# YuxiaWu/RAG4DyG

Hardware: AMD Instinct MI355X
Metric: query-seqs/sec encode+top-k over full pool (higher is better)
Workload: dtype f32 (f16x2 operands: two fp16 terms, three products, f32 accumulate)

## Files before the change

include/r4d.h:

```cpp
#ifndef R4D_H
#define R4D_H

#include <stddef.h>
#include <stdint.h>

#ifdef __cplusplus
extern "C" {
#endif

#define R4D_OK 0
#define R4D_ERR_INVALID (-1)
#define R4D_ERR_HIP (-2)
#define R4D_ERR_WORKSPACE (-3)

#define R4D_ABI_VERSION 6

int r4d_abi_version(void);
int r4d_build_flags(void);
const char* r4d_last_error(void);

typedef struct r4d_gpt2_config {
    int32_t n_layer;
    int32_t n_head;
    int32_t n_embd;
    int32_t vocab;
    int32_t n_positions;
    float   ln_eps;
} r4d_gpt2_config;

typedef struct r4d_gpt2_layer {
    const float* ln_1_w;      const float* ln_1_b;
    const float* c_attn_w;    const float* c_attn_b;
    const float* attn_proj_w; const float* attn_proj_b;
    const float* ln_2_w;      const float* ln_2_b;
    const float* c_fc_w;      const float* c_fc_b;
    const float* mlp_proj_w;  const float* mlp_proj_b;
    const float* c_attn_wT;   const float* attn_proj_wT;
    const float* c_fc_wT;     const float* mlp_proj_wT;
    const uint16_t* c_attn_w3;  const uint16_t* attn_proj_w3;
    const uint16_t* c_fc_w3;    const uint16_t* mlp_proj_w3;
    const uint16_t* c_attn_w3t; const uint16_t* attn_proj_w3t;
    const uint16_t* c_fc_w3t;   const uint16_t* mlp_proj_w3t;
    const float* c_attn_wTg;    const float* c_attn_lnc;
    const float* c_fc_wTg;      const float* c_fc_lnc;
    const uint16_t* c_attn_h2;  const uint16_t* attn_proj_h2;
    const uint16_t* c_fc_h2;    const uint16_t* mlp_proj_h2;
} r4d_gpt2_layer;

typedef struct r4d_gpt2_weights {
    const float* wte;
    const float* wpe;
    const float* ln_f_w;
    const float* ln_f_b;
    const r4d_gpt2_layer* layers;
    const float* lm_head;
} r4d_gpt2_weights;

size_t r4d_gpt2_workspace_bytes(const r4d_gpt2_config* cfg, int32_t B, int32_t T);

int r4d_gpt2_encode_f32(const r4d_gpt2_config* cfg, const r4d_gpt2_weights* w,
                        const int64_t* ids_d, const float* inputs_embeds_d, int32_t B, int32_t T,
                        float* out_hidden_d, float* out_meanpool_d, float* out_layers_d, float* out_qkv_d,
                        void* workspace_d, size_t workspace_bytes, void* stream);

size_t r4d_gpt2_groups_workspace_bytes(const r4d_gpt2_config* cfg, int32_t n_groups, const int32_t* Bs,
                                       const int32_t* Ts);
int r4d_gpt2_encode_groups_f32(const r4d_gpt2_config* cfg, const r4d_gpt2_weights* w, int32_t n_groups,
                               const int64_t* const* ids_d, const int32_t* Bs, const int32_t* Ts,
                               float* out_meanpool_d, void* workspace_d, size_t workspace_bytes, void* stream);

int r4d_gpt2_encode_groups_ex_f32(const r4d_gpt2_config* cfg, const r4d_gpt2_weights* w, int32_t n_groups,
                                  const int64_t* const* ids_d, const float* const* embeds_d, const int32_t* Bs,
                                  const int32_t* Ts, float* out_hidden_d, float* out_meanpool_d, float* out_qkv_d,
                                  void* workspace_d, size_t workspace_bytes, void* stream);

size_t r4d_gpt2_decode_workspace_bytes(const r4d_gpt2_config* cfg, int32_t B);
int r4d_gpt2_decode_step_f32(const r4d_gpt2_config* cfg, const r4d_gpt2_weights* w, const int64_t* ids_d,
                             const float* inputs_embeds_d, const int32_t* pos_d, float* kv_cache_d, int32_t B,
                             int32_t t_cap, float* out_hidden_d, void* workspace_d, size_t workspace_bytes,
                             void* stream);

typedef struct r4d_greedy_state {
    float* last_d;
    float* logits_d;
    int64_t* next_d;
    int32_t* lens_d;
    int32_t* pos_d;
    int32_t* active_d;
    int32_t* gen_len_d;
    int32_t* out_tokens_d;
    const int32_t* params_d;
    int32_t out_cap;
} r4d_greedy_state;
typedef struct r4d_decode_graph r4d_decode_graph;

size_t r4d_gpt2_greedy_workspace_bytes(const r4d_gpt2_config* cfg, int32_t B);
int r4d_gpt2_greedy_step_f32(const r4d_gpt2_config* cfg, const r4d_gpt2_weights* w, const r4d_greedy_state* st,
                             float* kv_cache_d, int32_t B, int32_t t_cap, void* workspace_d, size_t workspace_bytes,
                             void* stream);
int r4d_gpt2_greedy_graph_create(const r4d_gpt2_config* cfg, const r4d_gpt2_weights* w, const r4d_greedy_state* st,
                                 float* kv_cache_d, int32_t B, int32_t t_cap, void* workspace_d, size_t workspace_bytes,
                                 r4d_decode_graph** out_graph);
int r4d_decode_graph_launch(r4d_decode_graph* graph, int32_t n_steps, void* stream);
void r4d_decode_graph_destroy(r4d_decode_graph* graph);

int r4d_lm_logits_f32(const float* hidden_d, const float* wte_d, int32_t M, int32_t V, int32_t d,
                      float* logits_d, void* stream);

int r4d_set_attention_fused(int32_t mode);

int r4d_set_attention_h2(int32_t on);
int r4d_set_attention_kblk(int32_t on);
int r4d_pack_kblk_words(const uint32_t* qkv_words_d, int64_t rows, int32_t n_head, int32_t d, uint32_t* kblk_d, void* stream);
int r4d_attention_h2_kblk_f32(const uint32_t* qkv_words_d, const uint32_t* kblk_d, int32_t B, int32_t T, int32_t n_head, int32_t d,
                              float* a_d, void* stream);
int r4d_pack_h2_words_f32(const float* x_d, int64_t n, uint32_t* words_d, void* stream);
int r4d_attention_h2_f32(const uint32_t* qkv_words_d, int32_t B, int32_t T, int32_t n_head, int32_t d, float* a_d, void* stream);

int r4d_set_gemm_h2p(int32_t on);
int r4d_layernorm_lines_f32(const float* x_d, const float* w_d, const float* b_d, int32_t rows, int32_t d, float eps,
                            uint16_t* y_lines_d, void* stream);
int r4d_split2_lines_f16(const float* x_d, int64_t rows, int32_t K, uint16_t* lines_d, void* stream);
int r4d_conv1d_h2p_f32(const uint16_t* x_lines_d, const uint16_t* planes_d, const float* bias_d, const float* residual_d, int32_t M,
                       int32_t K, int32_t N, int32_t epilogue, int32_t out_lines, void* y_d, void* stream);

#define R4D_RANGE_NONFINITE_HIDDEN 1u
#define R4D_RANGE_BAD_NORM 2u
#define R4D_RANGE_BAD_LABEL 4u
int r4d_set_range_flag(uint32_t* flag_d);

int r4d_layernorm_f32(const float* x_d, const float* w_d, const float* b_d, int32_t rows, int32_t d,
                      float eps, float* y_d, void* stream);
int r4d_conv1d_f32(const float* x_d, const float* w_d, const float* w_t_d ,
                   const float* bias_d, const float* residual_d,
                   int32_t M, int32_t K, int32_t N, int32_t epilogue, float* y_d, void* stream);
int r4d_split3_planes_bf16(const float* w_d, int32_t K, int32_t N, int32_t transposed, uint16_t* planes_d, void* stream);
int r4d_conv1d_s3_f32(const float* x_d, const uint16_t* planes_d, const float* bias_d, const float* residual_d,
                      int32_t M, int32_t K, int32_t N, int32_t epilogue, float* y_d, void* stream);
int r4d_split2_planes_f16(const float* w_d, int32_t K, int32_t N, int32_t transposed, uint16_t* planes_d, void* stream);
int r4d_conv1d_h2_f32(const float* x_d, const uint16_t* planes_d, const float* bias_d, const float* residual_d,
                      int32_t M, int32_t K, int32_t N, int32_t epilogue, float* y_d, void* stream);
int r4d_fold_layernorm_f32(const float* wT_d, const float* ln_w_d, const float* ln_b_d, int32_t N, int32_t K, float* wTg_d,
                           float* lnc_d, void* stream);
int r4d_set_gemm_split3(int32_t mode);
int r4d_get_gemm_split3(void);
size_t r4d_attention_workspace_bytes(int32_t B, int32_t n_head, int32_t T);
int r4d_attention_f32(const float* qkv_d, int32_t B, int32_t T, int32_t n_head, int32_t d,
                      float* a_d, void* scores_ws_d, size_t ws_bytes, void* stream);

int r4d_normalize_rows_f32(const float* x_d, int32_t n, int32_t d, float* out_d, void* stream);

size_t r4d_score_topk_workspace_bytes(int32_t Q, int32_t N, int32_t k);
int r4d_score_topk_f32(const float* q_hat_d, const float* pool_hat_d, int32_t Q, int32_t N, int32_t d,
                       int32_t k, int64_t index_offset, float* out_val_d, int64_t* out_idx_d,
                       float* out_scores_d, void* workspace_d, size_t workspace_bytes, void* stream);
size_t r4d_topk_f32_workspace_bytes(int32_t rows, int32_t n, int32_t k);
int r4d_topk_f32(const float* m_d, int32_t rows, int32_t n, int32_t k, float* out_val_d, int64_t* out_idx_d,
                 void* workspace_d, size_t workspace_bytes, void* stream);
size_t r4d_merge_topk_workspace_bytes(int32_t G, int32_t Q, int32_t k);
int r4d_merge_topk_f32(const float* vals_d, const int64_t* idx_d, int32_t G, int32_t Q, int32_t k,
                       float* out_val_d, int64_t* out_idx_d, void* workspace_d, size_t workspace_bytes, void* stream);
size_t r4d_argsort_workspace_bytes(int32_t rows, int32_t n, int32_t elem_bytes);
int r4d_argsort_desc_f32(const float* scores_d, int32_t rows, int32_t n, int32_t* perm_d, void* workspace_d,
                         size_t workspace_bytes, void* stream);
int r4d_argsort_desc_f64(const double* scores_d, int32_t rows, int32_t n, int32_t* perm_d, void* workspace_d,
                         size_t workspace_bytes, void* stream);

int r4d_jaccard_f64(const int32_t* a_ptr_d, const int32_t* a_idx_d, int32_t na, int32_t a_nnz,
                    const int32_t* b_ptr_d, const int32_t* b_idx_d, int32_t nb, int32_t b_nnz,
                    int32_t vocab, int32_t zero_diag, double* out_d, void* stream);
int r4d_jaccard_ordered_f64(const int32_t* a_ptr_d, const int32_t* a_idx_d, int32_t na, int32_t a_nnz,
                            const int32_t* b_ptr_d, const int32_t* b_idx_d, int32_t nb, int32_t b_nnz,
                            int32_t vocab, int32_t zero_diag, const int32_t* a_order_d,
                            const uint32_t* a_dense_d, const uint32_t* b_dense_d, double* out_d, void* stream);
size_t r4d_jaccard_prepared_workspace_bytes(int32_t na, int32_t a_nnz, int32_t nb, int32_t b_nnz, int32_t vocab);
int r4d_jaccard_prepared_f64(const int32_t* a_ptr_d, const int32_t* a_idx_d, int32_t na, int32_t a_nnz,
                             const int32_t* b_ptr_d, const int32_t* b_idx_d, int32_t nb, int32_t b_nnz,
                             int32_t vocab, int32_t zero_diag, int32_t dense_split, int32_t sort_rows,
                             double* out_d, void* workspace_d, size_t workspace_bytes, void* stream);
size_t r4d_topk_f64_workspace_bytes(int32_t rows, int32_t n, int32_t k);
int r4d_topk_f64(const double* m_d, int32_t rows, int32_t n, int32_t k, double* out_val_d,
                 int32_t* out_idx_d, void* workspace_d, size_t workspace_bytes, void* stream);

typedef struct r4d_gpt2_layer_grads {
    float* ln_1_w;      float* ln_1_b;
    float* c_attn_w;    float* c_attn_b;
    float* attn_proj_w; float* attn_proj_b;
    float* ln_2_w;      float* ln_2_b;
    float* c_fc_w;      float* c_fc_b;
    float* mlp_proj_w;  float* mlp_proj_b;
} r4d_gpt2_layer_grads;
typedef struct r4d_gpt2_grads {
    float* wte;
    float* wpe;
    float* ln_f_w;
    float* ln_f_b;
    const r4d_gpt2_layer_grads* layers;
} r4d_gpt2_grads;

typedef struct {
    float embd_p, attn_p, resid_p;
    uint64_t seed, step;
} r4d_train_dropout;
#define R4D_DROPOUT_SITE_EMBD 65535u
int r4d_dropout_f32(const float* x_d, const float* resid_d, int64_t n, float* out_d, float p, uint64_t seed, uint64_t step,
                    uint32_t site, uint64_t index_base, void* stream);

int r4d_set_train_attention(int32_t mode);
int r4d_get_train_attention(void);

size_t r4d_gpt2_train_workspace_bytes(const r4d_gpt2_config* cfg, int32_t n_groups, const int32_t* Bs, const int32_t* Ts);
int r4d_gpt2_train_forward_f32(const r4d_gpt2_config* cfg, const r4d_gpt2_weights* w, int32_t n_groups,
                               const int64_t* const* ids_d, const int32_t* Bs, const int32_t* Ts, float* out_meanpool_d,
                               const r4d_train_dropout* dropout, void* workspace_d, size_t workspace_bytes, void* stream);
int r4d_gpt2_train_backward_f32(const r4d_gpt2_config* cfg, const r4d_gpt2_weights* w, const r4d_gpt2_grads* grads,
                                int32_t n_groups, const int64_t* const* ids_d, const int32_t* Bs, const int32_t* Ts,
                                const float* d_meanpool_d, const r4d_train_dropout* dropout,
                                void* workspace_d, size_t workspace_bytes, void* stream);
size_t r4d_retriever_losses_workspace_bytes(int32_t B);
int r4d_retriever_losses_f32(const float* emb_d, const float* t_anchor_d, const float* t_pos_d, const float* t_neg_d, int32_t B,
                             int32_t d, float temperature, float lambda_decay, float alpha, float grad_scale, float* losses_d,
                             float* d_emb_d, void* workspace_d, size_t workspace_bytes, void* stream);
int r4d_gpt2_train_forward_hidden_f32(const r4d_gpt2_config* cfg, const r4d_gpt2_weights* w, int32_t n_groups,
                                      const int64_t* const* ids_d, const int32_t* Bs, const int32_t* Ts, float* out_hidden_d,
                                      const r4d_train_dropout* dropout, void* workspace_d, size_t workspace_bytes, void* stream);
int r4d_gpt2_train_backward_hidden_f32(const r4d_gpt2_config* cfg, const r4d_gpt2_weights* w, const r4d_gpt2_grads* grads,
                                       int32_t n_groups, const int64_t* const* ids_d, const int32_t* Bs, const int32_t* Ts,
                                       const float* d_hidden_d, const r4d_train_dropout* dropout,
                                       void* workspace_d, size_t workspace_bytes, void* stream);
size_t r4d_lm_ce_workspace_bytes(int32_t N);
int r4d_lm_ce_f32(float* logits_d, int32_t N, int32_t V, int32_t ldV, const int64_t* ids_d, const int64_t* labels_d, int32_t T,
                  float grad_scale, float* loss_d, void* workspace_d, size_t workspace_bytes, void* stream);
typedef struct {
    const float* wte_pad;
    int32_t ldV;
    const uint16_t* w3;
    const uint16_t* w3t;
    const uint16_t* h2;
} r4d_lm_head;
size_t r4d_gpt2_lm_train_workspace_bytes(const r4d_gpt2_config* cfg, int32_t B, int32_t T, int32_t ldV);
int r4d_gpt2_lm_train_step_f32(const r4d_gpt2_config* cfg, const r4d_gpt2_weights* w, const r4d_gpt2_grads* grads,
                               const r4d_lm_head* head, const int64_t* ids_d, int32_t B, int32_t T, float grad_scale, float* loss_d,
                               const r4d_train_dropout* dropout, void* workspace_d, size_t workspace_bytes, void* stream);
#define R4D_HEAD_GRAD_UNTIED 0
#define R4D_HEAD_GRAD_TIED 1
#define R4D_HEAD_GRAD_NONE 2
size_t r4d_rag_train_workspace_bytes(const r4d_gpt2_config* cfg, int32_t B, int32_t Ta, int32_t ldV);
int r4d_rag_train_step_f32(const r4d_gpt2_config* cfg, const r4d_gpt2_weights* w, const r4d_gpt2_grads* grads, const r4d_lm_head* head,
                           int32_t head_mode, float* head_grad_d, const int64_t* aug_ids_d, const float* fused_d, int32_t B, int32_t Ta,
                           int32_t r, float grad_scale, float* loss_d, float* d_fused_d, float* hidden_out_d,
                           const r4d_train_dropout* dropout, void* workspace_d, size_t workspace_bytes, void* stream);
int r4d_weighted_bag_f32(const float* table_d, int32_t vocab, int32_t d, const int64_t* ids_d, const float* weights_d,
                         const int32_t* offsets_d, int32_t n_bags, float* out_d, void* stream);
size_t r4d_embedding_scatter_workspace_bytes(int32_t vocab, int32_t d);
int r4d_embedding_scatter_f32(const float* src_d, const int32_t* row_of_d, const float* weights_d, const int64_t* ids_d, int32_t n,
                              int32_t d, int32_t vocab, float* out_d, void* workspace_d, size_t workspace_bytes, void* stream);
size_t r4d_weight_grad_workspace_bytes(int32_t rows, int32_t in_features, int32_t out_features);
int r4d_weight_grad_f32(const float* x_d, const float* dy_d, int32_t rows, int32_t in_features, int32_t out_features, float* dw_d,
                        float* db_d, void* workspace_d, size_t workspace_bytes, void* stream);
size_t r4d_layernorm_bwd_workspace_bytes(int32_t rows, int32_t d);
int r4d_layernorm_bwd_f32(const float* x_d, const float* w_d, const float* dy_d, const float* add_d, int32_t rows, int32_t d,
                          float eps, float* dx_d, float* dw_d, float* db_d, void* workspace_d, size_t workspace_bytes,
                          void* stream);
int r4d_gelu_new_f32(const float* pre_d, int64_t n, float* y_d, void* stream);
int r4d_gelu_new_bwd_f32(const float* pre_d, const float* dy_d, int64_t n, float* dx_d, void* stream);
int r4d_causal_softmax_bwd_f32(const float* p_d, float* dp_d, int32_t nbh, int32_t T, int32_t ld, float scale_div, void* stream);
int r4d_softmax_dropout_bwd_transpose_f32(const float* p_d, float* dp_d, float* dst_d, int32_t nbh, int32_t T, int32_t ld, float scale_div,
                                          float attn_p, uint64_t seed, uint64_t step, uint32_t site, uint64_t index_base, void* stream);
int r4d_dropout_transpose_f32(const float* p_d, float* out_d, int32_t nbh, int32_t T, int32_t ld, float attn_p, uint64_t seed,
                              uint64_t step, uint32_t site, uint64_t index_base, void* stream);
#define R4D_SUMSQ_FLOATS 1025
int r4d_sumsq_accumulate_f32(const float* x_d, int64_t n, float* accum_d, void* stream);
int r4d_adamw_step_f32(float* p_d, const float* g_d, float* m_d, float* v_d, int64_t n, double lr, double beta1, double beta2,
                       double eps, double weight_decay, int32_t step, const float* grad_sumsq_d, float max_grad_norm,
                       void* stream);

int r4d_profile_enable(int32_t on);
int r4d_profile_num_classes(void);
const char* r4d_profile_class_name(int32_t cls);
int r4d_profile_read(int32_t cls, double* total_ms, int64_t* launches, double* work);

int r4d_dispatch_num_branches(void);
const char* r4d_dispatch_branch_name(int32_t i);
int64_t r4d_dispatch_branch_hits(int32_t i);
int r4d_dispatch_reset(void);

#ifdef __cplusplus
}
#endif
#endif
```

rag4dyg_amd/_lib.py:

```python
import ctypes
import os
from ctypes import POINTER, Structure, c_char_p, c_double, c_float, c_int32, c_int64, c_size_t, c_uint32, c_uint64, c_void_p

PKG = os.path.dirname(os.path.abspath(__file__))
LIB_PATH = os.environ.get("R4D_LIB_PATH") or os.path.join(PKG, "librag4dyg_hip.so")

R4D_ABI_VERSION = 6
HEAD_GRAD_UNTIED, HEAD_GRAD_TIED, HEAD_GRAD_NONE = 0, 1, 2


class R4DError(RuntimeError):
    pass


class GPT2ConfigC(Structure):
    _fields_ = [("n_layer", c_int32), ("n_head", c_int32), ("n_embd", c_int32), ("vocab", c_int32),
                ("n_positions", c_int32), ("ln_eps", c_float)]


class GPT2LayerC(Structure):
    _fields_ = [(n, c_void_p) for n in ("ln_1_w", "ln_1_b", "c_attn_w", "c_attn_b", "attn_proj_w", "attn_proj_b",
                                         "ln_2_w", "ln_2_b", "c_fc_w", "c_fc_b", "mlp_proj_w", "mlp_proj_b",
                                         "c_attn_wT", "attn_proj_wT", "c_fc_wT", "mlp_proj_wT",
                                         "c_attn_w3", "attn_proj_w3", "c_fc_w3", "mlp_proj_w3",
                                         "c_attn_w3t", "attn_proj_w3t", "c_fc_w3t", "mlp_proj_w3t",
                                         "c_attn_wTg", "c_attn_lnc", "c_fc_wTg", "c_fc_lnc",
                                         "c_attn_h2", "attn_proj_h2", "c_fc_h2", "mlp_proj_h2")]


class GreedyStateC(Structure):
    _fields_ = [(n, c_void_p) for n in ("last_d", "logits_d", "next_d", "lens_d", "pos_d", "active_d", "gen_len_d",
                                         "out_tokens_d", "params_d")] + [("out_cap", c_int32)]


class GPT2LayerGradsC(Structure):
    _fields_ = [(n, c_void_p) for n in ("ln_1_w", "ln_1_b", "c_attn_w", "c_attn_b", "attn_proj_w", "attn_proj_b",
                                         "ln_2_w", "ln_2_b", "c_fc_w", "c_fc_b", "mlp_proj_w", "mlp_proj_b")]


class TrainDropoutC(Structure):
    _fields_ = [("embd_p", c_float), ("attn_p", c_float), ("resid_p", c_float), ("seed", c_uint64), ("step", c_uint64)]


class GPT2GradsC(Structure):
    _fields_ = [("wte", c_void_p), ("wpe", c_void_p), ("ln_f_w", c_void_p), ("ln_f_b", c_void_p),
                ("layers", POINTER(GPT2LayerGradsC))]


class LMHeadC(Structure):
    _fields_ = [("wte_pad", c_void_p), ("ldV", c_int32), ("w3", c_void_p), ("w3t", c_void_p), ("h2", c_void_p)]


class GPT2WeightsC(Structure):
    _fields_ = [("wte", c_void_p), ("wpe", c_void_p), ("ln_f_w", c_void_p), ("ln_f_b", c_void_p),
                ("layers", POINTER(GPT2LayerC)), ("lm_head", c_void_p)]


_P = c_void_p
PROTOTYPES = {
    "r4d_abi_version": (c_int32, []),
    "r4d_build_flags": (c_int32, []),
    "r4d_last_error": (c_char_p, []),
    "r4d_gpt2_workspace_bytes": (c_size_t, [POINTER(GPT2ConfigC), c_int32, c_int32]),
    "r4d_gpt2_encode_f32": (c_int32, [POINTER(GPT2ConfigC), POINTER(GPT2WeightsC), _P, _P, c_int32, c_int32,
                                      _P, _P, _P, _P, _P, c_size_t, _P]),
    "r4d_gpt2_groups_workspace_bytes": (c_size_t, [POINTER(GPT2ConfigC), c_int32, POINTER(c_int32), POINTER(c_int32)]),
    "r4d_gpt2_encode_groups_f32": (c_int32, [POINTER(GPT2ConfigC), POINTER(GPT2WeightsC), c_int32, POINTER(_P),
                                             POINTER(c_int32), POINTER(c_int32), _P, _P, c_size_t, _P]),
    "r4d_gpt2_encode_groups_ex_f32": (c_int32, [POINTER(GPT2ConfigC), POINTER(GPT2WeightsC), c_int32, POINTER(_P), POINTER(_P),
                                                POINTER(c_int32), POINTER(c_int32), _P, _P, _P, _P, c_size_t, _P]),
    "r4d_set_attention_fused": (c_int32, [c_int32]),
    "r4d_set_attention_h2": (c_int32, [c_int32]),
    "r4d_set_attention_kblk": (c_int32, [c_int32]),
    "r4d_pack_kblk_words": (c_int32, [_P, c_int64, c_int32, c_int32, _P, _P]),
    "r4d_attention_h2_kblk_f32": (c_int32, [_P, _P, c_int32, c_int32, c_int32, c_int32, _P, _P]),
    "r4d_set_range_flag": (c_int32, [_P]),
    "r4d_set_gemm_h2p": (c_int32, [c_int32]),
    "r4d_layernorm_lines_f32": (c_int32, [_P, _P, _P, c_int32, c_int32, c_float, _P, _P]),
    "r4d_split2_lines_f16": (c_int32, [_P, c_int64, c_int32, _P, _P]),
    "r4d_conv1d_h2p_f32": (c_int32, [_P, _P, _P, _P, c_int32, c_int32, c_int32, c_int32, c_int32, _P, _P]),
    "r4d_pack_h2_words_f32": (c_int32, [_P, c_int64, _P, _P]),
    "r4d_attention_h2_f32": (c_int32, [_P, c_int32, c_int32, c_int32, c_int32, _P, _P]),
    "r4d_gpt2_decode_workspace_bytes": (c_size_t, [POINTER(GPT2ConfigC), c_int32]),
    "r4d_gpt2_decode_step_f32": (c_int32, [POINTER(GPT2ConfigC), POINTER(GPT2WeightsC), _P, _P, _P, _P, c_int32, c_int32,
                                           _P, _P, c_size_t, _P]),
    "r4d_gpt2_greedy_workspace_bytes": (c_size_t, [POINTER(GPT2ConfigC), c_int32]),
    "r4d_gpt2_greedy_step_f32": (c_int32, [POINTER(GPT2ConfigC), POINTER(GPT2WeightsC), POINTER(GreedyStateC), _P, c_int32,
                                           c_int32, _P, c_size_t, _P]),
    "r4d_gpt2_greedy_graph_create": (c_int32, [POINTER(GPT2ConfigC), POINTER(GPT2WeightsC), POINTER(GreedyStateC), _P,
                                               c_int32, c_int32, _P, c_size_t, POINTER(_P)]),
    "r4d_decode_graph_launch": (c_int32, [_P, c_int32, _P]),
    "r4d_decode_graph_destroy": (None, [_P]),
    "r4d_lm_logits_f32": (c_int32, [_P, _P, c_int32, c_int32, c_int32, _P, _P]),
    "r4d_layernorm_f32": (c_int32, [_P, _P, _P, c_int32, c_int32, c_float, _P, _P]),
    "r4d_conv1d_f32": (c_int32, [_P, _P, _P, _P, _P, c_int32, c_int32, c_int32, c_int32, _P, _P]),
    "r4d_split3_planes_bf16": (c_int32, [_P, c_int32, c_int32, c_int32, _P, _P]),
    "r4d_conv1d_s3_f32": (c_int32, [_P, _P, _P, _P, c_int32, c_int32, c_int32, c_int32, _P, _P]),
    "r4d_split2_planes_f16": (c_int32, [_P, c_int32, c_int32, c_int32, _P, _P]),
    "r4d_conv1d_h2_f32": (c_int32, [_P, _P, _P, _P, c_int32, c_int32, c_int32, c_int32, _P, _P]),
    "r4d_fold_layernorm_f32": (c_int32, [_P, _P, _P, c_int32, c_int32, _P, _P, _P]),
    "r4d_set_gemm_split3": (c_int32, [c_int32]),
    "r4d_get_gemm_split3": (c_int32, []),
    "r4d_attention_workspace_bytes": (c_size_t, [c_int32, c_int32, c_int32]),
    "r4d_attention_f32": (c_int32, [_P, c_int32, c_int32, c_int32, c_int32, _P, _P, c_size_t, _P]),
    "r4d_normalize_rows_f32": (c_int32, [_P, c_int32, c_int32, _P, _P]),
    "r4d_score_topk_workspace_bytes": (c_size_t, [c_int32, c_int32, c_int32]),
    "r4d_score_topk_f32": (c_int32, [_P, _P, c_int32, c_int32, c_int32, c_int32, c_int64, _P, _P, _P, _P,
                                     c_size_t, _P]),
    "r4d_topk_f32_workspace_bytes": (c_size_t, [c_int32, c_int32, c_int32]),
    "r4d_topk_f32": (c_int32, [_P, c_int32, c_int32, c_int32, _P, _P, _P, c_size_t, _P]),
    "r4d_merge_topk_workspace_bytes": (c_size_t, [c_int32, c_int32, c_int32]),
    "r4d_merge_topk_f32": (c_int32, [_P, _P, c_int32, c_int32, c_int32, _P, _P, _P, c_size_t, _P]),
    "r4d_argsort_workspace_bytes": (c_size_t, [c_int32, c_int32, c_int32]),
    "r4d_argsort_desc_f32": (c_int32, [_P, c_int32, c_int32, _P, _P, c_size_t, _P]),
    "r4d_argsort_desc_f64": (c_int32, [_P, c_int32, c_int32, _P, _P, c_size_t, _P]),
    "r4d_jaccard_f64": (c_int32, [_P, _P, c_int32, c_int32, _P, _P, c_int32, c_int32, c_int32, c_int32, _P, _P]),
    "r4d_jaccard_ordered_f64": (c_int32, [_P, _P, c_int32, c_int32, _P, _P, c_int32, c_int32, c_int32, c_int32, _P, _P, _P, _P, _P]),
    "r4d_jaccard_prepared_workspace_bytes": (c_size_t, [c_int32, c_int32, c_int32, c_int32, c_int32]),
    "r4d_jaccard_prepared_f64": (c_int32, [_P, _P, c_int32, c_int32, _P, _P, c_int32, c_int32, c_int32, c_int32, c_int32, c_int32, _P, _P,
                                           c_size_t, _P]),
    "r4d_topk_f64_workspace_bytes": (c_size_t, [c_int32, c_int32, c_int32]),
    "r4d_topk_f64": (c_int32, [_P, c_int32, c_int32, c_int32, _P, _P, _P, c_size_t, _P]),
    "r4d_gpt2_train_workspace_bytes": (c_size_t, [POINTER(GPT2ConfigC), c_int32, POINTER(c_int32), POINTER(c_int32)]),
    "r4d_gpt2_train_forward_f32": (c_int32, [POINTER(GPT2ConfigC), POINTER(GPT2WeightsC), c_int32, POINTER(_P), POINTER(c_int32),
                                             POINTER(c_int32), _P, POINTER(TrainDropoutC), _P, c_size_t, _P]),
    "r4d_gpt2_train_backward_f32": (c_int32, [POINTER(GPT2ConfigC), POINTER(GPT2WeightsC), POINTER(GPT2GradsC), c_int32, POINTER(_P),
                                              POINTER(c_int32), POINTER(c_int32), _P, POINTER(TrainDropoutC), _P, c_size_t, _P]),
    "r4d_gpt2_train_forward_hidden_f32": (c_int32, [POINTER(GPT2ConfigC), POINTER(GPT2WeightsC), c_int32, POINTER(_P), POINTER(c_int32),
                                                    POINTER(c_int32), _P, POINTER(TrainDropoutC), _P, c_size_t, _P]),
    "r4d_gpt2_train_backward_hidden_f32": (c_int32, [POINTER(GPT2ConfigC), POINTER(GPT2WeightsC), POINTER(GPT2GradsC), c_int32,
                                                     POINTER(_P), POINTER(c_int32), POINTER(c_int32), _P, POINTER(TrainDropoutC), _P,
                                                     c_size_t, _P]),
    "r4d_lm_ce_workspace_bytes": (c_size_t, [c_int32]),
    "r4d_lm_ce_f32": (c_int32, [_P, c_int32, c_int32, c_int32, _P, _P, c_int32, c_float, _P, _P, c_size_t, _P]),
    "r4d_gpt2_lm_train_workspace_bytes": (c_size_t, [POINTER(GPT2ConfigC), c_int32, c_int32, c_int32]),
    "r4d_gpt2_lm_train_step_f32": (c_int32, [POINTER(GPT2ConfigC), POINTER(GPT2WeightsC), POINTER(GPT2GradsC), POINTER(LMHeadC), _P,
                                             c_int32, c_int32, c_float, _P, POINTER(TrainDropoutC), _P, c_size_t, _P]),
    "r4d_rag_train_workspace_bytes": (c_size_t, [POINTER(GPT2ConfigC), c_int32, c_int32, c_int32]),
    "r4d_rag_train_step_f32": (c_int32, [POINTER(GPT2ConfigC), POINTER(GPT2WeightsC), POINTER(GPT2GradsC), POINTER(LMHeadC), c_int32, _P,
                                         _P, _P, c_int32, c_int32, c_int32, c_float, _P, _P, _P, POINTER(TrainDropoutC), _P, c_size_t, _P]),
    "r4d_weighted_bag_f32": (c_int32, [_P, c_int32, c_int32, _P, _P, _P, c_int32, _P, _P]),
    "r4d_embedding_scatter_workspace_bytes": (c_size_t, [c_int32, c_int32]),
    "r4d_embedding_scatter_f32": (c_int32, [_P, _P, _P, _P, c_int32, c_int32, c_int32, _P, _P, c_size_t, _P]),
    "r4d_retriever_losses_workspace_bytes": (c_size_t, [c_int32]),
    "r4d_retriever_losses_f32": (c_int32, [_P, _P, _P, _P, c_int32, c_int32, c_float, c_float, c_float, c_float, _P, _P, _P, c_size_t, _P]),
    "r4d_dropout_f32": (c_int32, [_P, _P, c_int64, _P, c_float, c_uint64, c_uint64, c_uint32, c_uint64, _P]),
    "r4d_weight_grad_workspace_bytes": (c_size_t, [c_int32, c_int32, c_int32]),
    "r4d_weight_grad_f32": (c_int32, [_P, _P, c_int32, c_int32, c_int32, _P, _P, _P, c_size_t, _P]),
    "r4d_layernorm_bwd_workspace_bytes": (c_size_t, [c_int32, c_int32]),
    "r4d_layernorm_bwd_f32": (c_int32, [_P, _P, _P, _P, c_int32, c_int32, c_float, _P, _P, _P, _P, c_size_t, _P]),
    "r4d_gelu_new_f32": (c_int32, [_P, c_int64, _P, _P]),
    "r4d_gelu_new_bwd_f32": (c_int32, [_P, _P, c_int64, _P, _P]),
    "r4d_causal_softmax_bwd_f32": (c_int32, [_P, _P, c_int32, c_int32, c_int32, c_float, _P]),
    "r4d_softmax_dropout_bwd_transpose_f32": (c_int32, [_P, _P, _P, c_int32, c_int32, c_int32, c_float, c_float, c_uint64, c_uint64,
                                                        c_uint32, c_uint64, _P]),
    "r4d_dropout_transpose_f32": (c_int32, [_P, _P, c_int32, c_int32, c_int32, c_float, c_uint64, c_uint64, c_uint32, c_uint64, _P]),
    "r4d_set_train_attention": (c_int32, [c_int32]),
    "r4d_get_train_attention": (c_int32, []),
    "r4d_sumsq_accumulate_f32": (c_int32, [_P, c_int64, _P, _P]),
    "r4d_adamw_step_f32": (c_int32, [_P, _P, _P, _P, c_int64, c_double, c_double, c_double, c_double, c_double, c_int32, _P, c_float, _P]),
    "r4d_dispatch_num_branches": (c_int32, []),
    "r4d_dispatch_branch_name": (c_char_p, [c_int32]),
    "r4d_dispatch_branch_hits": (c_int64, [c_int32]),
    "r4d_dispatch_reset": (c_int32, []),
    "r4d_profile_enable": (c_int32, [c_int32]),
    "r4d_profile_num_classes": (c_int32, []),
    "r4d_profile_class_name": (c_char_p, [c_int32]),
    "r4d_profile_read": (c_int32, [c_int32, POINTER(c_double), POINTER(c_int64), POINTER(c_double)]),
}

_LIB = None


def load():
    global _LIB
    if _LIB is not None:
        return _LIB
    if not os.path.exists(LIB_PATH):
        raise R4DError(f"{LIB_PATH} not found: build it with `python -m rag4dyg_amd.build` "
                       "(there is no CPU fallback for the product path)")
    import torch
    lib = ctypes.CDLL(LIB_PATH, mode=ctypes.RTLD_GLOBAL)
    for name, (res, args) in PROTOTYPES.items():
        fn = getattr(lib, name)
        fn.restype = res
        fn.argtypes = args
    got = lib.r4d_abi_version()
    if got != R4D_ABI_VERSION:
        raise R4DError(f"ABI mismatch: library {got}, binding {R4D_ABI_VERSION}")
    flags = lib.r4d_build_flags()
    if flags and os.environ.get("R4D_ALLOW_ABLATED_LIB") != "1":
        raise R4DError(f"{LIB_PATH} is a kernel-ablation build (r4d_build_flags() = {flags:#x}): timing aid for tools/ only; "
                       "the product refuses it (set R4D_ALLOW_ABLATED_LIB=1 in a tuning script)")
    _LIB = lib
    return lib


def check(rc, what):
    if rc != 0:
        msg = load().r4d_last_error().decode("utf-8", "replace")
        raise R4DError(f"{what} failed (rc={rc}): {msg}")
```

rag4dyg_amd/build.py:

```python
import os
import subprocess
import sys
from concurrent.futures import ThreadPoolExecutor

PKG = os.path.dirname(os.path.abspath(__file__))
CSRC = os.path.join(PKG, "csrc")
OBJ = os.path.join(PKG, "_build")
LIB = os.path.join(PKG, "librag4dyg_hip.so")
HIPCC = os.environ.get("HIPCC", "/opt/rocm/bin/hipcc")
FLAGS = ["-O3", "--offload-arch=gfx950", "-fPIC", "-std=c++17", "-Wall", "-Wno-unused-function"]


def sources():
    return sorted(os.path.join(CSRC, f) for f in os.listdir(CSRC) if f.endswith(".hip"))


def _deps_mtime():
    hdrs = [os.path.join(CSRC, f) for f in os.listdir(CSRC) if f.endswith(".h")]
    hdrs.append(os.path.join(os.path.dirname(PKG), "include", "r4d.h"))
    return max(os.path.getmtime(h) for h in hdrs)


def _compile(src, force, hdr_m):
    obj = os.path.join(OBJ, os.path.basename(src)[:-4] + ".o")
    if not force and os.path.exists(obj) and os.path.getmtime(obj) >= max(os.path.getmtime(src), hdr_m):
        return obj, False
    cmd = [HIPCC, *FLAGS, "-c", src, "-o", obj]
    r = subprocess.run(cmd, capture_output=True, text=True)
    if r.returncode != 0:
        raise RuntimeError(f"hipcc failed for {src}:\n{r.stdout}\n{r.stderr}")
    if r.stderr.strip():
        sys.stderr.write(r.stderr)
    return obj, True


HANDOFF_KERNELS = {"topk.hip": {"topk_chunk_kernelIfE": (4, 2), "topk_chunk_kernelIdE": (4, 2)},
                   "gemm_skinny.hip": {"gemm_skinny16_kernelILi2ELi0E": (2, 1), "gemm_skinny16_kernelILi3ELi0E": (2, 1)}}


def check_handoff_lowering(src):
    import re
    import tempfile
    names = HANDOFF_KERNELS[os.path.basename(src)]
    with tempfile.TemporaryDirectory() as td:
        asm = os.path.join(td, "k.s")
        r = subprocess.run([HIPCC, "-O3", "--offload-arch=gfx950", "-std=c++17", "--offload-device-only", "-S", src, "-o", asm],
                           capture_output=True, text=True)
        if r.returncode != 0:
            raise RuntimeError(f"hipcc -S failed for {src}:\n{r.stderr}")
        text = open(asm).read()
    for name, (want_st, want_ld) in names.items():
        m = re.search(r"^(_ZN3r4d\d+" + re.escape(name) + r"[^\n:]*):[^\n]*\n(.*?)s_endpgm", text, re.S | re.M)
        if not m:
            raise RuntimeError(f"hand-off check: kernel {name} not found in the assembly of {src}")
        body = m.group(2)
        stores = re.findall(r"global_store_dword(?:x2)? [^\n]*", body)
        loads_sc1 = [ln for ln in re.findall(r"global_load_dword(?:x2)? [^\n]*", body) if " sc1" in ln]
        stores_sc1 = [ln for ln in stores if " sc1" in ln]
        ticket = re.findall(r"global_atomic_add[^\n]*", body)
        if not ticket or len(stores_sc1) < want_st or len(loads_sc1) < want_ld:
            raise RuntimeError(f"hand-off check FAILED for {name}: {len(stores_sc1)} sc1 stores (want {want_st}), {len(loads_sc1)} sc1 loads (want {want_ld}), "
                               f"{len(ticket)} ticket atomics -- the relaxed agent-scope publish / consume of {os.path.basename(src)} "
                               "is no longer lowered to write-through / L1-bypassing instructions; use release / acquire there")


PACKED_F32_FILES = ("gemm_h2.hip", "attention_h2.hip")
PACKED_F32_FORMS = {
    "v_pk_mul_f32 V, V, S op_sel_hi:[1,0]", "v_pk_mul_f32 V, S, V op_sel_hi:[0,1]", "v_pk_mul_f32 V, V, S", "v_pk_mul_f32 V, S, V",
    "v_pk_fma_f32 V, V, S, V op_sel_hi:[1,0,1]", "v_pk_fma_f32 V, S, V, V op_sel_hi:[0,1,1]", "v_pk_fma_f32 V, V, S, V", "v_pk_fma_f32 V, S, V, V",
    "v_pk_fma_f32 V, V, S, V op_sel_hi:[1,0,1] neg_lo:[0,0,1] neg_hi:[0,0,1]",
    "v_pk_fma_f32 V, V, S, V op_sel_hi:[1,0,0] neg_lo:[1,0,0] neg_hi:[1,0,0]",
    "v_pk_fma_f32 V, S, V, V op_sel_hi:[0,1,1] neg_lo:[1,0,0] neg_hi:[1,0,0]",
    "v_pk_add_f32 V, V, S op_sel_hi:[1,0]", "v_pk_add_f32 V, S, V op_sel_hi:[0,1]",
}


def check_packed_f32_forms(src):
    import re
    import tempfile
    with tempfile.TemporaryDirectory() as td:
        asm = os.path.join(td, "k.s")
        r = subprocess.run([HIPCC, "-O3", "--offload-arch=gfx950", "-std=c++17", "--offload-device-only", "-S", src, "-o", asm],
                           capture_output=True, text=True)
        if r.returncode != 0:
            raise RuntimeError(f"hipcc -S failed for {src}:\n{r.stderr}")
        text = open(asm).read()
    seen = {}
    for ln in re.findall(r"^\s*(v_pk_(?:fma|mul|add)_f32 [^\n;]*)", text, re.M):
        if not re.search(r"\bs\[?\d", ln):
            continue
        form = re.sub(r"a\[[0-9:]+\]", "V", re.sub(r"v\[[0-9:]+\]", "V", re.sub(r"\bs\[[0-9:]+\]|\bs\d+\b", "S", ln))).strip()
        seen[form] = seen.get(form, 0) + 1
    new = {f: n for f, n in seen.items() if f not in PACKED_F32_FORMS}
    if new:
        raise RuntimeError(f"packed-fp32 census FAILED for {os.path.basename(src)}: operand forms with an SGPR source that "
                           f"tools/pk_fma_probe.hip has not verified on gfx950: {new} -- add the form to the probe, run it on the GPU, "
                           "then list it in rag4dyg_amd/build.py:PACKED_F32_FORMS (or pin that arithmetic scalar)")
    return seen


def build_library(force=False, verbose=True):
    os.makedirs(OBJ, exist_ok=True)
    hdr_m = _deps_mtime()
    with ThreadPoolExecutor(max_workers=4) as ex:
        res = list(ex.map(lambda s: _compile(s, force, hdr_m), sources()))
    objs = [o for o, _ in res]
    for src, (_o, compiled) in zip(sources(), res):
        if compiled and os.path.basename(src) in HANDOFF_KERNELS:
            check_handoff_lowering(src)
        if compiled and os.path.basename(src) in PACKED_F32_FILES:
            check_packed_f32_forms(src)
    stale = os.path.exists(LIB) and any(os.path.getmtime(o) > os.path.getmtime(LIB) for o in objs)
    if force or stale or any(c for _, c in res) or not os.path.exists(LIB):
        cmd = [HIPCC, "--offload-arch=gfx950", "-shared", "-fPIC", "-o", LIB, *objs]
        r = subprocess.run(cmd, capture_output=True, text=True)
        if r.returncode != 0:
            raise RuntimeError(f"link failed:\n{r.stdout}\n{r.stderr}")
        if verbose:
            print(f"built {LIB}")
    elif verbose:
        print(f"up to date: {LIB}")
    return LIB


if __name__ == "__main__":
    build_library(force="--force" in sys.argv)
```

rag4dyg_amd/csrc/common.h:

```cpp
#pragma once
#include <hip/hip_runtime.h>
#include <stdint.h>
#include <stdio.h>
#include <stdarg.h>
#include "../../include/r4d.h"

namespace r4d {

void set_error(const char* fmt, ...);
int dbgflag_kc(); int dbgflag_att(); int dbgflag_sk(); int dbgflag_jac(); int dbgflag_scan(); int dbgflag_s3(); int dbgflag_h2();

#define R4D_REQUIRE(cond, ...)                     \
    do {                                           \
        if (!(cond)) {                             \
            r4d::set_error(__VA_ARGS__);           \
            return R4D_ERR_INVALID;                \
        }                                          \
    } while (0)

#define R4D_HIP(call)                                                                  \
    do {                                                                               \
        hipError_t e_ = (call);                                                        \
        if (e_ != hipSuccess) {                                                        \
            r4d::set_error("%s: %s", #call, hipGetErrorString(e_));                    \
            return R4D_ERR_HIP;                                                        \
        }                                                                              \
    } while (0)

#define R4D_CHECK_LAUNCH(name)                                                         \
    do {                                                                               \
        hipError_t e_ = hipGetLastError();                                             \
        if (e_ != hipSuccess) {                                                        \
            r4d::set_error("%s: launch failed: %s", name, hipGetErrorString(e_));      \
            return R4D_ERR_HIP;                                                        \
        }                                                                              \
    } while (0)

enum ProfClass {
    PK_GEMM_128x128_NN = 0, PK_GEMM_128x128_NT, PK_GEMM_128x64_NN, PK_GEMM_128x64_NT, PK_GEMM_64x64_NN,
    PK_GEMM_64x64_NT, PK_GEMM_KC_128x128x32, PK_GEMM_KC_128x128x16, PK_GEMM_KC_128x64x16, PK_GEMM_KC_64x64x32, PK_GEMM_S3_128x256, PK_GEMM_S3_128x128, PK_GEMM_S3TN, PK_GEMM_H2_128x256, PK_GEMM_H2_128x128, PK_GEMM_SKINNY, PK_GEMM_SKINNY_EPI,
    PK_EMBED_LN, PK_LAYERNORM, PK_SOFTMAX, PK_DECODE_ATTN, PK_GREEDY_ADVANCE,
    PK_ATTN_FUSED, PK_LNF_MEANPOOL, PK_MEANPOOL_REDUCE, PK_NORMALIZE, PK_POOL_SCAN, PK_TOPK, PK_MERGE_TOPK, PK_RANK_COUNT, PK_JACCARD, PK_JACCARD_PREP, PK_LM_CE,
    PK_SPLICE_EMBED, PK_WEIGHTED_BAG, PK_EMB_SCATTER, PK_COUNT
};
extern bool g_prof_on;
void prof_begin_impl(int cls, double work, hipStream_t s);
void prof_end_impl(hipStream_t s);
struct ProfScope {
    hipStream_t s; bool on;
    ProfScope(int cls, double work, hipStream_t st) : s(st), on(g_prof_on) { if (on) prof_begin_impl(cls, work, s); }
    ~ProfScope() { if (on) prof_end_impl(s); }
};

#define R4D_BRANCH_LIST(X)                                                                                              \
    X(KC_128x128x16, "gemm_kc:128x128x16") X(KC_128x64x16, "gemm_kc:128x64x16") X(KC_64x64x32, "gemm_kc:64x64x32")       \
    X(KC_128x128x32, "tuning:gemm_kc:128x128x32") X(KC_ROWSPLIT, "gemm_kc:row-split (two launches)")                      \
    X(S3_128x256, "gemm_s3:128x256x32") X(S3_PERSISTENT, "gemm_s3:128x256x32 persistent (pipeline across tiles)") X(S3_128x128, "gemm_s3:128x128x32") X(S3_F32B, "gemm_s3:both operands split on the fly (scoring GEMM)") X(S3_TN, "gemm_s3tn:128x256x32 (weight gradients, transposing LDS reads)")      \
    X(H2_128x256, "gemm_h2:128x256x32 (f16x2)") X(H2_128x128, "gemm_h2:128x128x32 (f16x2)") X(H2P_128x256, "gemm_h2p:128x256x32 (f16x2, A as lines, LDS-DMA)") X(H2P_128x128, "gemm_h2p:128x128x32 (f16x2, A as lines, LDS-DMA)") \
    X(F32_128x128, "gemm_f32:128x128") X(F32_128x64, "gemm_f32:128x64") X(F32_64x64, "gemm_f32:64x64")                   \
    X(F32_NT, "gemm_f32:B as [N,K]") X(F32_NN, "gemm_f32:B as [K,N]") X(TN_SPLITK, "gemm_tn:split-K") X(TN_SINGLE, "gemm_tn:one slice") \
    X(SK16_NG2, "skinny16:ng2") X(SK16_NG3, "skinny16:ng3") X(SK16_NG2_LN, "skinny16:ng2+layernorm") X(SK16_LN_FOLDED, "skinny16:LayerNorm pre-folded into the weight") X(SK16_NG3_LN, "skinny16:ng3+layernorm") \
    X(SK16_SPLITK, "skinny16:split-K last-arriver") X(SK8_NG2, "skinny8:ng2") X(SK8_NG3, "skinny8:ng3")                    \
    X(SK8_LN, "tuning:skinny8:+layernorm") X(SK8_SPLITK, "skinny8:split-K + epilogue launch") X(SK_PLAIN, "skinny:plain + epilogue launch") \
    X(ATT_KS32, "attention:key-split hd32") X(ATT_KS64, "attention:key-split hd64") X(ATT_CS96, "attention:column-split hd96") \
    X(ATT_CS128, "attention:column-split hd128") X(ATT_CS256, "attention:column-split hd256") X(ATT_H2_KS32, "attention:f16x2 key-split hd32") X(ATT_H2_KS64, "attention:f16x2 key-split hd64") X(ATT_H2_KS96, "attention:f16x2 key-split hd96") X(ATT_H2_128, "attention:f16x2 hd128") X(ATT_H2_256, "attention:f16x2 hd256") X(ATT_H2_KS32_KBLK, "attention:f16x2 key-split hd32, key-blocked K") X(ATT_H2_KS64_KBLK, "attention:f16x2 key-split hd64, key-blocked K") X(ATT_H2_KS96_KBLK, "attention:f16x2 key-split hd96, key-blocked K") X(ATT_H2_128_KBLK, "attention:f16x2 hd128, key-blocked K") X(ATT_H2_256_KBLK, "attention:f16x2 hd256, key-blocked K")                              \
    X(ATT_KS_FORCED, "tuning:attention:key-split at hd96/128/256") X(ATT_3LAUNCH, "attention:three-launch GEMM form")      \
    X(SCAN_1_1, "scan:d32") X(SCAN_2_1, "scan:d64") X(SCAN_4_1, "scan:d128") X(SCAN_4_2, "scan:d256") X(SCAN_4_3, "scan:d384") \
    X(SCAN_8_2, "scan:d512") X(SCAN_4_4, "tuning:scan:d512 4-way") X(SCAN_8_3, "scan:d768") X(SCAN_8_4, "scan:d1024")       \
    X(SCAN_SHORT, "scan:short shard (even rows, two tiles in flight)") X(SCAN_DMA, "scan:short shard, LDS-DMA staged") X(SCAN_RING, "scan:long shard, LDS-DMA ring") X(SCAN_GEMM, "scan:tiled GEMM (Q > 64 or other d)") X(SCAN_TILED, "scan:128x256 tiles in the scan kernels' arithmetic (Q >= 64)") X(SCAN_BF16X3, "scan:bf16x3 operands") X(SCAN_F32, "scan:exact-f32 operands")  \
    X(TOPK_ONE_WG, "topk:one workgroup per row") X(TOPK_TICKET, "topk:cross-workgroup ticket merge")                      \
    X(TOPK_MULTI, "topk:second launch over candidates") X(TOPK_F64, "topk:f64 rows")                                      \
    X(EMBED_LN4, "embed+layernorm:16-byte lanes") X(EMBED_GENERIC, "embed+layernorm:generic") X(LN4_2, "layernorm:ln4<2>") X(LN4_4, "layernorm:ln4<4>") X(LN4_8, "layernorm:ln4<8>") X(LN_GENERIC, "layernorm:generic") \
    X(LNF_8, "lnf_meanpool:<8>") X(LNF_16, "lnf_meanpool:<16>") X(LNF_32, "lnf_meanpool:<32>")                             \
    X(DEC_ATT_32, "decode_attention:<32>") X(DEC_ATT_64, "decode_attention:<64>")                                         \
    X(JAC_LDS, "jaccard:LDS table") X(JAC_MERGE, "jaccard:merge walk (vocab too large for LDS)")                          \
    X(JAC_PREP_DENSE_LDS, "jaccard_prep:dense tokens, LDS histogram") X(JAC_PREP_DENSE_GLOBAL, "jaccard_prep:dense tokens, global histogram") X(JAC_PREP_ORDER, "jaccard_prep:rows longest first") \
    X(ARGSORT_ONE, "argsort:one chunk") X(ARGSORT_MULTI, "argsort:chunk sort + rank scatter")
enum DispatchBranch {
#define X(id, name) BR_##id,
    R4D_BRANCH_LIST(X)
#undef X
    BR_COUNT
};
extern unsigned long long g_branch_hits[BR_COUNT];
#define R4D_BRANCH(id) (++r4d::g_branch_hits[r4d::BR_##id])

extern unsigned* g_range_flag;

static inline size_t align_up(size_t x, size_t a) { return (x + a - 1) / a * a; }
static inline int cdiv(int a, int b) { return (a + b - 1) / b; }

enum GemmEpilogue { EPI_NONE = 0, EPI_GELU = 1, EPI_RESIDUAL = 2, EPI_SCALE_DIV = 3, EPI_HALF_PLUS = 4,
                    EPI_GELU_KEEP = 5, EPI_GELU_GRAD = 6,
                    EPI_H2WORDS = 7 };
enum GemmCausal { CAUSAL_NONE = 0, CAUSAL_QK = 1, CAUSAL_PV = 2 };

struct GemmArgs {
    const float* A; const float* B; float* C;
    const float* bias;
    const float* resid;
    int M, N, K;
    int lda, ldb, ldc, ldr;
    int b_trans;
    int b_rows;
    int a_cols;
    int nbatch, nb1;
    long long sA0, sA1, sB0, sB1, sC0, sC1;
    int epilogue; float scale_div;
    int causal;
};
int launch_gemm_f32(const GemmArgs& g, hipStream_t stream);
int launch_gemm_f32_kc(const GemmArgs& g, hipStream_t stream);
size_t gemm_tn_scratch_floats(int M, int N, int Kt);
int launch_gemm_f32_tn(const float* A, const float* B, float* C, int M, int N, int Kt, int lda, int ldb, float* scratch,
                       hipStream_t stream, float* colsum_out = nullptr, float* colsum_scratch = nullptr,
                       size_t colsum_scratch_floats = 0, bool* colsum_done = nullptr);
bool gemm_skinny_supported(int M, int K, int N);
size_t gemm_skinny_scratch_floats(int K, int N);
bool gemm_skinny_fuses_ln(int M, int K, int N);
void* gemm_skinny_counters(float* scratch, size_t* bytes);
int launch_gemm_skinny(const float* x, const float* wT, const float* bias, const float* resid, int M, int K, int N,
                       int epilogue, float* y, float* scratch, hipStream_t s, const float* ln_w = nullptr,
                       const float* ln_b = nullptr, float ln_eps = 0.f, bool counters_zeroed = false, const float* ln_fold = nullptr);
int launch_fold_layernorm(const float* wT, const float* g, const float* beta, int N, int K, float* wTg, float* lnc, hipStream_t s);

struct S3Args {
    const float* A; const unsigned short* planes; float* C;
    const float* bias; const float* resid;
    int M, N, K, lda, ldc, ldr, epilogue;
    unsigned* kblk; int kb_hd;
};
bool gemm_s3_supported(int M, int K, int N);
int launch_gemm_s3(const S3Args& a, hipStream_t stream);
bool gemm_s3_f32b_supported(int M, int K, int N);
int launch_gemm_s3_f32b(const float* A, const float* B, float* C, int M, int N, int K, int lda, int ldc, int epilogue, hipStream_t stream);
int launch_gemm_s3_scan_order(const float* q_hat, const float* pool_hat, float* scores, int Q, int N, int d, int ng, hipStream_t stream);
bool gemm_h2_supported(int M, int K, int N);
int launch_gemm_h2(const S3Args& a, hipStream_t stream);
int launch_split2_planes(const float* w, int N, int K, long long ld_k, long long ld_n, unsigned short* planes, hipStream_t s);
extern int g_gemm_h2p;
bool gemm_h2p_supported(int M, int K, int N);
int launch_gemm_h2p(const S3Args& a, const unsigned short* a_lines, bool out_lines, hipStream_t stream);
int launch_split2_lines(const float* x, long long rows, int K, unsigned short* lines, hipStream_t s);
extern int g_gemm_split3;
int conv1d(const float* x, const float* w, const float* wT, const float* bias, const float* resid, int M, int K, int N,
           int epilogue, float* y, hipStream_t s, float* skinny_scratch = nullptr, bool sk_counters_zeroed = false,
           const unsigned short* w3 = nullptr, const unsigned short* w2h = nullptr);
bool gemm_s3tn_supported(int I, int J, int M, int lda, int ldb);
int gemm_s3tn_slices(int I, int J, int M, int max_slices);
int launch_gemm_s3tn(const float* X, const float* dY, float* out, int I, int J, int M, int lda, int ldb, int S, int* slices_out,
                     hipStream_t stream, float* db_partials = nullptr);
int launch_split3_planes(const float* w, int N, int K, long long ld_k, long long ld_n, unsigned short* planes, hipStream_t s);

struct DropKey { unsigned seed_lo, seed_hi, step_lo, step_hi; };
int launch_dropout(const float* x, const float* resid, long long n, float* out, float p, DropKey key, unsigned site,
                   unsigned long long base, hipStream_t s);
constexpr int EMB_SUM_BITS = 62;
__device__ __forceinline__ int emb_scale_exp(unsigned max_bits, int lg_rows) {
    const int e = (int)((max_bits >> 23) & 255u) - 126;
    return EMB_SUM_BITS - lg_rows - e;
}
static inline int emb_lg_rows(long long table_rows) {
    int lg = 0;
    while ((1LL << lg) < table_rows) ++lg;
    return lg;
}
int launch_embedding_fix_to_f32(const unsigned long long* acc, long long n, long long table_rows, float* out, hipStream_t s);

size_t gpt2_train_workspace_floats(const r4d_gpt2_config* cfg, int n_groups, const int32_t* Bs, const int32_t* Ts);
struct SpliceIn { const float* fused; int r; };
int gpt2_train_forward(const r4d_gpt2_config* cfg, const r4d_gpt2_weights* w, int n_groups, const int64_t* const* ids_d,
                       const int32_t* Bs, const int32_t* Ts, float* out_meanpool_d, float* out_hidden_d,
                       const r4d_train_dropout* dropout, void* workspace_d, size_t workspace_bytes, hipStream_t s,
                       const SpliceIn* sp = nullptr);
int gpt2_train_backward(const r4d_gpt2_config* cfg, const r4d_gpt2_weights* w, const r4d_gpt2_grads* gr, int n_groups,
                        const int64_t* const* ids_d, const int32_t* Bs, const int32_t* Ts, const float* d_meanpool_d,
                        const float* d_hidden_d, const r4d_train_dropout* dropout, void* workspace_d, size_t workspace_bytes,
                        hipStream_t s, const SpliceIn* sp = nullptr, float* d_fused = nullptr);
int launch_splice_embed_ln(const int64_t* aug_ids, const float* fused, int r, const float* wte, const float* wpe, int vocab, int B,
                           int T, int d, const float* w, const float* b, float eps, float* x_out, float* y_out, hipStream_t s);

struct LMLayout { size_t train, h, logits, dh, dwte, tn, ce, total; };
LMLayout lm_layout(const r4d_gpt2_config* cfg, int B, int T, int ldV);
int check_ce(int N, int V, int ldV, int T);
int lm_head_train(const float* h, int N, int V, int d, const r4d_lm_head* head, const int64_t* src, int T, float gscale, float* loss,
                  float* logits, float* dh, float* dwte, float* tn_scratch, float* ce_ws, hipStream_t s);
int launch_add_inplace(float* y, const float* x, long long n, hipStream_t s);

template <typename T> size_t topk_ws_bytes(int rows, int n, int k);
template <typename T>
int topk_rows(const T* vals, const long long* idx_in, int rows, int n, long long ld, int k, long long index_offset, T* out_v,
              long long* out_i, void* ws, size_t ws_bytes, bool counters_zeroed, hipStream_t s);

int launch_layernorm(const float* x, const float* w, const float* b, int rows, int d, float eps, float* y,
                     hipStream_t s);
bool layernorm_lines_supported(int d);
int launch_layernorm_lines(const float* x, const float* w, const float* b, int rows, int d, float eps, unsigned short* y_lines, hipStream_t s);
constexpr int ATT_MAXG = 16;
struct RowGroups {
    int n;
    int B[ATT_MAXG], T[ATT_MAXG];
    const int64_t* ids[ATT_MAXG];
    const float* emb[ATT_MAXG];
};
int launch_embed_layernorm_groups(const RowGroups& G, const float* wte, const float* wpe, int vocab, int d,
                                  const float* w, const float* b, float eps, float* x_out, float* y_out, hipStream_t s, bool y_lines = false);
int launch_causal_softmax(float* S, int nbh, int T, int ld, int row_tile, hipStream_t s);
int launch_embed_pos_layernorm(const int64_t* ids, const float* emb, const int32_t* pos, const float* wte,
                               const float* wpe, int vocab, int n_positions, int t_cap, int B, int d, const float* w,
                               const float* b, float eps, float* x_out, float* y_out, hipStream_t s,
                               void* zero_words = nullptr, size_t zero_bytes = 0);
int launch_decode_attention(const float* qkv_new, float* kv_layer, const int32_t* pos, int B, int t_cap, int H, int d,
                            float* out, hipStream_t s);
struct GreedyState {
    int64_t* next; int32_t* lens; int32_t* pos; int32_t* active; int32_t* gen_len; int32_t* out_tokens;
    const int32_t* params;
    int out_cap, t_cap;
};
struct GreedyEmbed { const float* wte; const float* wpe; float* x_out; unsigned* zero_words; int vocab, n_positions, d, n_zero; };
int launch_greedy_advance(const float* logits, int B, int V, const GreedyState& st, hipStream_t s, const GreedyEmbed* embed = nullptr);
struct AttnGroups {
    int n;
    int seq_prefix[ATT_MAXG + 1];
    int T[ATT_MAXG];
    long long row0[ATT_MAXG];
};
bool attention_h2_supported(int H, int d);
int launch_attention_h2_groups(const unsigned* qkv_words, int n, const int* Bs, const int* Ts, const long long* row0s, int H, int d,
                               float* out, hipStream_t s, bool out_lines = false, const unsigned* kblk = nullptr);
int launch_pack_kblk_words(const unsigned* qkv_words, long long M, int H, int d, unsigned* kblk, hipStream_t s);
static inline size_t kblk_words(size_t M, int d) { return (M + 31) / 32 * 32 * (size_t)d; }
int launch_pack_h2_words(const float* x, long long n, unsigned* words, hipStream_t s);
int dbgflag_att_h2();
int launch_attention_fused(const float* qkv, int B, int T, int H, int d, float* out, hipStream_t s);
int launch_attention_fused_groups(const float* qkv, int n, const int* Bs, const int* Ts, const long long* row0s, int H,
                                  int d, float* out, hipStream_t s);
extern int g_attention_variant;
extern int g_attention_fused;
constexpr int LNF_ROWS_PER_CHUNK = 16;
size_t lnf_meanpool_scratch_floats(int B, int T, int d);
int launch_lnf_meanpool_groups(const RowGroups& G, const float* x, const float* w, const float* b, int d, float eps,
                               float* hidden_out, float* pool_out, float* scratch, hipStream_t s);

}
```

rag4dyg_amd/csrc/encoder.hip:

```cpp
#include <math.h>
#include <stdlib.h>
#include <string.h>
#include <vector>
#include "common.h"

namespace r4d {

static thread_local char g_err[512] = "";
void set_error(const char* fmt, ...) {
    va_list ap;
    va_start(ap, fmt);
    vsnprintf(g_err, sizeof(g_err), fmt, ap);
    va_end(ap);
}

int g_gemm_split3 = 1;

int conv1d(const float* x, const float* w, const float* wT, const float* bias, const float* resid, int M, int K,
           int N, int epilogue, float* y, hipStream_t s, float* skinny_scratch, bool sk_counters_zeroed,
           const unsigned short* w3, const unsigned short* w2h) {
    if (skinny_scratch && wT && gemm_skinny_supported(M, K, N))
        return launch_gemm_skinny(x, wT, bias, resid, M, K, N, epilogue, y, skinny_scratch, s, nullptr, nullptr, 0.f,
                                  sk_counters_zeroed);
    if (w2h && g_gemm_split3 == 2 && (epilogue <= EPI_RESIDUAL || epilogue == EPI_GELU_KEEP || epilogue == EPI_H2WORDS) && gemm_h2_supported(M, K, N)) {
        S3Args a;
        memset(&a, 0, sizeof(a));
        a.A = x; a.planes = w2h; a.C = y; a.bias = bias; a.resid = resid;
        a.M = M; a.N = N; a.K = K; a.lda = K; a.ldc = N; a.ldr = N; a.epilogue = epilogue;
        return launch_gemm_h2(a, s);
    }
    if (w3 && g_gemm_split3 && gemm_s3_supported(M, K, N)) {
        S3Args a;
        memset(&a, 0, sizeof(a));
        a.A = x; a.planes = w3; a.C = y; a.bias = bias; a.resid = resid;
        a.M = M; a.N = N; a.K = K; a.lda = K; a.ldc = N; a.ldr = N; a.epilogue = epilogue;
        return launch_gemm_s3(a, s);
    }
    R4D_REQUIRE(epilogue != EPI_H2WORDS, "conv1d: the h2-word epilogue exists in the f16x2 GEMM only");
    GemmArgs g;
    memset(&g, 0, sizeof(g));
    g.A = x; g.C = y; g.bias = bias; g.resid = resid;
    g.M = M; g.N = N; g.K = K; g.lda = K; g.ldc = N; g.ldr = N;
    if (wT) { g.B = wT; g.ldb = K; g.b_trans = 1; g.b_rows = N; }
    else { g.B = w; g.ldb = N; g.b_trans = 0; g.b_rows = K; }
    g.nbatch = 1; g.nb1 = 1;
    g.epilogue = epilogue; g.scale_div = 1.f; g.causal = CAUSAL_NONE;
    return launch_gemm_f32(g, s);
}

static int conv1d_lines(const unsigned short* x_lines, const unsigned short* w2h, const float* bias, const float* resid, int M, int K, int N,
                        int epilogue, void* y, bool out_lines, hipStream_t s, unsigned* kblk = nullptr, int kb_hd = 0) {
    S3Args a;
    memset(&a, 0, sizeof(a));
    a.planes = w2h; a.C = (float*)y; a.bias = bias; a.resid = resid;
    a.M = M; a.N = N; a.K = K; a.lda = K; a.ldc = N; a.ldr = N; a.epilogue = epilogue;
    a.kblk = kblk; a.kb_hd = kb_hd;
    return launch_gemm_h2p(a, x_lines, out_lines, s);
}

static inline int tpad(int T) { return (T + 127) / 128 * 128; }

int g_attention_fused = -1;
int g_attention_h2 = 1;
static int g_attention_kblk = -1;

static int attention(const float* qkv, int B, int T, int H, int d, float* a_out, float* scores, hipStream_t s) {
    const bool fused = g_attention_fused != 0;
    if (fused) {
        const int rc_f = launch_attention_fused(qkv, B, T, H, d, a_out, s);
        if (rc_f <= 0) return rc_f;
    }
    R4D_BRANCH(ATT_3LAUNCH);
    const int hd = d / H, ld = tpad(T);
    GemmArgs g;
    memset(&g, 0, sizeof(g));
    g.A = qkv; g.B = qkv + d; g.C = scores;
    g.M = T; g.N = T; g.K = hd; g.lda = 3 * d; g.ldb = 3 * d; g.ldc = ld;
    g.b_trans = 1; g.b_rows = T; g.nbatch = B * H; g.nb1 = H;
    g.sA0 = (long long)T * 3 * d; g.sA1 = hd; g.sB0 = g.sA0; g.sB1 = hd;
    g.sC0 = (long long)H * T * ld; g.sC1 = (long long)T * ld;
    g.epilogue = EPI_SCALE_DIV; g.scale_div = (float)sqrt((double)hd); g.causal = CAUSAL_QK;
    int rc = launch_gemm_f32(g, s);
    if (rc) return rc;
    rc = launch_causal_softmax(scores, B * H, T, ld, 128, s);
    if (rc) return rc;
    memset(&g, 0, sizeof(g));
    g.A = scores; g.B = qkv + 2 * d; g.C = a_out;
    g.M = T; g.N = hd; g.K = T; g.lda = ld; g.ldb = 3 * d; g.ldc = d;
    g.b_trans = 0; g.b_rows = T; g.nbatch = B * H; g.nb1 = H;
    g.sA0 = (long long)H * T * ld; g.sA1 = (long long)T * ld;
    g.sB0 = (long long)T * 3 * d; g.sB1 = hd; g.sC0 = (long long)T * d; g.sC1 = hd;
    g.a_cols = ld;
    g.epilogue = EPI_NONE; g.scale_div = 1.f; g.causal = CAUSAL_PV;
    return launch_gemm_f32(g, s);
}

struct Group {
    const int64_t* ids; const float* emb; int B, T; size_t row0, seq0;
};

static RowGroups row_groups(const Group* groups, int g0, int n_groups) {
    RowGroups R;
    R.n = n_groups - g0 < ATT_MAXG ? n_groups - g0 : ATT_MAXG;
    for (int j = 0; j < ATT_MAXG; ++j) {
        const bool in = j < R.n;
        R.B[j] = in ? groups[g0 + j].B : 0; R.T[j] = in ? groups[g0 + j].T : 0;
        R.ids[j] = in ? groups[g0 + j].ids : nullptr; R.emb[j] = in ? groups[g0 + j].emb : nullptr;
    }
    return R;
}

struct Workspace {
    float *x, *ln, *qkv, *att, *fc, *scores, *pool;
    unsigned* kblk;
    size_t bytes;
};
static Workspace carve(void* base, size_t M, size_t score_floats, size_t pool_floats, int d) {
    size_t off = 0;
    auto take = [&](size_t nfloat) {
        float* p = base ? (float*)((char*)base + off) : nullptr;
        off += align_up(nfloat * sizeof(float), 256);
        return p;
    };
    Workspace w;
    w.x = take(M * d); w.ln = take(M * d); w.qkv = take(M * 3 * d); w.att = take(M * d); w.fc = take(M * 4 * d);
    w.scores = take(score_floats);
    w.pool = take(pool_floats);
    w.kblk = reinterpret_cast<unsigned*>(take(kblk_words(M, d)));
    w.bytes = off;
    return w;
}
static size_t score_floats(int B, int H, int T) { return (size_t)B * H * T * tpad(T); }

static int check_cfg(const r4d_gpt2_config* c) {
    R4D_REQUIRE(c != nullptr, "gpt2: null config");
    R4D_REQUIRE(c->n_layer >= 1 && c->n_head >= 1 && c->n_embd >= 64, "gpt2: bad config L=%d H=%d d=%d", c->n_layer,
                c->n_head, c->n_embd);
    R4D_REQUIRE(c->n_embd % 64 == 0 && c->n_embd <= 2048, "gpt2: n_embd=%d must be a multiple of 64, <= 2048", c->n_embd);
    R4D_REQUIRE(c->n_embd % c->n_head == 0 && (c->n_embd / c->n_head) % 16 == 0,
                "gpt2: head_dim=%d/%d must be a multiple of 16", c->n_embd, c->n_head);
    return R4D_OK;
}

}

using namespace r4d;

extern "C" {

int r4d_abi_version(void) { return R4D_ABI_VERSION; }
int r4d_build_flags(void) {
    return dbgflag_kc() | (dbgflag_att() << 1) | (dbgflag_sk() << 2) | (dbgflag_jac() << 3) | (dbgflag_scan() << 4) | (dbgflag_s3() << 5) | (dbgflag_h2() << 6) | (dbgflag_att_h2() << 7);
}
int r4d_fold_layernorm_f32(const float* wT_d, const float* ln_w_d, const float* ln_b_d, int32_t N, int32_t K, float* wTg_d,
                           float* lnc_d, void* stream) {
    return launch_fold_layernorm(wT_d, ln_w_d, ln_b_d, N, K, wTg_d, lnc_d, (hipStream_t)stream);
}

int r4d_set_gemm_split3(int32_t mode) { g_gemm_split3 = mode == 2 ? 2 : (mode != 0); return R4D_OK; }
int r4d_get_gemm_split3(void) { return g_gemm_split3; }
int r4d_set_range_flag(uint32_t* flag_d) { g_range_flag = flag_d; return R4D_OK; }
int r4d_set_attention_kblk(int32_t on) {
    const int prev = g_attention_kblk < 0 ? 1 : g_attention_kblk;
    g_attention_kblk = on != 0;
    return prev;
}
int r4d_set_attention_h2(int32_t on) {
    const int prev = g_attention_h2;
    g_attention_h2 = on != 0;
    return prev;
}

int r4d_set_attention_fused(int32_t mode) {
    g_attention_variant = (mode == 2) ? 1 : 0;
    g_attention_fused = mode < 0 ? -1 : (mode != 0);
    return R4D_OK;
}
const char* r4d_last_error(void) { return g_err; }

size_t r4d_gpt2_workspace_bytes(const r4d_gpt2_config* cfg, int32_t B, int32_t T) {
    if (!cfg || B <= 0 || T <= 0) return 0;
    return carve(nullptr, (size_t)B * T, score_floats(B, cfg->n_head, T), lnf_meanpool_scratch_floats(B, T, cfg->n_embd),
                 cfg->n_embd).bytes;
}

size_t r4d_gpt2_groups_workspace_bytes(const r4d_gpt2_config* cfg, int32_t n_groups, const int32_t* Bs,
                                       const int32_t* Ts) {
    if (!cfg || n_groups <= 0 || !Bs || !Ts) return 0;
    size_t M = 0, sc = 0, pl = 0;
    for (int g = 0; g < n_groups; ++g) {
        if (Bs[g] <= 0 || Ts[g] <= 0) return 0;
        M += (size_t)Bs[g] * Ts[g];
        const size_t f = score_floats(Bs[g], cfg->n_head, Ts[g]);
        if (f > sc) sc = f;
        pl += lnf_meanpool_scratch_floats(Bs[g], Ts[g], cfg->n_embd);
    }
    return carve(nullptr, M, sc, pl, cfg->n_embd).bytes;
}

}

namespace r4d {

static int encode_impl(const r4d_gpt2_config* cfg, const r4d_gpt2_weights* w, const Group* groups, int n_groups,
                       float* out_hidden_d, float* out_meanpool_d, float* out_layers_d, float* out_qkv_d,
                       void* workspace_d, size_t workspace_bytes, hipStream_t s) {
    int rc = check_cfg(cfg);
    if (rc) return rc;
    R4D_REQUIRE(w && w->wte && w->wpe && w->ln_f_w && w->ln_f_b && w->layers, "gpt2: null weights");
    R4D_REQUIRE(out_hidden_d || out_meanpool_d, "gpt2: no output requested");
    const int d = cfg->n_embd, H = cfg->n_head;
    size_t Mtot = 0, sc = 0, pl = 0;
    for (int g = 0; g < n_groups; ++g) {
        const Group& G = groups[g];
        R4D_REQUIRE((G.ids != nullptr) != (G.emb != nullptr),
                    "gpt2: specify exactly one of input_ids and inputs_embeds");
        R4D_REQUIRE(G.B >= 1 && G.T >= 1, "gpt2: empty batch B=%d T=%d", G.B, G.T);
        R4D_REQUIRE(G.T <= cfg->n_positions && G.T <= 1024, "gpt2: T=%d exceeds n_positions=%d", G.T, cfg->n_positions);
        Mtot += (size_t)G.B * G.T;
        const size_t f = score_floats(G.B, H, G.T);
        if (f > sc) sc = f;
        pl += lnf_meanpool_scratch_floats(G.B, G.T, d);
    }
    R4D_REQUIRE(Mtot <= 0x7fffffff / (size_t)(16 * d), "gpt2: %zu rows in one call is too many", Mtot);
    const int M = (int)Mtot;
    Workspace ws = carve(workspace_d, Mtot, sc, pl, d);
    if (!workspace_d || workspace_bytes < ws.bytes) {
        set_error("gpt2: workspace %zu bytes < required %zu", workspace_bytes, ws.bytes);
        return R4D_ERR_WORKSPACE;
    }
    for (int l = 0; l < cfg->n_layer; ++l) {
        const r4d_gpt2_layer& L = w->layers[l];
        R4D_REQUIRE(L.ln_1_w && L.c_attn_w && L.attn_proj_w && L.ln_2_w && L.c_fc_w && L.mlp_proj_w,
                    "gpt2: null weight in layer %d", l);
        const bool lines = g_gemm_split3 == 2 && g_gemm_h2p && L.c_attn_h2 && L.c_fc_h2 && L.mlp_proj_h2 && layernorm_lines_supported(d) &&
                           gemm_h2p_supported(M, d, 3 * d) && gemm_h2p_supported(M, d, 4 * d) && gemm_h2p_supported(M, 4 * d, d);
        unsigned short* ln_lines = reinterpret_cast<unsigned short*>(ws.ln);
        unsigned short* fc_lines = reinterpret_cast<unsigned short*>(ws.fc);
        if (l == 0) {
            for (int g0 = 0; g0 < n_groups; g0 += ATT_MAXG) {
                const RowGroups R = row_groups(groups, g0, n_groups);
                const size_t r0 = groups[g0].row0;
                rc = launch_embed_layernorm_groups(R, w->wte, w->wpe, cfg->vocab, d, L.ln_1_w, L.ln_1_b, cfg->ln_eps,
                                                   ws.x + r0 * d, ws.ln + r0 * d, s, lines);
                if (rc) return rc;
            }
        } else if ((rc = lines ? launch_layernorm_lines(ws.x, L.ln_1_w, L.ln_1_b, M, d, cfg->ln_eps, ln_lines, s)
                               : launch_layernorm(ws.x, L.ln_1_w, L.ln_1_b, M, d, cfg->ln_eps, ws.ln, s))) {
            return rc;
        }
        if (out_layers_d &&
            hipMemcpyAsync(out_layers_d + (size_t)l * M * d, ws.x, (size_t)M * d * sizeof(float),
                           hipMemcpyDeviceToDevice, s) != hipSuccess) {
            set_error("gpt2: layer copy failed");
            return R4D_ERR_HIP;
        }
        float* qkv = out_qkv_d ? out_qkv_d + (size_t)l * M * 3 * d : ws.qkv;
        bool words = !out_qkv_d && g_attention_h2 && g_attention_fused != 0 && g_gemm_split3 == 2 && L.c_attn_h2 &&
                     attention_h2_supported(H, d) && gemm_h2_supported(M, d, 3 * d);
        for (int g0 = 0; g0 < n_groups && words; g0 += ATT_MAXG) {
            int nseq = 0;
            for (int j = g0; j < n_groups && j < g0 + ATT_MAXG; ++j) nseq += groups[j].B;
            if (nseq > 65535) words = false;
        }
        if (g_attention_kblk < 0) { const char* e = getenv("R4D_ATT_KBLK"); g_attention_kblk = e ? atoi(e) != 0 : 1; }
        const bool kblk = words && lines && g_attention_kblk && (d / H) % 32 == 0;
        if (kblk && (M & 31) &&
            hipMemsetAsync(ws.kblk + (size_t)(M / 32) * 32 * d, 0, (size_t)32 * d * sizeof(unsigned), s) != hipSuccess) {
            set_error("gpt2: memset of the key-block tail failed");
            return R4D_ERR_HIP;
        }
        if (lines) rc = conv1d_lines(ln_lines, L.c_attn_h2, L.c_attn_b, nullptr, M, d, 3 * d, words ? EPI_H2WORDS : EPI_NONE, qkv, false, s,
                                     kblk ? ws.kblk : nullptr, kblk ? d / H : 0);
        else rc = conv1d(ws.ln, L.c_attn_w, L.c_attn_wT, L.c_attn_b, nullptr, M, d, 3 * d, words ? EPI_H2WORDS : EPI_NONE, qkv, s, nullptr, false, L.c_attn_w3, L.c_attn_h2);
        if (rc) return rc;
        const bool att_lines = words && lines && L.attn_proj_h2 && gemm_h2p_supported(M, d, d);
        bool fused_done = false;
        if (words) {
            fused_done = true;
            for (int g0 = 0; g0 < n_groups; g0 += ATT_MAXG) {
                int Bs[ATT_MAXG], Ts[ATT_MAXG];
                long long r0[ATT_MAXG];
                const int n = n_groups - g0 < ATT_MAXG ? n_groups - g0 : ATT_MAXG;
                for (int j = 0; j < n; ++j) { Bs[j] = groups[g0 + j].B; Ts[j] = groups[g0 + j].T; r0[j] = (long long)groups[g0 + j].row0; }
                if ((rc = launch_attention_h2_groups(reinterpret_cast<const unsigned*>(qkv), n, Bs, Ts, r0, H, d, ws.att, s, att_lines,
                                                     kblk ? ws.kblk : nullptr))) return rc;
            }
        } else if (g_attention_fused != 0) {
            fused_done = true;
            for (int g0 = 0; g0 < n_groups && fused_done; g0 += ATT_MAXG) {
                int Bs[ATT_MAXG], Ts[ATT_MAXG];
                long long r0[ATT_MAXG];
                const int n = n_groups - g0 < ATT_MAXG ? n_groups - g0 : ATT_MAXG;
                int nseq = 0;
                for (int j = 0; j < n; ++j) {
                    Bs[j] = groups[g0 + j].B; Ts[j] = groups[g0 + j].T; r0[j] = (long long)groups[g0 + j].row0;
                    nseq += Bs[j];
                }
                if (nseq > 65535) { fused_done = false; break; }
                rc = launch_attention_fused_groups(qkv, n, Bs, Ts, r0, H, d, ws.att, s);
                if (rc < 0) return rc;
                if (rc > 0) fused_done = false;
            }
        }
        if (!fused_done) {
            for (int g = 0; g < n_groups; ++g) {
                const Group& G = groups[g];
                if ((rc = attention(qkv + G.row0 * 3 * d, G.B, G.T, H, d, ws.att + G.row0 * d, ws.scores, s))) return rc;
            }
        }
        if (att_lines) rc = conv1d_lines(reinterpret_cast<const unsigned short*>(ws.att), L.attn_proj_h2, L.attn_proj_b, ws.x, M, d, d, EPI_RESIDUAL, ws.x, false, s);
        else rc = conv1d(ws.att, L.attn_proj_w, L.attn_proj_wT, L.attn_proj_b, ws.x, M, d, d, EPI_RESIDUAL, ws.x, s, nullptr, false, L.attn_proj_w3, L.attn_proj_h2);
        if (rc) return rc;
        if (lines) {
            if ((rc = launch_layernorm_lines(ws.x, L.ln_2_w, L.ln_2_b, M, d, cfg->ln_eps, ln_lines, s))) return rc;
            if ((rc = conv1d_lines(ln_lines, L.c_fc_h2, L.c_fc_b, nullptr, M, d, 4 * d, EPI_GELU, fc_lines, true, s))) return rc;
            if ((rc = conv1d_lines(fc_lines, L.mlp_proj_h2, L.mlp_proj_b, ws.x, M, 4 * d, d, EPI_RESIDUAL, ws.x, false, s))) return rc;
            continue;
        }
        if ((rc = launch_layernorm(ws.x, L.ln_2_w, L.ln_2_b, M, d, cfg->ln_eps, ws.ln, s))) return rc;
        if ((rc = conv1d(ws.ln, L.c_fc_w, L.c_fc_wT, L.c_fc_b, nullptr, M, d, 4 * d, EPI_GELU, ws.fc, s, nullptr, false, L.c_fc_w3, L.c_fc_h2))) return rc;
        if ((rc = conv1d(ws.fc, L.mlp_proj_w, L.mlp_proj_wT, L.mlp_proj_b, ws.x, M, 4 * d, d, EPI_RESIDUAL, ws.x, s, nullptr, false, L.mlp_proj_w3, L.mlp_proj_h2))) return rc;
    }
    size_t part0 = 0;
    for (int g0 = 0; g0 < n_groups; g0 += ATT_MAXG) {
        const RowGroups R = row_groups(groups, g0, n_groups);
        const Group& G = groups[g0];
        rc = launch_lnf_meanpool_groups(R, ws.x + G.row0 * d, w->ln_f_w, w->ln_f_b, d, cfg->ln_eps,
                                        out_hidden_d ? out_hidden_d + G.row0 * d : nullptr,
                                        out_meanpool_d ? out_meanpool_d + G.seq0 * d : nullptr, ws.pool + part0, s);
        if (rc) return rc;
        for (int j = 0; j < R.n; ++j) part0 += lnf_meanpool_scratch_floats(R.B[j], R.T[j], d);
    }
    return R4D_OK;
}

}

extern "C" {

int r4d_gpt2_encode_f32(const r4d_gpt2_config* cfg, const r4d_gpt2_weights* w, const int64_t* ids_d,
                        const float* inputs_embeds_d, int32_t B, int32_t T, float* out_hidden_d,
                        float* out_meanpool_d, float* out_layers_d, float* out_qkv_d, void* workspace_d,
                        size_t workspace_bytes, void* stream) {
    Group G = {ids_d, inputs_embeds_d, B, T, 0, 0};
    return encode_impl(cfg, w, &G, 1, out_hidden_d, out_meanpool_d, out_layers_d, out_qkv_d, workspace_d,
                       workspace_bytes, (hipStream_t)stream);
}

int r4d_gpt2_encode_groups_f32(const r4d_gpt2_config* cfg, const r4d_gpt2_weights* w, int32_t n_groups,
                               const int64_t* const* ids_d, const int32_t* Bs, const int32_t* Ts,
                               float* out_meanpool_d, void* workspace_d, size_t workspace_bytes, void* stream) {
    R4D_REQUIRE(n_groups >= 1 && n_groups <= 4096 && ids_d && Bs && Ts, "gpt2 groups: bad arguments");
    R4D_REQUIRE(out_meanpool_d, "gpt2 groups: out_meanpool_d is null");
    std::vector<Group> gs((size_t)n_groups);
    size_t row0 = 0, seq0 = 0;
    for (int g = 0; g < n_groups; ++g) {
        gs[g] = Group{ids_d[g], nullptr, Bs[g], Ts[g], row0, seq0};
        if (Bs[g] > 0 && Ts[g] > 0) { row0 += (size_t)Bs[g] * Ts[g]; seq0 += (size_t)Bs[g]; }
    }
    return encode_impl(cfg, w, gs.data(), n_groups, nullptr, out_meanpool_d, nullptr, nullptr, workspace_d,
                       workspace_bytes, (hipStream_t)stream);
}

int r4d_gpt2_encode_groups_ex_f32(const r4d_gpt2_config* cfg, const r4d_gpt2_weights* w, int32_t n_groups,
                                  const int64_t* const* ids_d, const float* const* embeds_d, const int32_t* Bs,
                                  const int32_t* Ts, float* out_hidden_d, float* out_meanpool_d, float* out_qkv_d,
                                  void* workspace_d, size_t workspace_bytes, void* stream) {
    R4D_REQUIRE(n_groups >= 1 && n_groups <= 4096 && Bs && Ts, "gpt2 groups: bad arguments");
    R4D_REQUIRE((ids_d != nullptr) != (embeds_d != nullptr), "gpt2 groups: specify exactly one of ids_d and embeds_d");
    std::vector<Group> gs((size_t)n_groups);
    size_t row0 = 0, seq0 = 0;
    for (int g = 0; g < n_groups; ++g) {
        gs[g] = Group{ids_d ? ids_d[g] : nullptr, embeds_d ? embeds_d[g] : nullptr, Bs[g], Ts[g], row0, seq0};
        if (Bs[g] > 0 && Ts[g] > 0) { row0 += (size_t)Bs[g] * Ts[g]; seq0 += (size_t)Bs[g]; }
    }
    return encode_impl(cfg, w, gs.data(), n_groups, out_hidden_d, out_meanpool_d, nullptr, out_qkv_d, workspace_d,
                       workspace_bytes, (hipStream_t)stream);
}

static size_t decode_skinny_floats(int d) {
    size_t m = 0;
    const int shapes[4][2] = {{d, 3 * d}, {d, d}, {d, 4 * d}, {4 * d, d}};
    for (auto& kn : shapes)
        if (gemm_skinny_supported(1, kn[0], kn[1])) { const size_t f = gemm_skinny_scratch_floats(kn[0], kn[1]); if (f > m) m = f; }
    return m;
}

size_t r4d_gpt2_decode_workspace_bytes(const r4d_gpt2_config* cfg, int32_t B) {
    if (!cfg || B <= 0) return 0;
    return carve(nullptr, (size_t)B, 0, decode_skinny_floats(cfg->n_embd), cfg->n_embd).bytes;
}

static int decode_step_impl(const r4d_gpt2_config* cfg, const r4d_gpt2_weights* w, const int64_t* ids_d,
                            const float* inputs_embeds_d, const int32_t* pos_d, float* kv_cache_d, int32_t B,
                            int32_t t_cap, float* out_hidden_d, void* workspace_d, size_t workspace_bytes,
                            void* stream, bool x_ready) {
    hipStream_t s = (hipStream_t)stream;
    int rc = check_cfg(cfg);
    if (rc) return rc;
    R4D_REQUIRE(w && w->wte && w->wpe && w->ln_f_w && w->ln_f_b && w->layers, "gpt2 decode: null weights");
    R4D_REQUIRE(x_ready || (ids_d != nullptr) != (inputs_embeds_d != nullptr), "gpt2 decode: specify exactly one of ids and inputs_embeds");
    R4D_REQUIRE(pos_d && kv_cache_d && out_hidden_d, "gpt2 decode: null pointer");
    R4D_REQUIRE(B >= 1 && t_cap >= 1, "gpt2 decode: B=%d t_cap=%d", B, t_cap);
    const int d = cfg->n_embd, H = cfg->n_head;
    const size_t sk_floats = decode_skinny_floats(d);
    Workspace ws = carve(workspace_d, (size_t)B, 0, sk_floats, d);
    if (!workspace_d || workspace_bytes < ws.bytes) {
        set_error("gpt2 decode: workspace %zu bytes < required %zu", workspace_bytes, ws.bytes);
        return R4D_ERR_WORKSPACE;
    }
    float* sk = (sk_floats && B <= 32) ? ws.pool : nullptr;
    const size_t layer_stride = (size_t)B * t_cap * 2 * d;
    size_t cbytes = 0;
    void* cnt = sk ? gemm_skinny_counters(sk, &cbytes) : nullptr;
    for (int l = 0; l < cfg->n_layer; ++l) {
        const r4d_gpt2_layer& L = w->layers[l];
        R4D_REQUIRE(L.ln_1_w && L.c_attn_w && L.attn_proj_w && L.ln_2_w && L.c_fc_w && L.mlp_proj_w,
                    "gpt2 decode: null weight in layer %d", l);
        const bool fuse_ln = sk && L.c_attn_wT && L.c_fc_wT && gemm_skinny_fuses_ln(B, d, 3 * d);
        if (l == 0 && !x_ready)
            rc = launch_embed_pos_layernorm(ids_d, inputs_embeds_d, pos_d, w->wte, w->wpe, cfg->vocab, cfg->n_positions,
                                            t_cap, B, d, L.ln_1_w, L.ln_1_b, cfg->ln_eps, ws.x, ws.ln, s, cnt, cbytes);
        else if (!fuse_ln)
            rc = launch_layernorm(ws.x, L.ln_1_w, L.ln_1_b, B, d, cfg->ln_eps, ws.ln, s);
        if (rc) return rc;
        if (fuse_ln && (l > 0 || x_ready))
            rc = (L.c_attn_wTg && L.c_attn_lnc)
                     ? launch_gemm_skinny(ws.x, L.c_attn_wTg, L.c_attn_b, nullptr, B, d, 3 * d, EPI_NONE, ws.qkv, sk, s, nullptr, nullptr,
                                          cfg->ln_eps, true, L.c_attn_lnc)
                     : launch_gemm_skinny(ws.x, L.c_attn_wT, L.c_attn_b, nullptr, B, d, 3 * d, EPI_NONE, ws.qkv, sk, s, L.ln_1_w,
                                          L.ln_1_b, cfg->ln_eps, true);
        else
            rc = conv1d(ws.ln, L.c_attn_w, L.c_attn_wT, L.c_attn_b, nullptr, B, d, 3 * d, EPI_NONE, ws.qkv, s, sk);
        if (rc) return rc;
        if ((rc = launch_decode_attention(ws.qkv, kv_cache_d + (size_t)l * layer_stride, pos_d, B, t_cap, H, d, ws.att, s)))
            return rc;
        if ((rc = conv1d(ws.att, L.attn_proj_w, L.attn_proj_wT, L.attn_proj_b, ws.x, B, d, d, EPI_RESIDUAL, ws.x, s, sk, true))) return rc;
        if (fuse_ln) {
            rc = (L.c_fc_wTg && L.c_fc_lnc)
                     ? launch_gemm_skinny(ws.x, L.c_fc_wTg, L.c_fc_b, nullptr, B, d, 4 * d, EPI_GELU, ws.fc, sk, s, nullptr, nullptr,
                                          cfg->ln_eps, true, L.c_fc_lnc)
                     : launch_gemm_skinny(ws.x, L.c_fc_wT, L.c_fc_b, nullptr, B, d, 4 * d, EPI_GELU, ws.fc, sk, s, L.ln_2_w, L.ln_2_b,
                                          cfg->ln_eps, true);
        } else {
            if ((rc = launch_layernorm(ws.x, L.ln_2_w, L.ln_2_b, B, d, cfg->ln_eps, ws.ln, s))) return rc;
            rc = conv1d(ws.ln, L.c_fc_w, L.c_fc_wT, L.c_fc_b, nullptr, B, d, 4 * d, EPI_GELU, ws.fc, s, sk);
        }
        if (rc) return rc;
        if ((rc = conv1d(ws.fc, L.mlp_proj_w, L.mlp_proj_wT, L.mlp_proj_b, ws.x, B, 4 * d, d, EPI_RESIDUAL, ws.x, s, sk, true))) return rc;
    }
    return launch_layernorm(ws.x, w->ln_f_w, w->ln_f_b, B, d, cfg->ln_eps, out_hidden_d, s);
}

int r4d_gpt2_decode_step_f32(const r4d_gpt2_config* cfg, const r4d_gpt2_weights* w, const int64_t* ids_d,
                             const float* inputs_embeds_d, const int32_t* pos_d, float* kv_cache_d, int32_t B,
                             int32_t t_cap, float* out_hidden_d, void* workspace_d, size_t workspace_bytes,
                             void* stream) {
    return decode_step_impl(cfg, w, ids_d, inputs_embeds_d, pos_d, kv_cache_d, B, t_cap, out_hidden_d, workspace_d, workspace_bytes,
                            stream, false);
}

static size_t greedy_pool_floats(const r4d_gpt2_config* cfg) {
    const size_t a = decode_skinny_floats(cfg->n_embd);
    const size_t b = gemm_skinny_supported(1, cfg->n_embd, cfg->vocab) ? gemm_skinny_scratch_floats(cfg->n_embd, cfg->vocab) : 0;
    return a > b ? a : b;
}

size_t r4d_gpt2_greedy_workspace_bytes(const r4d_gpt2_config* cfg, int32_t B) {
    if (!cfg || B <= 0) return 0;
    return carve(nullptr, (size_t)B, 0, greedy_pool_floats(cfg), cfg->n_embd).bytes;
}

int r4d_gpt2_greedy_step_f32(const r4d_gpt2_config* cfg, const r4d_gpt2_weights* w, const r4d_greedy_state* st,
                             float* kv_cache_d, int32_t B, int32_t t_cap, void* workspace_d, size_t workspace_bytes,
                             void* stream) {
    hipStream_t s = (hipStream_t)stream;
    int rc = check_cfg(cfg);
    if (rc) return rc;
    R4D_REQUIRE(w && w->wte && st && st->last_d && st->logits_d, "gpt2 greedy: null pointer");
    R4D_REQUIRE(B >= 1 && t_cap >= 1, "gpt2 greedy: B=%d t_cap=%d", B, t_cap);
    const int d = cfg->n_embd, V = cfg->vocab;
    Workspace ws = carve(workspace_d, (size_t)B, 0, greedy_pool_floats(cfg), d);
    if (!workspace_d || workspace_bytes < ws.bytes) {
        set_error("gpt2 greedy: workspace %zu bytes < required %zu", workspace_bytes, ws.bytes);
        return R4D_ERR_WORKSPACE;
    }
    const float* head = w->lm_head ? w->lm_head : w->wte;
    if (B <= 32 && gemm_skinny_supported(B, d, V))
        rc = launch_gemm_skinny(st->last_d, head, nullptr, nullptr, B, d, V, EPI_NONE, st->logits_d, ws.pool, s);
    else
        rc = r4d_lm_logits_f32(st->last_d, head, B, V, d, st->logits_d, stream);
    if (rc) return rc;
    GreedyState g;
    g.next = st->next_d; g.lens = st->lens_d; g.pos = st->pos_d; g.active = st->active_d; g.gen_len = st->gen_len_d;
    g.out_tokens = st->out_tokens_d; g.params = st->params_d; g.out_cap = st->out_cap; g.t_cap = t_cap;
    GreedyEmbed ge;
    ge.wte = w->wte; ge.wpe = w->wpe; ge.x_out = ws.x; ge.vocab = cfg->vocab; ge.n_positions = cfg->n_positions; ge.d = d;
    size_t cbytes = 0;
    void* cnt = ws.pool ? gemm_skinny_counters(ws.pool, &cbytes) : nullptr;
    ge.zero_words = (unsigned*)cnt; ge.n_zero = (int)(cbytes / 4);
    if ((rc = launch_greedy_advance(st->logits_d, B, V, g, s, &ge))) return rc;
    return decode_step_impl(cfg, w, st->next_d, nullptr, st->pos_d, kv_cache_d, B, t_cap, st->last_d, workspace_d, workspace_bytes,
                            stream, true);
}

struct r4d_decode_graph { hipGraph_t graph; hipGraphExec_t exec; };

int r4d_gpt2_greedy_graph_create(const r4d_gpt2_config* cfg, const r4d_gpt2_weights* w, const r4d_greedy_state* st,
                                 float* kv_cache_d, int32_t B, int32_t t_cap, void* workspace_d, size_t workspace_bytes,
                                 r4d_decode_graph** out_graph) {
    R4D_REQUIRE(out_graph, "gpt2 greedy graph: null out_graph");
    *out_graph = nullptr;
    R4D_REQUIRE(!g_prof_on, "gpt2 greedy graph: switch the launch profiler off before capturing");
    hipStream_t cap = nullptr;
    R4D_HIP(hipStreamCreateWithFlags(&cap, hipStreamNonBlocking));
    hipError_t e = hipStreamBeginCapture(cap, hipStreamCaptureModeRelaxed);
    if (e != hipSuccess) {
        (void)hipStreamDestroy(cap);
        set_error("gpt2 greedy graph: begin capture: %s", hipGetErrorString(e));
        return R4D_ERR_HIP;
    }
    const int rc = r4d_gpt2_greedy_step_f32(cfg, w, st, kv_cache_d, B, t_cap, workspace_d, workspace_bytes, cap);
    hipGraph_t graph = nullptr;
    e = hipStreamEndCapture(cap, &graph);
    (void)hipStreamDestroy(cap);
    if (rc) {
        if (graph) (void)hipGraphDestroy(graph);
        return rc;
    }
    if (e != hipSuccess || !graph) {
        set_error("gpt2 greedy graph: end capture: %s", hipGetErrorString(e));
        return R4D_ERR_HIP;
    }
    hipGraphExec_t exec = nullptr;
    e = hipGraphInstantiate(&exec, graph, nullptr, nullptr, 0);
    if (e != hipSuccess) {
        (void)hipGraphDestroy(graph);
        set_error("gpt2 greedy graph: instantiate: %s", hipGetErrorString(e));
        return R4D_ERR_HIP;
    }
    *out_graph = new r4d_decode_graph{graph, exec};
    return R4D_OK;
}

int r4d_decode_graph_launch(r4d_decode_graph* graph, int32_t n_steps, void* stream) {
    R4D_REQUIRE(graph && graph->exec && n_steps >= 0, "decode graph: null graph or n_steps=%d", n_steps);
    for (int i = 0; i < n_steps; ++i) R4D_HIP(hipGraphLaunch(graph->exec, (hipStream_t)stream));
    return R4D_OK;
}

void r4d_decode_graph_destroy(r4d_decode_graph* graph) {
    if (!graph) return;
    if (graph->exec) (void)hipGraphExecDestroy(graph->exec);
    if (graph->graph) (void)hipGraphDestroy(graph->graph);
    delete graph;
}

int r4d_lm_logits_f32(const float* hidden_d, const float* wte_d, int32_t M, int32_t V, int32_t d, float* logits_d,
                      void* stream) {
    R4D_REQUIRE(hidden_d && wte_d && logits_d, "lm_logits: null pointer");
    GemmArgs g;
    memset(&g, 0, sizeof(g));
    g.A = hidden_d; g.B = wte_d; g.C = logits_d;
    g.M = M; g.N = V; g.K = d; g.lda = d; g.ldb = d; g.ldc = V;
    g.b_trans = 1; g.b_rows = V; g.nbatch = 1; g.nb1 = 1; g.epilogue = EPI_NONE; g.scale_div = 1.f;
    return launch_gemm_f32(g, (hipStream_t)stream);
}

int r4d_layernorm_f32(const float* x_d, const float* w_d, const float* b_d, int32_t rows, int32_t d, float eps,
                      float* y_d, void* stream) {
    R4D_REQUIRE(x_d && w_d && b_d && y_d, "layernorm: null pointer");
    return launch_layernorm(x_d, w_d, b_d, rows, d, eps, y_d, (hipStream_t)stream);
}

int r4d_layernorm_lines_f32(const float* x_d, const float* w_d, const float* b_d, int32_t rows, int32_t d, float eps,
                            uint16_t* y_lines_d, void* stream) {
    R4D_REQUIRE(x_d && w_d && b_d && y_lines_d, "layernorm_lines: null pointer");
    return launch_layernorm_lines(x_d, w_d, b_d, rows, d, eps, y_lines_d, (hipStream_t)stream);
}

int r4d_conv1d_f32(const float* x_d, const float* w_d, const float* w_t_d, const float* bias_d, const float* residual_d,
                   int32_t M, int32_t K, int32_t N, int32_t epilogue, float* y_d, void* stream) {
    R4D_REQUIRE(x_d && w_d && y_d, "conv1d: null pointer");
    R4D_REQUIRE(epilogue >= 0 && epilogue <= 2, "conv1d: epilogue %d not in {0,1,2}", epilogue);
    R4D_REQUIRE(epilogue != EPI_RESIDUAL || residual_d, "conv1d: residual epilogue needs residual_d");
    return conv1d(x_d, w_d, w_t_d, bias_d, residual_d, M, K, N, epilogue, y_d, (hipStream_t)stream);
}

size_t r4d_attention_workspace_bytes(int32_t B, int32_t n_head, int32_t T) {
    if (B <= 0 || n_head <= 0 || T <= 0) return 0;
    return align_up((size_t)B * n_head * T * tpad(T) * sizeof(float), 256);
}

int r4d_attention_f32(const float* qkv_d, int32_t B, int32_t T, int32_t n_head, int32_t d, float* a_d,
                      void* scores_ws_d, size_t ws_bytes, void* stream) {
    R4D_REQUIRE(qkv_d && a_d && scores_ws_d, "attention: null pointer");
    R4D_REQUIRE(n_head >= 1 && d % n_head == 0 && (d / n_head) % 16 == 0, "attention: head_dim must be a multiple of 16");
    R4D_REQUIRE(T >= 1 && T <= 1024, "attention: T=%d out of range", T);
    if (ws_bytes < r4d_attention_workspace_bytes(B, n_head, T)) {
        set_error("attention: workspace too small");
        return R4D_ERR_WORKSPACE;
    }
    return attention(qkv_d, B, T, n_head, d, a_d, (float*)scores_ws_d, (hipStream_t)stream);
}

}
```

rag4dyg_amd/csrc/encoder_ops.hip:

```cpp
#include <string.h>
#include "common.h"
#include "h2.h"

namespace r4d {

constexpr int MAXV = 32;

__device__ __forceinline__ float wave_sum(float v) {
#pragma unroll
    for (int o = 32; o > 0; o >>= 1) v += __shfl_xor(v, o, 64);
    return v;
}
__device__ __forceinline__ float wave_max(float v) {
#pragma unroll
    for (int o = 32; o > 0; o >>= 1) v = fmaxf(v, __shfl_xor(v, o, 64));
    return v;
}

__device__ __forceinline__ void ln_row(float (&v)[MAXV], int nv, int d, float eps) {
    float s = 0.f;
#pragma unroll
    for (int i = 0; i < MAXV; ++i) if (i < nv) s += v[i];
    const float mean = wave_sum(s) / (float)d;
    float q = 0.f;
#pragma unroll
    for (int i = 0; i < MAXV; ++i) if (i < nv) { const float t = v[i] - mean; q += t * t; }
    const float rstd = rsqrtf(wave_sum(q) / (float)d + eps);
#pragma unroll
    for (int i = 0; i < MAXV; ++i) if (i < nv) v[i] = (v[i] - mean) * rstd;
}

__global__ __launch_bounds__(256) void ln_kernel(const float* __restrict__ x_in, int rows, int d, const float* __restrict__ w,
                                                 const float* __restrict__ b, float eps, float* __restrict__ y_out) {
    const int lane = threadIdx.x & 63;
    const int row = blockIdx.x * 4 + (threadIdx.x >> 6);
    if (row >= rows) return;
    const int nv = d >> 6;
    float v[MAXV];
#pragma unroll
    for (int i = 0; i < MAXV; ++i) if (i < nv) v[i] = x_in[(long long)row * d + lane + 64 * i];
    ln_row(v, nv, d, eps);
#pragma unroll
    for (int i = 0; i < MAXV; ++i)
        if (i < nv) y_out[(long long)row * d + lane + 64 * i] = v[i] * w[lane + 64 * i] + b[lane + 64 * i];
}

__device__ __forceinline__ void store_lines4(float* y_rows, long long row, int d, int col, float a0, float a1, float a2, float a3) {
    unsigned h0, l0, h1, l1;
    split2_pair<true>(a0, a1, h0, l0);
    split2_pair<true>(a2, a3, h1, l1);
    unsigned char* dst = reinterpret_cast<unsigned char*>(y_rows) + row * (long long)d * 4 + (col >> 5) * 128 + (col & 31) * 2;
    *reinterpret_cast<uint2*>(dst) = make_uint2(h0, h1);
    *reinterpret_cast<uint2*>(dst + 64) = make_uint2(l0, l1);
}

template <int NQ, bool LINES = false>
__global__ __launch_bounds__(256) void ln4_kernel(const float* __restrict__ x_in, int rows, int d, const float* __restrict__ w,
                                                  const float* __restrict__ b, float eps, float* __restrict__ y_out) {
    const int lane = threadIdx.x & 63;
    const int row = blockIdx.x * 4 + (threadIdx.x >> 6);
    if (row >= rows) return;
    const int nq = d >> 8;
    const float4* xr = reinterpret_cast<const float4*>(x_in + (long long)row * d) + lane;
    float4 v[NQ];
#pragma unroll
    for (int i = 0; i < NQ; ++i) v[i] = (i < nq) ? xr[64 * i] : make_float4(0.f, 0.f, 0.f, 0.f);
    float s_ = 0.f;
#pragma unroll
    for (int i = 0; i < NQ; ++i) s_ += (v[i].x + v[i].y) + (v[i].z + v[i].w);
    const float mean = wave_sum(s_) / (float)d;
    float q = 0.f;
#pragma unroll
    for (int i = 0; i < NQ; ++i)
        if (i < nq) {
            const float a0 = v[i].x - mean, a1 = v[i].y - mean, a2 = v[i].z - mean, a3 = v[i].w - mean;
            q += (a0 * a0 + a1 * a1) + (a2 * a2 + a3 * a3);
        }
    const float rstd = rsqrtf(wave_sum(q) / (float)d + eps);
    float4* yr = reinterpret_cast<float4*>(y_out + (long long)row * d) + lane;
#pragma unroll
    for (int i = 0; i < NQ; ++i)
        if (i < nq) {
            const float4 ww = reinterpret_cast<const float4*>(w)[lane + 64 * i], bb = reinterpret_cast<const float4*>(b)[lane + 64 * i];
            const float4 y4 = make_float4((v[i].x - mean) * rstd * ww.x + bb.x, (v[i].y - mean) * rstd * ww.y + bb.y,
                                          (v[i].z - mean) * rstd * ww.z + bb.z, (v[i].w - mean) * rstd * ww.w + bb.w);
            if constexpr (LINES) store_lines4(y_out, row, d, 4 * lane + 256 * i, y4.x, y4.y, y4.z, y4.w);
            else yr[64 * i] = y4;
        }
}

bool layernorm_lines_supported(int d) { return d % 256 == 0 && d <= 64 * MAXV; }
int launch_layernorm_lines(const float* x, const float* w, const float* b, int rows, int d, float eps, unsigned short* y_lines, hipStream_t s) {
    R4D_REQUIRE(layernorm_lines_supported(d) && (((uintptr_t)x | (uintptr_t)y_lines | (uintptr_t)w | (uintptr_t)b) & 15) == 0,
                "layernorm_lines: d=%d must be a multiple of 256 and the pointers 16-byte aligned", d);
    if (rows <= 0) return R4D_OK;
    ProfScope prof(PK_LAYERNORM, 8.0 * rows * d, s);
    float* y = reinterpret_cast<float*>(y_lines);
    if (d <= 512) { R4D_BRANCH(LN4_2); hipLaunchKernelGGL((ln4_kernel<2, true>), dim3(cdiv(rows, 4)), dim3(256), 0, s, x, rows, d, w, b, eps, y); }
    else if (d <= 1024) { R4D_BRANCH(LN4_4); hipLaunchKernelGGL((ln4_kernel<4, true>), dim3(cdiv(rows, 4)), dim3(256), 0, s, x, rows, d, w, b, eps, y); }
    else { R4D_BRANCH(LN4_8); hipLaunchKernelGGL((ln4_kernel<8, true>), dim3(cdiv(rows, 4)), dim3(256), 0, s, x, rows, d, w, b, eps, y); }
    R4D_CHECK_LAUNCH("layernorm_lines");
    return R4D_OK;
}

int launch_layernorm(const float* x, const float* w, const float* b, int rows, int d, float eps, float* y,
                     hipStream_t s) {
    R4D_REQUIRE(d % 64 == 0 && d <= 64 * MAXV, "layernorm: d=%d must be a multiple of 64 and <= %d", d, 64 * MAXV);
    if (rows <= 0) return R4D_OK;
    ProfScope prof(PK_LAYERNORM, 8.0 * rows * d, s);
    const bool vec = d % 256 == 0 && (((uintptr_t)x | (uintptr_t)y | (uintptr_t)w | (uintptr_t)b) & 15) == 0;
    if (vec && d <= 512) R4D_BRANCH(LN4_2); else if (vec && d <= 1024) R4D_BRANCH(LN4_4); else if (vec) R4D_BRANCH(LN4_8); else R4D_BRANCH(LN_GENERIC);
    if (vec && d <= 512) hipLaunchKernelGGL(ln4_kernel<2>, dim3(cdiv(rows, 4)), dim3(256), 0, s, x, rows, d, w, b, eps, y);
    else if (vec && d <= 1024) hipLaunchKernelGGL(ln4_kernel<4>, dim3(cdiv(rows, 4)), dim3(256), 0, s, x, rows, d, w, b, eps, y);
    else if (vec) hipLaunchKernelGGL(ln4_kernel<8>, dim3(cdiv(rows, 4)), dim3(256), 0, s, x, rows, d, w, b, eps, y);
    else
    hipLaunchKernelGGL(ln_kernel, dim3(cdiv(rows, 4)), dim3(256), 0, s, x, rows, d, w, b, eps, y);
    R4D_CHECK_LAUNCH("layernorm");
    return R4D_OK;
}

struct RowTable {
    int n;
    int T[ATT_MAXG];
    int seq_prefix[ATT_MAXG + 1];
    long long row_prefix[ATT_MAXG + 1];
    long long part_prefix[ATT_MAXG + 1];
    __device__ __forceinline__ long long row0_of(int g, int bidx) const { return row_prefix[g] + (long long)bidx * T[g]; }
};
struct RowInputs { const int64_t* ids[ATT_MAXG]; const float* emb[ATT_MAXG]; };

static RowTable make_table(const RowGroups& G) {
    RowTable t;
    t.n = G.n;
    t.seq_prefix[0] = 0; t.row_prefix[0] = 0; t.part_prefix[0] = 0;
    for (int g = 0; g < ATT_MAXG; ++g) {
        const int B = g < G.n ? G.B[g] : 0, T = g < G.n ? G.T[g] : 0;
        t.T[g] = T;
        t.seq_prefix[g + 1] = t.seq_prefix[g] + B;
        t.row_prefix[g + 1] = t.row_prefix[g] + (long long)B * T;
        t.part_prefix[g + 1] = t.part_prefix[g] + (long long)B * cdiv(T > 0 ? T : 1, LNF_ROWS_PER_CHUNK) * (B > 0);
    }
    return t;
}

__global__ __launch_bounds__(256) void embed_ln_groups_kernel(const RowTable G, const RowInputs in,
                                                              const float* __restrict__ wte, const float* __restrict__ wpe,
                                                              int vocab, int d, const float* __restrict__ w,
                                                              const float* __restrict__ b, float eps,
                                                              float* __restrict__ x_out, float* __restrict__ y_out) {
    const int lane = threadIdx.x & 63;
    const long long row = (long long)blockIdx.x * 4 + (threadIdx.x >> 6);
    if (row >= G.row_prefix[G.n]) return;
    int g = 0;
    while (g + 1 < G.n && row >= G.row_prefix[g + 1]) ++g;
    const long long local = row - G.row_prefix[g];
    const int nv = d >> 6;
    float v[MAXV];
    const float* src;
    bool bad = false;
    if (in.ids[g]) {
        const long long id = in.ids[g][local];
        bad = id < 0 || id >= vocab;
        src = wte + (bad ? 0 : id) * (long long)d;
    } else {
        src = in.emb[g] + local * d;
    }
    const float* pe = wpe + (local % G.T[g]) * d;
#pragma unroll
    for (int i = 0; i < MAXV; ++i)
        if (i < nv) {
            const float e = src[lane + 64 * i] + pe[lane + 64 * i];
            v[i] = bad ? __builtin_nanf("") : e;
            x_out[row * d + lane + 64 * i] = v[i];
        }
    ln_row(v, nv, d, eps);
#pragma unroll
    for (int i = 0; i < MAXV; ++i)
        if (i < nv) y_out[row * d + lane + 64 * i] = v[i] * w[lane + 64 * i] + b[lane + 64 * i];
}

template <int NQ, bool LINES = false>
__global__ __launch_bounds__(256) void embed_ln4_groups_kernel(const RowTable G, const RowInputs in,
                                                               const float* __restrict__ wte, const float* __restrict__ wpe,
                                                               int vocab, int d, const float* __restrict__ w,
                                                               const float* __restrict__ b, float eps,
                                                               float* __restrict__ x_out, float* __restrict__ y_out) {
    const int lane = threadIdx.x & 63;
    const long long row = (long long)blockIdx.x * 4 + (threadIdx.x >> 6);
    if (row >= G.row_prefix[G.n]) return;
    int g = 0;
    while (g + 1 < G.n && row >= G.row_prefix[g + 1]) ++g;
    const long long local = row - G.row_prefix[g];
    const int nq = d >> 8;
    const float* src;
    bool bad = false;
    if (in.ids[g]) {
        const long long id = in.ids[g][local];
        bad = id < 0 || id >= vocab;
        src = wte + (bad ? 0 : id) * (long long)d;
    } else {
        src = in.emb[g] + local * d;
    }
    const float4* s4 = reinterpret_cast<const float4*>(src) + lane;
    const float4* p4 = reinterpret_cast<const float4*>(wpe + (local % G.T[g]) * d) + lane;
    float4* xr = reinterpret_cast<float4*>(x_out + row * d) + lane;
    float4 v[NQ];
#pragma unroll
    for (int i = 0; i < NQ; ++i) {
        v[i] = make_float4(0.f, 0.f, 0.f, 0.f);
        if (i < nq) {
            const float4 e = s4[64 * i], q = p4[64 * i];
            const float nan = __builtin_nanf("");
            v[i] = bad ? make_float4(nan, nan, nan, nan) : make_float4(e.x + q.x, e.y + q.y, e.z + q.z, e.w + q.w);
            xr[64 * i] = v[i];
        }
    }
    float s_ = 0.f;
#pragma unroll
    for (int i = 0; i < NQ; ++i) s_ += (v[i].x + v[i].y) + (v[i].z + v[i].w);
    const float mean = wave_sum(s_) / (float)d;
    float q = 0.f;
#pragma unroll
    for (int i = 0; i < NQ; ++i)
        if (i < nq) {
            const float a0 = v[i].x - mean, a1 = v[i].y - mean, a2 = v[i].z - mean, a3 = v[i].w - mean;
            q += (a0 * a0 + a1 * a1) + (a2 * a2 + a3 * a3);
        }
    const float rstd = rsqrtf(wave_sum(q) / (float)d + eps);
    float4* yr = reinterpret_cast<float4*>(y_out + row * d) + lane;
#pragma unroll
    for (int i = 0; i < NQ; ++i)
        if (i < nq) {
            const float4 ww = reinterpret_cast<const float4*>(w)[lane + 64 * i], bb = reinterpret_cast<const float4*>(b)[lane + 64 * i];
            const float4 y4 = make_float4((v[i].x - mean) * rstd * ww.x + bb.x, (v[i].y - mean) * rstd * ww.y + bb.y,
                                          (v[i].z - mean) * rstd * ww.z + bb.z, (v[i].w - mean) * rstd * ww.w + bb.w);
            if constexpr (LINES) store_lines4(y_out, row, d, 4 * lane + 256 * i, y4.x, y4.y, y4.z, y4.w);
            else yr[64 * i] = y4;
        }
}

int launch_embed_layernorm_groups(const RowGroups& G, const float* wte, const float* wpe, int vocab, int d,
                                  const float* w, const float* b, float eps, float* x_out, float* y_out, hipStream_t s, bool y_lines) {
    R4D_REQUIRE(d % 64 == 0 && d <= 64 * MAXV, "embed: d=%d must be a multiple of 64 and <= %d", d, 64 * MAXV);
    R4D_REQUIRE(G.n >= 1 && G.n <= ATT_MAXG, "embed: %d batches per launch (max %d)", G.n, ATT_MAXG);
    const RowTable t = make_table(G);
    const long long rows = t.row_prefix[G.n];
    if (rows <= 0) return R4D_OK;
    RowInputs in;
    for (int g = 0; g < ATT_MAXG; ++g) { in.ids[g] = g < G.n ? G.ids[g] : nullptr; in.emb[g] = g < G.n ? G.emb[g] : nullptr; }
    ProfScope prof(PK_EMBED_LN, 12.0 * rows * d + 8.0 * rows, s);
    uintptr_t align = (uintptr_t)wte | (uintptr_t)wpe | (uintptr_t)w | (uintptr_t)b | (uintptr_t)x_out | (uintptr_t)y_out;
    for (int g = 0; g < G.n; ++g) align |= (uintptr_t)in.emb[g];
    const bool vec = d % 256 == 0 && (align & 15) == 0;
    const dim3 grid((unsigned)cdiv(rows, 4));
    if (y_lines) {
        R4D_REQUIRE(vec, "embed: line output needs d %% 256 == 0 and 16-byte aligned pointers");
        R4D_BRANCH(EMBED_LN4);
        if (d <= 512) hipLaunchKernelGGL((embed_ln4_groups_kernel<2, true>), grid, dim3(256), 0, s, t, in, wte, wpe, vocab, d, w, b, eps, x_out, y_out);
        else if (d <= 1024) hipLaunchKernelGGL((embed_ln4_groups_kernel<4, true>), grid, dim3(256), 0, s, t, in, wte, wpe, vocab, d, w, b, eps, x_out, y_out);
        else hipLaunchKernelGGL((embed_ln4_groups_kernel<8, true>), grid, dim3(256), 0, s, t, in, wte, wpe, vocab, d, w, b, eps, x_out, y_out);
        R4D_CHECK_LAUNCH("embed_layernorm");
        return R4D_OK;
    }
    if (vec && d <= 512) { R4D_BRANCH(EMBED_LN4); hipLaunchKernelGGL(embed_ln4_groups_kernel<2>, grid, dim3(256), 0, s, t, in, wte, wpe, vocab, d, w, b, eps, x_out, y_out); }
    else if (vec && d <= 1024) { R4D_BRANCH(EMBED_LN4); hipLaunchKernelGGL(embed_ln4_groups_kernel<4>, grid, dim3(256), 0, s, t, in, wte, wpe, vocab, d, w, b, eps, x_out, y_out); }
    else if (vec) { R4D_BRANCH(EMBED_LN4); hipLaunchKernelGGL(embed_ln4_groups_kernel<8>, grid, dim3(256), 0, s, t, in, wte, wpe, vocab, d, w, b, eps, x_out, y_out); }
    else {
        R4D_BRANCH(EMBED_GENERIC);
        hipLaunchKernelGGL(embed_ln_groups_kernel, grid, dim3(256), 0, s, t, in, wte, wpe, vocab, d, w, b, eps, x_out, y_out);
    }
    R4D_CHECK_LAUNCH("embed_layernorm");
    return R4D_OK;
}

__global__ __launch_bounds__(256) void embed_pos_ln_kernel(const int64_t* __restrict__ ids, const float* __restrict__ emb,
                                                           const int32_t* __restrict__ pos, const float* __restrict__ wte,
                                                           const float* __restrict__ wpe, int vocab, int n_positions,
                                                           int t_cap, int B, int d, const float* __restrict__ w,
                                                           const float* __restrict__ b, float eps,
                                                           float* __restrict__ x_out, float* __restrict__ y_out,
                                                           unsigned* __restrict__ zero_words, int n_zero) {
    if (blockIdx.x == 0)
        for (int i = threadIdx.x; i < n_zero; i += 256) zero_words[i] = 0u;
    const int lane = threadIdx.x & 63;
    const int row = blockIdx.x * 4 + (threadIdx.x >> 6);
    if (row >= B) return;
    const int nv = d >> 6;
    const int p = pos[row];
    bool bad = p < 0 || p >= n_positions || p >= t_cap;
    const float* src;
    if (ids) {
        const long long id = ids[row];
        bad = bad || id < 0 || id >= vocab;
        src = wte + (bad ? 0 : id) * (long long)d;
    } else {
        src = emb + (long long)row * d;
    }
    const float* pe = wpe + (long long)(bad ? 0 : p) * d;
    float v[MAXV];
#pragma unroll
    for (int i = 0; i < MAXV; ++i)
        if (i < nv) {
            const float e = src[lane + 64 * i] + pe[lane + 64 * i];
            v[i] = bad ? __builtin_nanf("") : e;
            x_out[(long long)row * d + lane + 64 * i] = v[i];
        }
    ln_row(v, nv, d, eps);
#pragma unroll
    for (int i = 0; i < MAXV; ++i)
        if (i < nv) y_out[(long long)row * d + lane + 64 * i] = v[i] * w[lane + 64 * i] + b[lane + 64 * i];
}

int launch_embed_pos_layernorm(const int64_t* ids, const float* emb, const int32_t* pos, const float* wte,
                               const float* wpe, int vocab, int n_positions, int t_cap, int B, int d, const float* w,
                               const float* b, float eps, float* x_out, float* y_out, hipStream_t s, void* zero_words,
                               size_t zero_bytes) {
    R4D_REQUIRE(d % 64 == 0 && d <= 64 * MAXV, "embed: d=%d must be a multiple of 64 and <= %d", d, 64 * MAXV);
    if (B <= 0) return R4D_OK;
    ProfScope prof(PK_EMBED_LN, 12.0 * B * d + 12.0 * B, s);
    hipLaunchKernelGGL(embed_pos_ln_kernel, dim3(cdiv(B, 4)), dim3(256), 0, s, ids, emb, pos, wte, wpe, vocab,
                       n_positions, t_cap, B, d, w, b, eps, x_out, y_out, (unsigned*)zero_words, (int)(zero_bytes / 4));
    R4D_CHECK_LAUNCH("embed_pos_layernorm");
    return R4D_OK;
}

template <int GL>
__global__ __launch_bounds__(512) void decode_attn_kernel(const float* __restrict__ qkv_new, float* __restrict__ kv,
                                                          const int32_t* __restrict__ pos, int t_cap, int H, int d,
                                                          float* __restrict__ out) {
    constexpr int NGRP = 512 / GL, U = 8;
    __shared__ float4 pacc[NGRP][GL];
    __shared__ float pm[NGRP], pl[NGRP];
    const int h = blockIdx.x, b = blockIdx.y;
    const int hd = d / H;
    const int tid = threadIdx.x, grp = tid / GL, gl = tid % GL;
    const bool on = 4 * gl < hd;
    const int p = pos[b];
    if (p < 0 || p >= t_cap) {
        for (int c = tid; c < hd; c += 512) out[(long long)b * d + h * hd + c] = __builtin_nanf("");
        return;
    }
    typedef unsigned int u32x4d __attribute__((ext_vector_type(4)));
    typedef float f32x4d __attribute__((ext_vector_type(4)));
    const float4 z4 = make_float4(0.f, 0.f, 0.f, 0.f);
    float* kvb = kv + (long long)b * t_cap * 2 * d + h * hd;
    const float* nq = qkv_new + (long long)b * 3 * d + h * hd;
    const int glc = min(gl, hd / 4 - 1);
    float4 q4 = reinterpret_cast<const float4*>(nq)[glc];
    if (!on) q4 = z4;
    const float scale = sqrtf((float)hd);
    float m = -INFINITY, l = 0.f;
    float4 acc = z4;
    auto group_sum = [](float v) {
#pragma unroll
        for (int o = GL / 2; o >= 1; o >>= 1) v += __shfl_xor(v, o);
        return v;
    };
    if (grp == 0) {
        const float4 k4 = reinterpret_cast<const float4*>(nq + d)[glc];
        const float4 v4 = reinterpret_cast<const float4*>(nq + 2 * d)[glc];
        reinterpret_cast<float4*>(kvb + (long long)p * 2 * d)[glc] = k4;
        reinterpret_cast<float4*>(kvb + (long long)p * 2 * d + d)[glc] = v4;
        m = group_sum((k4.x * q4.x + k4.y * q4.y) + (k4.z * q4.z + k4.w * q4.w)) / scale;
        l = 1.f;
        acc = v4;
    }
    const unsigned row_bytes = 2u * d * 4u;
    const __amdgpu_buffer_rsrc_t k_rsrc = __builtin_amdgcn_make_buffer_rsrc(kvb, 0, (unsigned)t_cap * row_bytes - h * hd * 4u, 0x00020000);
    const unsigned v_off = (unsigned)d * 4u + 16u * glc;
    for (int t0 = 0; t0 < p; t0 += NGRP * U) {
        u32x4d kr[U], vr[U];
#pragma unroll
        for (int u = 0; u < U; ++u) {
            const unsigned ro = (unsigned)min(t0 + u * NGRP + grp, p - 1) * row_bytes;
            kr[u] = __builtin_amdgcn_raw_buffer_load_b128(k_rsrc, ro + 16u * glc, 0, 0);
            vr[u] = __builtin_amdgcn_raw_buffer_load_b128(k_rsrc, ro + v_off, 0, 0);
        }
        float sv[U];
        float mn = m;
#pragma unroll
        for (int u = 0; u < U; ++u) {
            const f32x4d k4 = __builtin_bit_cast(f32x4d, kr[u]);
            const float dot = group_sum((k4.x * q4.x + k4.y * q4.y) + (k4.z * q4.z + k4.w * q4.w)) / scale;
            sv[u] = (t0 + u * NGRP + grp < p) ? dot : -INFINITY;
            mn = fmaxf(mn, sv[u]);
        }
        if (mn != -INFINITY) {
            const float corr = __expf(m - mn);
            l *= corr; acc.x *= corr; acc.y *= corr; acc.z *= corr; acc.w *= corr;
#pragma unroll
            for (int u = 0; u < U; ++u) {
                const f32x4d v4 = __builtin_bit_cast(f32x4d, vr[u]);
                const float e = __expf(sv[u] - mn);
                l += e;
                acc.x += e * v4.x; acc.y += e * v4.y; acc.z += e * v4.z; acc.w += e * v4.w;
            }
            m = mn;
        }
    }
    pacc[grp][gl] = acc;
    if (gl == 0) { pm[grp] = m; pl[grp] = l; }
    __syncthreads();
    if (grp == 0 && on) {
        float M = pm[0];
#pragma unroll
        for (int g = 1; g < NGRP; ++g) M = fmaxf(M, pm[g]);
        float L = 0.f;
        float4 o = z4;
#pragma unroll
        for (int g = 0; g < NGRP; ++g) {
            const float w = __expf(pm[g] - M);
            const float4 a = pacc[g][gl];
            L += pl[g] * w;
            o.x += a.x * w; o.y += a.y * w; o.z += a.z * w; o.w += a.w * w;
        }
        o.x /= L; o.y /= L; o.z /= L; o.w /= L;
        reinterpret_cast<float4*>(out + (long long)b * d + h * hd)[gl] = o;
    }
}

int launch_decode_attention(const float* qkv_new, float* kv_layer, const int32_t* pos, int B, int t_cap, int H, int d,
                            float* out, hipStream_t s) {
    const int hd = d / H;
    R4D_REQUIRE(hd * H == d && hd % 4 == 0 && hd <= 256, "decode attention: head_dim=%d (multiple of 4, max 256)", hd);
    R4D_REQUIRE(d % 4 == 0 && t_cap >= 1 && (size_t)t_cap * 2 * d * 4 < ((size_t)1 << 31),
                "decode attention: d=%d t_cap=%d (a sequence's cache must stay below 2 GB)", d, t_cap);
    if (B <= 0) return R4D_OK;
    ProfScope prof(PK_DECODE_ATTN, 16.0 * B * d, s);
    if (hd <= 128) R4D_BRANCH(DEC_ATT_32); else R4D_BRANCH(DEC_ATT_64);
    if (hd <= 128) hipLaunchKernelGGL(decode_attn_kernel<32>, dim3(H, B), dim3(512), 0, s, qkv_new, kv_layer, pos, t_cap, H, d, out);
    else hipLaunchKernelGGL(decode_attn_kernel<64>, dim3(H, B), dim3(512), 0, s, qkv_new, kv_layer, pos, t_cap, H, d, out);
    R4D_CHECK_LAUNCH("decode_attention");
    return R4D_OK;
}

__global__ __launch_bounds__(256) void greedy_advance_kernel(const float* __restrict__ logits, int V, GreedyState st,
                                                             GreedyEmbed emb) {
    __shared__ float sv[4];
    __shared__ int si[4];
    __shared__ int s_next, s_pos;
    const int b = blockIdx.x, tid = threadIdx.x, lane = tid & 63, wid = tid >> 6;
    if (b == 0)
        for (int i = tid; i < emb.n_zero; i += 256) emb.zero_words[i] = 0u;
    const float* row = logits + (long long)b * V;
    float best = -INFINITY;
    int bi = 0x7fffffff;
    for (int j = tid; j < V; j += 256) {
        const float v = row[j];
        if (v > best || bi == 0x7fffffff) { best = v; bi = j; }
    }
#pragma unroll
    for (int o = 32; o >= 1; o >>= 1) {
        const float ov = __shfl_xor(best, o);
        const int oi = __shfl_xor(bi, o);
        if (ov > best || (ov == best && oi < bi)) { best = ov; bi = oi; }
    }
    if (lane == 0) { sv[wid] = best; si[wid] = bi; }
    __syncthreads();
    if (tid == 0) {
        for (int w = 1; w < 4; ++w)
            if (sv[w] > best || (sv[w] == best && si[w] < bi)) { best = sv[w]; bi = si[w]; }
        int a = st.active[b];
        const int len = st.lens[b];
        if (a) {
            int g = st.gen_len[b];
            if (g < st.out_cap) st.out_tokens[(long long)b * st.out_cap + g] = bi;
            ++g;
            st.gen_len[b] = g;
            const int max_gen = st.params[0], len_limit = min(st.params[1], st.t_cap), n_eos = min(st.params[2], 4);
            bool stop = g >= max_gen || g >= st.out_cap || len + 1 >= len_limit;
            for (int e = 0; e < n_eos; ++e) stop |= bi == st.params[3 + e];
            if (stop) a = 0;
            st.active[b] = a;
        }
        st.next[b] = bi;
        st.pos[b] = a ? len : 0;
        st.lens[b] = len + a;
        s_next = bi; s_pos = a ? len : 0;
    }
    if (!emb.x_out) return;
    __syncthreads();
    const int id = s_next, p = s_pos;
    const bool bad = p < 0 || p >= emb.n_positions || p >= st.t_cap || id < 0 || id >= emb.vocab;
    const float* src = emb.wte + (long long)(bad ? 0 : id) * emb.d;
    const float* pe = emb.wpe + (long long)(bad ? 0 : p) * emb.d;
    for (int c = tid; c < emb.d; c += 256) emb.x_out[(long long)b * emb.d + c] = bad ? __builtin_nanf("") : src[c] + pe[c];
}

int launch_greedy_advance(const float* logits, int B, int V, const GreedyState& st, hipStream_t s, const GreedyEmbed* embed) {
    R4D_REQUIRE(logits && st.next && st.lens && st.pos && st.active && st.gen_len && st.out_tokens && st.params,
                "greedy advance: null pointer");
    R4D_REQUIRE(V >= 1 && st.out_cap >= 1 && st.t_cap >= 1, "greedy advance: V=%d out_cap=%d t_cap=%d", V, st.out_cap, st.t_cap);
    if (B <= 0) return R4D_OK;
    ProfScope prof(PK_GREEDY_ADVANCE, 4.0 * B * (double)V, s);
    GreedyEmbed e;
    memset(&e, 0, sizeof(e));
    if (embed) {
        e = *embed;
        R4D_REQUIRE(e.wte && e.wpe && e.x_out && e.d >= 1, "greedy advance: bad embedding arguments");
    }
    hipLaunchKernelGGL(greedy_advance_kernel, dim3(B), dim3(256), 0, s, logits, V, st, e);
    R4D_CHECK_LAUNCH("greedy_advance");
    return R4D_OK;
}

__global__ __launch_bounds__(256) void causal_softmax_kernel(float* __restrict__ S, int nrows_total, int T, int ld,
                                                             int row_tile) {
    const int lane = threadIdx.x & 63;
    const long long gr = (long long)blockIdx.x * 4 + (threadIdx.x >> 6);
    if (gr >= nrows_total) return;
    const int i = (int)(gr % T);
    float* row = S + (gr / T) * (long long)T * ld + (long long)i * ld;
    const int n = i + 1;
    float v[16];
    float m = -INFINITY;
#pragma unroll
    for (int c = 0; c < 16; ++c) {
        const int j = lane + 64 * c;
        v[c] = (j < n) ? row[j] : -INFINITY;
        m = fmaxf(m, v[c]);
    }
    m = wave_max(m);
    float s = 0.f;
#pragma unroll
    for (int c = 0; c < 16; ++c) {
        v[c] = (lane + 64 * c < n) ? expf(v[c] - m) : 0.f;
        s += v[c];
    }
    s = wave_sum(s);
    const int nfill = min(ld, (n + row_tile - 1) / row_tile * row_tile);
#pragma unroll
    for (int c = 0; c < 16; ++c) {
        const int j = lane + 64 * c;
        if (j < nfill) row[j] = v[c] / s;
    }
}

int launch_causal_softmax(float* S, int nbh, int T, int ld, int row_tile, hipStream_t s) {
    R4D_REQUIRE(T <= 1024, "attention: T=%d exceeds n_positions cap 1024", T);
    const long long rows = (long long)nbh * T;
    ProfScope prof(PK_SOFTMAX, 4.0 * nbh * T * (double)(T + 1), s);
    hipLaunchKernelGGL(causal_softmax_kernel, dim3((unsigned)((rows + 3) / 4)), dim3(256), 0, s, S, (int)rows, T, ld,
                       row_tile);
    R4D_CHECK_LAUNCH("causal_softmax");
    return R4D_OK;
}

template <int NV>
__global__ __launch_bounds__(256) void lnf_partial_kernel(const RowTable G, const float* __restrict__ x,
                                                          const float* __restrict__ w, const float* __restrict__ b, int d,
                                                          float eps, float* __restrict__ hidden_out,
                                                          float* __restrict__ partial, unsigned* __restrict__ range_flag) {
    extern __shared__ float red[];
    const int lane = threadIdx.x & 63, wid = threadIdx.x >> 6;
    const int chunk = blockIdx.x, seq = blockIdx.y;
    int g = 0;
    while (g + 1 < G.n && seq >= G.seq_prefix[g + 1]) ++g;
    const int T = G.T[g], S = (T + LNF_ROWS_PER_CHUNK - 1) / LNF_ROWS_PER_CHUNK;
    if (chunk >= S) return;
    const int bidx = seq - G.seq_prefix[g];
    const long long row0 = G.row0_of(g, bidx);
    const int nv = d >> 6;
    const int t0 = chunk * LNF_ROWS_PER_CHUNK, t1 = min(T, t0 + LNF_ROWS_PER_CHUNK);
    constexpr int RPW = LNF_ROWS_PER_CHUNK / 4;
    float v[RPW][NV];
#pragma unroll
    for (int r = 0; r < RPW; ++r) {
        const int t = min(t0 + wid + 4 * r, T - 1);
#pragma unroll
        for (int i = 0; i < NV; ++i) v[r][i] = (i < nv) ? x[(row0 + t) * d + lane + 64 * i] : 0.f;
    }
    float acc[NV];
#pragma unroll
    for (int i = 0; i < NV; ++i) acc[i] = 0.f;
#pragma unroll
    for (int r = 0; r < RPW; ++r) {
        const int t = t0 + wid + 4 * r;
        float s_ = 0.f;
#pragma unroll
        for (int i = 0; i < NV; ++i) s_ += v[r][i];
        const float mean = wave_sum(s_) / (float)d;
        float q = 0.f;
#pragma unroll
        for (int i = 0; i < NV; ++i) if (i < nv) { const float c = v[r][i] - mean; q += c * c; }
        const float rstd = rsqrtf(wave_sum(q) / (float)d + eps);
        if (range_flag && t < t1 && !(rstd > 0.f) && lane == 0) atomicOr(range_flag, R4D_RANGE_NONFINITE_HIDDEN);
        if (t < t1) {
            const long long base = (row0 + t) * d;
#pragma unroll
            for (int i = 0; i < NV; ++i)
                if (i < nv) {
                    const float y = (v[r][i] - mean) * rstd * w[lane + 64 * i] + b[lane + 64 * i];
                    if (hidden_out) hidden_out[base + lane + 64 * i] = y;
                    acc[i] += y;
                }
        }
    }
    if (!partial) return;
#pragma unroll
    for (int i = 0; i < NV; ++i) if (i < nv) red[wid * d + lane + 64 * i] = acc[i];
    __syncthreads();
    const long long prow = G.part_prefix[g] + (long long)bidx * S + chunk;
    for (int c = threadIdx.x; c < d; c += 256)
        partial[prow * d + c] = (red[c] + red[d + c]) + (red[2 * d + c] + red[3 * d + c]);
}

__global__ __launch_bounds__(256) void meanpool_reduce_kernel(const RowTable G, const float* __restrict__ partial, int d,
                                                              float* __restrict__ pool_out) {
    const int seq = blockIdx.x;
    int g = 0;
    while (g + 1 < G.n && seq >= G.seq_prefix[g + 1]) ++g;
    const int T = G.T[g], S = (T + LNF_ROWS_PER_CHUNK - 1) / LNF_ROWS_PER_CHUNK;
    const long long prow = G.part_prefix[g] + (long long)(seq - G.seq_prefix[g]) * S;
    for (int c = threadIdx.x; c < d; c += 256) {
        float s = 0.f;
        for (int k = 0; k < S; ++k) s += partial[(prow + k) * d + c];
        pool_out[(long long)seq * d + c] = s / (float)T;
    }
}

size_t lnf_meanpool_scratch_floats(int B, int T, int d) { return (size_t)B * cdiv(T, LNF_ROWS_PER_CHUNK) * d; }

unsigned* g_range_flag = nullptr;

int launch_lnf_meanpool_groups(const RowGroups& G, const float* x, const float* w, const float* b, int d, float eps,
                               float* hidden_out, float* pool_out, float* scratch, hipStream_t s) {
    R4D_REQUIRE(d % 64 == 0 && d <= 64 * MAXV, "ln_f: d=%d must be a multiple of 64 and <= %d", d, 64 * MAXV);
    R4D_REQUIRE(!pool_out || scratch, "ln_f: mean-pool needs scratch");
    R4D_REQUIRE(G.n >= 1 && G.n <= ATT_MAXG, "ln_f: %d batches per launch (max %d)", G.n, ATT_MAXG);
    const RowTable t = make_table(G);
    const int nseq = t.seq_prefix[G.n];
    const long long rows = t.row_prefix[G.n], parts = t.part_prefix[G.n];
    if (nseq <= 0 || rows <= 0) return R4D_OK;
    R4D_REQUIRE(nseq <= 65535, "ln_f: %d sequences per launch exceed the grid limit", nseq);
    int Tmax = 0;
    for (int g = 0; g < G.n; ++g) Tmax = G.T[g] > Tmax ? G.T[g] : Tmax;
    {
        ProfScope prof(PK_LNF_MEANPOOL, 4.0 * rows * d * (hidden_out ? 2 : 1) + 4.0 * parts * d, s);
        const dim3 grid(cdiv(Tmax, LNF_ROWS_PER_CHUNK), nseq);
        float* part = pool_out ? scratch : nullptr;
        if (d <= 512) R4D_BRANCH(LNF_8); else if (d <= 1024) R4D_BRANCH(LNF_16); else R4D_BRANCH(LNF_32);
        if (d <= 512) hipLaunchKernelGGL(lnf_partial_kernel<8>, grid, dim3(256), 4 * d * sizeof(float), s, t, x, w, b, d, eps, hidden_out, part, g_range_flag);
        else if (d <= 1024) hipLaunchKernelGGL(lnf_partial_kernel<16>, grid, dim3(256), 4 * d * sizeof(float), s, t, x, w, b, d, eps, hidden_out, part, g_range_flag);
        else hipLaunchKernelGGL(lnf_partial_kernel<32>, grid, dim3(256), 4 * d * sizeof(float), s, t, x, w, b, d, eps, hidden_out, part, g_range_flag);
        R4D_CHECK_LAUNCH("lnf_partial");
    }
    if (pool_out) {
        ProfScope prof(PK_MEANPOOL_REDUCE, 4.0 * parts * d + 4.0 * nseq * d, s);
        hipLaunchKernelGGL(meanpool_reduce_kernel, dim3(nseq), dim3(256), 0, s, t, scratch, d, pool_out);
        R4D_CHECK_LAUNCH("meanpool_reduce");
    }
    return R4D_OK;
}

}
```

rag4dyg_amd/csrc/gemm_h2p.hip:

```cpp
#include <stdlib.h>
#include <string.h>
#include "common.h"
#include "h2.h"

namespace r4d {

typedef float f32x16p __attribute__((ext_vector_type(16)));
typedef float f32x2p __attribute__((ext_vector_type(2)));
typedef unsigned int u32x4p __attribute__((ext_vector_type(4)));
typedef _Float16 f16x8p __attribute__((ext_vector_type(8)));

int g_gemm_h2p = 1;

__device__ __forceinline__ f32x2p gelu_new_h2p(f32x2p x) {
    const float k0 = -2.0f * 0.7978845608028654f * 1.4426950408889634f, k1 = 0.044715f * k0;
    const f32x2p a = x * x * k1 + k0;
    const f32x2p w = x * a;
    f32x2p e;
    e.x = __builtin_amdgcn_exp2f(w.x); e.y = __builtin_amdgcn_exp2f(w.y);
    e = e + 1.0f;
    f32x2p r;
    r.x = __builtin_amdgcn_rcpf(e.x); r.y = __builtin_amdgcn_rcpf(e.y);
    return x * r;
}
__device__ __forceinline__ float gelu_new_h2p_1(float x) {
    const float k0 = -2.0f * 0.7978845608028654f * 1.4426950408889634f, k1 = 0.044715f * k0;
    return x * __builtin_amdgcn_rcpf(1.0f + __builtin_amdgcn_exp2f(x * __builtin_fmaf(x * x, k1, k0)));
}

struct H2PShape {
    int M, N, K, ldc, ldr;
    unsigned* kblk; int kb_hd;
};

__device__ __forceinline__ void h2p_dma2(const void* base, unsigned v0, unsigned v1, unsigned lds_dst) {
    unsigned keep;
    asm volatile("s_mov_b32 %0, m0\n\ts_mov_b32 m0, %4\n\ts_nop 0\n\t"
                 "global_load_lds_dwordx4 %1, %3\n\t"
                 "global_load_lds_dwordx4 %2, %3 offset:1024\n\t"
                 "s_mov_b32 m0, %0"
                 : "=&s"(keep) : "v"(v0), "v"(v1), "s"(base), "s"(lds_dst) : "memory");
}
__device__ __forceinline__ void h2p_dma4(const void* base, unsigned v0, unsigned v1, unsigned v2, unsigned v3, unsigned lds_dst) {
    unsigned keep;
    asm volatile("s_mov_b32 %0, m0\n\ts_mov_b32 m0, %6\n\ts_nop 0\n\t"
                 "global_load_lds_dwordx4 %1, %5\n\t"
                 "global_load_lds_dwordx4 %2, %5 offset:1024\n\t"
                 "global_load_lds_dwordx4 %3, %5 offset:2048\n\t"
                 "global_load_lds_dwordx4 %4, %5 offset:3072\n\t"
                 "s_mov_b32 m0, %0"
                 : "=&s"(keep) : "v"(v0), "v"(v1), "v"(v2), "v"(v3), "s"(base), "s"(lds_dst) : "memory");
}
template <int N_> __device__ __forceinline__ void h2p_wait_vm() { asm volatile("s_waitcnt vmcnt(%0)" :: "n"(N_) : "memory"); }

template <int BM, int BN, int EPI, bool OUT_LINES, int WGM = 2, int WGN = 4>
__global__ __launch_bounds__(64 * WGM * WGN, (WGM * WGN) / 4) void gemm_h2p_kernel(const unsigned short* __restrict__ Al, const unsigned short* __restrict__ Bp,
                                                          float* __restrict__ Cg, const float* __restrict__ biasg,
                                                          const float* __restrict__ residg, const H2PShape g) {
    constexpr int NW = WGM * WGN;
    constexpr int WM = BM / WGM, WN = BN / WGN, TM = WM / 32, TN = WN / 32;
    constexpr int STAGE = (BM + BN) * 8;
    constexpr int NBUF = 3;
    constexpr int NGA = BM / 8 / NW, NGB = BN / 8 / NW;
    constexpr int NDMA = NGA + NGB;
    static_assert(BM == 128 && (BN == 256 || BN == 128) && TM >= 1 && TN >= 1 && (NGA == 2 || NGA == 4) && (NGB == 2 || NGB == 4 || NGB == 8), "tile");
    __shared__ u32x4p lds[NBUF * STAGE];

    const int nblk = gridDim.x, xq = nblk >> 3, xr = nblk & 7, xcd = blockIdx.x & 7;
    const int bid = xcd * xq + min(xcd, xr) + (blockIdx.x >> 3);
    constexpr int GROUP_M = 8;
    const int tiles_m = (g.M + BM - 1) / BM, tiles_n = (g.N + BN - 1) / BN;
    const int per_group = GROUP_M * tiles_n;
    const int grp = bid / per_group, first_m = grp * GROUP_M;
    const int gsz = min(tiles_m - first_m, GROUP_M);
    const int tile_m = first_m + (bid % per_group) % gsz, tile_n = (bid % per_group) / gsz;
    const int m0 = tile_m * BM, n0 = tile_n * BN;
    const int nkt = g.K / 32;

    const int tid = threadIdx.x, lane = tid & 63, wid = tid >> 6;
    const int wm = wid / WGN, wn = wid % WGN;
    const int li = lane & 31, lh = lane >> 5;

    unsigned va[NGA], vb[NGB];
    const int lrow = lane >> 3, lslot = lane & 7;
#pragma unroll
    for (int i = 0; i < NGA; ++i) {
        const int r = (wid * NGA + i) * 8 + lrow;
        va[i] = (unsigned)min(m0 + r, g.M - 1) * (unsigned)(g.K * 4) + 16u * (unsigned)(lslot ^ ((r >> 1) & 7)) + 3072u - 1024u * (i & 3);
    }
#pragma unroll
    for (int i = 0; i < NGB; ++i) {
        const int r = (wid * NGB + i) * 8 + lrow;
        vb[i] = (unsigned)min(n0 + r, g.N - 1) * (unsigned)(g.K * 4) + 16u * (unsigned)(lslot ^ ((r >> 1) & 7)) + 3072u - 1024u * (i & 3);
    }
    const unsigned lds0 = __builtin_amdgcn_readfirstlane((unsigned)(size_t)lds);
    const unsigned wid_s = __builtin_amdgcn_readfirstlane((unsigned)wid);
    const unsigned dst_a = lds0 + (wid_s * NGA) * 1024u, dst_b = lds0 + ((unsigned)(BM / 8) + wid_s * NGB) * 1024u;
    const char* abase = reinterpret_cast<const char*>(Al) - 3072;
    const char* bbase = reinterpret_cast<const char*>(Bp) - 3072;
#define H2P_ISSUE(KT, STG)                                                                         \
    {                                                                                              \
        const unsigned so_ = (unsigned)(STG) * (unsigned)(STAGE * 16);                             \
        if constexpr (NGA == 4) h2p_dma4(abase + (size_t)(KT) * 128, va[0], va[1], va[2], va[3], dst_a + so_); \
        else h2p_dma2(abase + (size_t)(KT) * 128, va[0], va[1], dst_a + so_);                      \
        if constexpr (NGB == 8) {                                                                  \
            h2p_dma4(bbase + (size_t)(KT) * 128, vb[0], vb[1], vb[2], vb[3], dst_b + so_);          \
            h2p_dma4(bbase + (size_t)(KT) * 128, vb[4], vb[5], vb[6], vb[7], dst_b + so_ + 4096u);   \
        } else if constexpr (NGB == 4) h2p_dma4(bbase + (size_t)(KT) * 128, vb[0], vb[1], vb[2], vb[3], dst_b + so_); \
        else h2p_dma2(bbase + (size_t)(KT) * 128, vb[0], vb[1], dst_b + so_);                       \
    }

    const int fsw = (li >> 1) & 7;
    int f_off[2][2];
#pragma unroll
    for (int s_ = 0; s_ < 2; ++s_)
#pragma unroll
        for (int p = 0; p < 2; ++p) f_off[s_][p] = li * 8 + ((4 * p + 2 * s_ + lh) ^ fsw);
    const int fa_base = wm * WM * 8, fb_base = BM * 8 + wn * WN * 8;

    f32x16p acc0[TM][TN], acc1[TM][TN];
#pragma unroll
    for (int i = 0; i < TM; ++i)
#pragma unroll
        for (int j = 0; j < TN; ++j)
#pragma unroll
            for (int r = 0; r < 16; ++r) { acc0[i][j][r] = 0.f; acc1[i][j][r] = 0.f; }

#define H2P_MFMA(ACC, A_, B_, I_, J_) \
    ACC[I_][J_] = __builtin_amdgcn_mfma_f32_32x32x16_f16(__builtin_bit_cast(f16x8p, A_), __builtin_bit_cast(f16x8p, B_), ACC[I_][J_], 0, 0, 0);
    u32x4p fa[2][TM][2], fb[2][TN][2];
#define H2P_FRAGS(SET, STG, S)                                                                     \
    {                                                                                              \
        const u32x4p* st_ = lds + (STG) * STAGE;                                                   \
                                        \
        _Pragma("unroll") for (int i = 0; i < TM; ++i) fa[SET][i][1] = st_[fa_base + i * 256 + f_off[S][1]]; \
        _Pragma("unroll") for (int j = 0; j < TN; ++j) fb[SET][j][0] = st_[fb_base + j * 256 + f_off[S][0]]; \
        _Pragma("unroll") for (int i = 0; i < TM; ++i) fa[SET][i][0] = st_[fa_base + i * 256 + f_off[S][0]]; \
        _Pragma("unroll") for (int j = 0; j < TN; ++j) fb[SET][j][1] = st_[fb_base + j * 256 + f_off[S][1]]; \
    }
#define H2P_MFMAS(SET)                                                                             \
    {                                                                                              \
        _Pragma("unroll") for (int i = 0; i < TM; ++i) _Pragma("unroll") for (int j = 0; j < TN; ++j) H2P_MFMA(acc1, fa[SET][i][1], fb[SET][j][0], i, j) \
        _Pragma("unroll") for (int i = 0; i < TM; ++i) _Pragma("unroll") for (int j = 0; j < TN; ++j) H2P_MFMA(acc0, fa[SET][i][0], fb[SET][j][0], i, j) \
        _Pragma("unroll") for (int i = 0; i < TM; ++i) _Pragma("unroll") for (int j = 0; j < TN; ++j) H2P_MFMA(acc1, fa[SET][i][0], fb[SET][j][1], i, j) \
    }

    H2P_ISSUE(0, 0)
    if (nkt > 1) { H2P_ISSUE(1, 1) h2p_wait_vm<NDMA>(); } else { h2p_wait_vm<0>(); }
    __syncthreads();
    H2P_FRAGS(0, 0, 0)

    constexpr int NMF = 3 * TM * TN, NFR = 2 * (TM + TN);
    static_assert(NMF >= NFR, "interleave");
#define H2P_ITER(CUR, NXT, WR)                                                                     \
    {                                                                                              \
        __builtin_amdgcn_sched_barrier(0);                                                         \
        const bool more_ = kt + 2 < nkt;                                                           \
        if (more_) H2P_ISSUE(kt + 2, WR)                                                           \
        H2P_FRAGS(1, CUR, 1)                                                                       \
        H2P_MFMAS(0)                                                                               \
        _Pragma("unroll") for (int m_ = 0; m_ < NMF; ++m_) {                                       \
            __builtin_amdgcn_sched_group_barrier(0x008, 1, 0);                                     \
            if (m_ < NFR) __builtin_amdgcn_sched_group_barrier(0x100, 1, 0);                       \
        }                                                                                          \
        __builtin_amdgcn_sched_barrier(0);                                                         \
        if (more_) h2p_wait_vm<NDMA>(); else h2p_wait_vm<0>();                                     \
        asm volatile("s_waitcnt lgkmcnt(0)\n\ts_barrier" ::: "memory");                            \
        H2P_FRAGS(0, NXT, 0)                                                                       \
        H2P_MFMAS(1)                                                                               \
        _Pragma("unroll") for (int m_ = 0; m_ < NMF; ++m_) {                                       \
            __builtin_amdgcn_sched_group_barrier(0x008, 1, 0);                                     \
            if (m_ < NFR) __builtin_amdgcn_sched_group_barrier(0x100, 1, 0);                       \
        }                                                                                          \
        __builtin_amdgcn_sched_barrier(0);                                                         \
    }
    int kt = 0;
    for (; kt + 2 < nkt; kt += 3) {
        H2P_ITER(0, 1, 2)
        { ++kt; H2P_ITER(1, 2, 0) }
        { ++kt; H2P_ITER(2, 0, 1) }
        kt -= 2;
    }
    if (kt < nkt) {
        H2P_ITER(0, 1, 2)
        if (kt + 1 < nkt) { ++kt; H2P_ITER(1, 2, 0) }
    }
#undef H2P_ITER
#undef H2P_FRAGS
#undef H2P_MFMAS
#undef H2P_MFMA
#undef H2P_ISSUE

    constexpr float UNS = H2_A_UNSCALE;
    float* __restrict__ C = Cg;
    const bool interior = (m0 + BM <= g.M) & (n0 + BN <= g.N);
    if constexpr (OUT_LINES) {
        static_assert(EPI == EPI_GELU, "line output: the c_fc epilogue only");
        unsigned char* __restrict__ L = reinterpret_cast<unsigned char*>(Cg);
        const long long row_bytes = (long long)g.N * 4;
        const bool odd = li & 1;
#pragma unroll
        for (int j = 0; j < TN; ++j) {
            const int colb = n0 + wn * WN + j * 32;
            const bool col_ok = colb + li < g.N;
            const float bias = (biasg && col_ok) ? biasg[colb + li] : 0.f;
#pragma unroll
            for (int i = 0; i < TM; ++i) {
#pragma unroll
                for (int r2 = 0; r2 < 16; r2 += 2) {
                    f32x2p v2 = {__builtin_fmaf(acc1[i][j][r2], H2_LO_UNSCALE, acc0[i][j][r2]) * UNS + bias,
                                 __builtin_fmaf(acc1[i][j][r2 + 1], H2_LO_UNSCALE, acc0[i][j][r2 + 1]) * UNS + bias};
                    v2 = gelu_new_h2p(v2);
                    const float vx = v2.x, vy = v2.y;
                    const float send = odd ? vx : vy;
                    const float recv = __builtin_bit_cast(float, __builtin_amdgcn_mov_dpp(__builtin_bit_cast(int, send), 0xB1, 0xF, 0xF, true));
                    const float c0 = odd ? recv : vx, c1 = odd ? vy : recv;
                    unsigned h, l;
                    split2_pair<true>(c0, c1, h, l);
                    const int r = r2 + (odd ? 1 : 0);
                    const int row = m0 + wm * WM + i * 32 + (r & 3) + 8 * (r >> 2) + 4 * lh;
                    if (interior || (row < g.M && col_ok)) {
                        unsigned* dst = reinterpret_cast<unsigned*>(L + (long long)row * row_bytes + (long long)(colb >> 5) * 128 + (li >> 1) * 4);
                        dst[0] = h;
                        dst[16] = l;
                    }
                }
            }
        }
        return;
    } else {
        if (interior) {
            const int lane_c = ((wm * WM + 4 * lh) * g.ldc + wn * WN + li) * 4;
            const int lane_r = ((wm * WM + 4 * lh) * g.ldr + wn * WN + li) * 4;
            const __amdgpu_buffer_rsrc_t c_rsrc = __builtin_amdgcn_make_buffer_rsrc(
                C + (long long)m0 * g.ldc + n0, 0, ((BM - 1) * g.ldc + BN) * 4, 0x00020000);
            const __amdgpu_buffer_rsrc_t r_rsrc = __builtin_amdgcn_make_buffer_rsrc(
                const_cast<float*>(EPI == EPI_RESIDUAL ? residg + (long long)m0 * g.ldr + n0 : Cg), 0,
                EPI == EPI_RESIDUAL ? ((BM - 1) * g.ldr + BN) * 4 : 0, 0x00020000);
            const int kd = g.N / 3;
            const __amdgpu_buffer_rsrc_t kb_rsrc = __builtin_amdgcn_make_buffer_rsrc(
                (EPI == EPI_H2WORDS && g.kb_hd) ? g.kblk : reinterpret_cast<unsigned*>(Cg), 0,
                (EPI == EPI_H2WORDS && g.kb_hd) ? ((g.M + 31) / 32) * (kd * 128) : 0, 0x00020000);
            const int lane_kb = (li >> 3) * 1024 + ((li >> 2) & 1) * 512 + ((li & 3) + 4 * lh) * 16;
#pragma unroll
            for (int j = 0; j < TN; ++j) {
                const float bias = biasg ? biasg[n0 + wn * WN + j * 32 + li] : 0.f;
                const int colb = n0 + wn * WN + j * 32;
                const bool to_kb = EPI == EPI_H2WORDS && g.kb_hd && colb >= kd && colb < 2 * kd;
                const int kb_chunk = to_kb ? ((colb - kd) / g.kb_hd) * (g.kb_hd / 8) + ((colb - kd) % g.kb_hd) / 8 : 0;
#pragma unroll
                for (int i = 0; i < TM; ++i) {
                    const int kb_soff = (((m0 + wm * WM + i * 32) >> 5) * (kd / 8) + kb_chunk) * 1024;
                    float res[16];
                    if (EPI == EPI_RESIDUAL) {
#pragma unroll
                        for (int r = 0; r < 16; ++r)
                            res[r] = __builtin_bit_cast(float, __builtin_amdgcn_raw_buffer_load_b32(
                                r_rsrc, lane_r, ((i * 32 + (r & 3) + 8 * (r >> 2)) * g.ldr + j * 32) * 4, 0));
                    }
                    unsigned o[16];
#pragma unroll
                    for (int r2 = 0; r2 < 16; r2 += 2) {
                        f32x2p v2 = {__builtin_fmaf(acc1[i][j][r2], H2_LO_UNSCALE, acc0[i][j][r2]) * UNS + bias,
                                     __builtin_fmaf(acc1[i][j][r2 + 1], H2_LO_UNSCALE, acc0[i][j][r2 + 1]) * UNS + bias};
                        if (EPI == EPI_GELU) v2 = gelu_new_h2p(v2);
                        else if (EPI == EPI_RESIDUAL) { v2.x += res[r2]; v2.y += res[r2 + 1]; }
                        const float vx = v2.x, vy = v2.y;
                        o[r2] = __builtin_bit_cast(unsigned int, vx); o[r2 + 1] = __builtin_bit_cast(unsigned int, vy);
                        if (EPI == EPI_H2WORDS) h2_words<true>(v2.x, v2.y, o[r2], o[r2 + 1]);
                    }
                    if (EPI == EPI_H2WORDS && to_kb) {
                        const bool o1 = li & 1, o2 = li & 2;
#pragma unroll
                        for (int a4 = 0; a4 < 16; a4 += 4) {
                            unsigned x0 = o[a4], x1 = o[a4 + 1], x2 = o[a4 + 2], x3 = o[a4 + 3];
                            {
                                const unsigned s01 = o1 ? x0 : x1, s23 = o1 ? x2 : x3;
                                const unsigned r01 = (unsigned)__builtin_amdgcn_mov_dpp((int)s01, 0xB1, 0xF, 0xF, true);
                                const unsigned r23 = (unsigned)__builtin_amdgcn_mov_dpp((int)s23, 0xB1, 0xF, 0xF, true);
                                if (o1) { x0 = r01; x2 = r23; } else { x1 = r01; x3 = r23; }
                            }
                            {
                                const unsigned s02 = o2 ? x0 : x2, s13 = o2 ? x1 : x3;
                                const unsigned r02 = (unsigned)__builtin_amdgcn_mov_dpp((int)s02, 0x4E, 0xF, 0xF, true);
                                const unsigned r13 = (unsigned)__builtin_amdgcn_mov_dpp((int)s13, 0x4E, 0xF, 0xF, true);
                                if (o2) { x0 = r02; x1 = r13; } else { x2 = r02; x3 = r13; }
                            }
                            const u32x4p slot = {x0, x1, x2, x3};
                            __builtin_amdgcn_raw_buffer_store_b128(slot, kb_rsrc, lane_kb, kb_soff + 2 * a4 * 16, 0);
                        }
                    } else {
#pragma unroll
                        for (int r = 0; r < 16; ++r)
                            __builtin_amdgcn_raw_buffer_store_b32(o[r], c_rsrc, lane_c, ((i * 32 + (r & 3) + 8 * (r >> 2)) * g.ldc + j * 32) * 4, 0);
                    }
                }
            }
            return;
        }
#pragma unroll
        for (int j = 0; j < TN; ++j) {
            const int col = n0 + wn * WN + j * 32 + li;
            const bool col_ok = col < g.N;
            const int colc = min(col, g.N - 1);
            const float bias = biasg ? biasg[colc] : 0.f;
#pragma unroll
            for (int i = 0; i < TM; ++i) {
#pragma unroll
                for (int r = 0; r < 16; ++r) {
                    const int row = m0 + wm * WM + i * 32 + (r & 3) + 8 * (r >> 2) + 4 * lh;
                    float v = __builtin_fmaf(acc1[i][j][r], H2_LO_UNSCALE, acc0[i][j][r]) * UNS + bias;
                    if (EPI == EPI_GELU) v = gelu_new_h2p_1(v);
                    else if (EPI == EPI_RESIDUAL) v += residg[(long long)min(row, g.M - 1) * g.ldr + colc];
                    else if (EPI == EPI_H2WORDS) { unsigned w0, w1; h2_words<true>(v, 0.f, w0, w1); v = __builtin_bit_cast(float, w0); }
                    if (EPI == EPI_H2WORDS && g.kb_hd && col >= g.N / 3 && col < 2 * (g.N / 3)) {
                        const int kd = g.N / 3, e = (col - kd) % g.kb_hd, chunk = ((col - kd) / g.kb_hd) * (g.kb_hd / 8) + (e >> 3);
                        if (row < g.M)
                            g.kblk[((long long)(row >> 5) * (kd / 8) + chunk) * 256 + (((e >> 2) & 1) * 32 + (row & 31)) * 4 + (e & 3)] =
                                __builtin_bit_cast(unsigned, v);
                        continue;
                    }
                    if (row < g.M && col_ok) C[(long long)row * g.ldc + col] = v;
                }
            }
        }
    }
}

__global__ __launch_bounds__(256) void split2_lines_kernel(const float* __restrict__ x, long long n4, uint2* __restrict__ lines, int K) {
    const long long i = (long long)blockIdx.x * 256 + threadIdx.x;
    if (i >= n4) return;
    const float4 v = reinterpret_cast<const float4*>(x)[i];
    unsigned h0, l0, h1, l1;
    split2_pair<true>(v.x, v.y, h0, l0);
    split2_pair<true>(v.z, v.w, h1, l1);
    const long long e = i * 4, row = e / K;
    const int k = (int)(e - row * K);
    unsigned char* dst = reinterpret_cast<unsigned char*>(lines) + row * (long long)K * 4 + (k >> 5) * 128 + (k & 31) * 2;
    *reinterpret_cast<uint2*>(dst) = make_uint2(h0, h1);
    *reinterpret_cast<uint2*>(dst + 64) = make_uint2(l0, l1);
}

bool gemm_h2p_supported(int M, int K, int N) {
    return g_gemm_h2p != 0 && gemm_h2_supported(M, K, N) && (long long)M * K * 4 + 4096 < (1ll << 32) && (long long)N * K * 4 + 4096 < (1ll << 32);
}

template <int BN>
static int launch_h2p(const S3Args& a, const unsigned short* a_lines, bool out_lines, int cls, hipStream_t stream) {
    const int tiles = cdiv(a.M, 128) * cdiv(a.N, BN);
    ProfScope prof(cls, 2.0 * (double)a.M * a.N * a.K, stream);
    H2PShape sh;
    sh.M = a.M; sh.N = a.N; sh.K = a.K; sh.ldc = a.ldc; sh.ldr = a.ldr;
    sh.kblk = a.kblk; sh.kb_hd = a.kblk ? a.kb_hd : 0;
#define H2P_LAUNCH_(E, OL) hipLaunchKernelGGL((gemm_h2p_kernel<128, BN, E, OL>), dim3(tiles), dim3(512), 0, stream, a_lines, a.planes, a.C, a.bias, a.resid, sh)
    if (out_lines) {
        if (a.epilogue != EPI_GELU) { set_error("gemm_h2p: line output exists for the GELU epilogue only"); return R4D_ERR_INVALID; }
        H2P_LAUNCH_(EPI_GELU, true);
    } else {
        switch (a.epilogue) {
            case EPI_NONE: H2P_LAUNCH_(EPI_NONE, false); break;
            case EPI_GELU: H2P_LAUNCH_(EPI_GELU, false); break;
            case EPI_RESIDUAL: H2P_LAUNCH_(EPI_RESIDUAL, false); break;
            case EPI_H2WORDS: H2P_LAUNCH_(EPI_H2WORDS, false); break;
            default: set_error("gemm_h2p: epilogue %d has no instantiation", a.epilogue); return R4D_ERR_INVALID;
        }
    }
#undef H2P_LAUNCH_
    R4D_CHECK_LAUNCH("gemm_h2p");
    return R4D_OK;
}

int launch_gemm_h2p(const S3Args& a, const unsigned short* a_lines, bool out_lines, hipStream_t stream) {
    R4D_REQUIRE(a_lines && a.planes && a.C, "gemm_h2p: null pointer");
    R4D_REQUIRE(gemm_h2p_supported(a.M, a.K, a.N), "gemm_h2p: unsupported shape M=%d K=%d N=%d", a.M, a.K, a.N);
    R4D_REQUIRE(((uintptr_t)a_lines % 16) == 0 && ((uintptr_t)a.planes % 16) == 0, "gemm_h2p: alignment");
    R4D_REQUIRE(!out_lines || a.N % 32 == 0, "gemm_h2p: line output needs N %% 32 == 0 (N = %d)", a.N);
    R4D_REQUIRE(a.epilogue != EPI_RESIDUAL || a.resid, "gemm_h2p: the residual epilogue needs the second buffer");
    R4D_REQUIRE(!a.kblk || (a.epilogue == EPI_H2WORDS && a.N % 3 == 0 && a.kb_hd >= 32 && a.kb_hd % 32 == 0 && (a.N / 3) % a.kb_hd == 0),
                "gemm_h2p: the key-blocked K image goes with the h2-word epilogue, N = 3 d and a head_dim that is a multiple of 32");
    const long long b0 = (long long)cdiv(a.M, 128) * cdiv(a.N, 256), b1 = (long long)cdiv(a.M, 128) * cdiv(a.N, 128);
    const double c0 = (double)((b0 + 255) / 256) * 128 * 256, c1 = (double)((b1 + 255) / 256) * 128 * 128 / 0.9;
    if (c1 < c0) { R4D_BRANCH(H2P_128x128); return launch_h2p<128>(a, a_lines, out_lines, PK_GEMM_H2_128x128, stream); }
    R4D_BRANCH(H2P_128x256);
    return launch_h2p<256>(a, a_lines, out_lines, PK_GEMM_H2_128x256, stream);
}

int launch_split2_lines(const float* x, long long rows, int K, unsigned short* lines, hipStream_t s) {
    R4D_REQUIRE(x && lines && rows >= 0 && K >= 32 && K % 32 == 0, "split2_lines: bad arguments (K %% 32 == 0 wanted)");
    R4D_REQUIRE((((uintptr_t)x | (uintptr_t)lines) & 15) == 0, "split2_lines: alignment");
    const long long n4 = rows * K / 4;
    if (n4 == 0) return R4D_OK;
    hipLaunchKernelGGL(split2_lines_kernel, dim3((unsigned)((n4 + 255) / 256)), dim3(256), 0, s, x, n4, reinterpret_cast<uint2*>(lines), K);
    R4D_CHECK_LAUNCH("split2_lines");
    return R4D_OK;
}

}

using namespace r4d;

extern "C" {

int r4d_set_gemm_h2p(int32_t on) {
    const int prev = g_gemm_h2p;
    g_gemm_h2p = on != 0;
    return prev;
}

int r4d_split2_lines_f16(const float* x_d, int64_t rows, int32_t K, uint16_t* lines_d, void* stream) {
    return launch_split2_lines(x_d, rows, K, lines_d, (hipStream_t)stream);
}

int r4d_conv1d_h2p_f32(const uint16_t* x_lines_d, const uint16_t* planes_d, const float* bias_d, const float* residual_d, int32_t M,
                       int32_t K, int32_t N, int32_t epilogue, int32_t out_lines, void* y_d, void* stream) {
    R4D_REQUIRE(epilogue >= 0 && epilogue <= 2, "conv1d_h2p: epilogue %d not in {0,1,2}", epilogue);
    S3Args a;
    memset(&a, 0, sizeof(a));
    a.planes = planes_d; a.C = (float*)y_d; a.bias = bias_d; a.resid = residual_d;
    a.M = M; a.N = N; a.K = K; a.lda = K; a.ldc = N; a.ldr = N; a.epilogue = epilogue;
    return launch_gemm_h2p(a, x_lines_d, out_lines != 0, (hipStream_t)stream);
}

}
```

rag4dyg_amd/ops.py:

```python
import torch

from . import _lib
from ._lib import check


def _stream():
    return torch.cuda.current_stream().cuda_stream


def _dev(t, dtype, name):
    if not isinstance(t, torch.Tensor) or not t.is_cuda:
        raise _lib.R4DError(f"{name}: expected a tensor on the GPU (no CPU fallback in rag4dyg_amd)")
    if t.dtype != dtype:
        raise _lib.R4DError(f"{name}: expected dtype {dtype}, got {t.dtype}")
    if not t.is_contiguous():
        raise _lib.R4DError(f"{name}: tensor must be contiguous")
    return t.data_ptr()


_WS = {}


def workspace(nbytes, device, tag="default"):
    key = (str(device), tag)
    buf = _WS.get(key)
    if buf is None or buf.numel() < nbytes:
        buf = torch.empty(max(int(nbytes), 256), dtype=torch.uint8, device=device)
        _WS[key] = buf
    return buf


def layernorm(x, w, b, eps=1e-5):
    d = x.shape[-1]
    y = torch.empty_like(x)
    rows = x.numel() // d
    check(_lib.load().r4d_layernorm_f32(_dev(x, torch.float32, "x"), _dev(w, torch.float32, "w"),
                                        _dev(b, torch.float32, "b"), rows, d, eps, y.data_ptr(), _stream()), "layernorm")
    return y


def conv1d(x, w, bias, epilogue="none", residual=None, w_t=None):
    K, N = w.shape
    M = x.numel() // K
    y = torch.empty(x.shape[:-1] + (N,), dtype=torch.float32, device=x.device)
    epi = {"none": 0, "gelu": 1, "residual": 2}[epilogue]
    rp = _dev(residual, torch.float32, "residual") if residual is not None else None
    bp = _dev(bias, torch.float32, "bias") if bias is not None else None
    tp = _dev(w_t, torch.float32, "w_t") if w_t is not None else None
    check(_lib.load().r4d_conv1d_f32(_dev(x, torch.float32, "x"), _dev(w, torch.float32, "w"), tp, bp, rp, M, K, N, epi,
                                     y.data_ptr(), _stream()), "conv1d")
    return y


_GEMM_MODES = {"f32": 0, "bf16x3": 1, "f16x2": 2}
_GEMM_MODE = None
DEFAULT_GEMM_MODE = "f16x2"


def gemm_mode():
    global _GEMM_MODE
    if _GEMM_MODE is None:
        import os
        m = os.environ.get("R4D_GEMM_MODE")
        if m is None:
            m = "f32" if os.environ.get("R4D_GEMM_SPLIT3", "1") == "0" else DEFAULT_GEMM_MODE
        set_gemm_mode(m)
    return _GEMM_MODE


_LAST_SPLIT_MODE = None


def set_gemm_mode(mode):
    global _GEMM_MODE, _LAST_SPLIT_MODE
    if mode not in _GEMM_MODES:
        raise ValueError(f"gemm mode {mode!r}: one of {sorted(_GEMM_MODES)}")
    _GEMM_MODE = mode
    if mode != "f32":
        _LAST_SPLIT_MODE = mode
    check(_lib.load().r4d_set_gemm_split3(_GEMM_MODES[mode]), "set_gemm_split3")


def gemm_split3_enabled():
    return gemm_mode() != "f32"


def set_gemm_split3(on):
    if not on:
        set_gemm_mode("f32")
    elif gemm_mode() == "f32":
        import os
        m = _LAST_SPLIT_MODE or os.environ.get("R4D_GEMM_MODE", DEFAULT_GEMM_MODE)
        set_gemm_mode(m if m != "f32" else DEFAULT_GEMM_MODE)


H2_MAX_WEIGHT = 6.0e4


def split2_planes(w, transposed=False):
    if transposed:
        N, K = w.shape
    else:
        K, N = w.shape
    amax = float(w.detach().abs().max())
    if not (amax < H2_MAX_WEIGHT):
        return None
    if K % 32:
        raise ValueError(f"split2_planes: K = {K} is not a multiple of 32")
    planes = torch.empty(N, K // 32, 2, 32, dtype=torch.int16, device=w.device)
    check(_lib.load().r4d_split2_planes_f16(_dev(w, torch.float32, "w"), K, N, int(bool(transposed)), planes.data_ptr(),
                                            _stream()), "split2_planes")
    return planes


def set_gemm_h2p(on):
    return bool(_lib.load().r4d_set_gemm_h2p(1 if on else 0))


def split2_lines(x):
    K = x.shape[-1]
    rows = x.numel() // K
    out = torch.empty(rows, K // 32, 2, 32, dtype=torch.int16, device=x.device)
    check(_lib.load().r4d_split2_lines_f16(_dev(x, torch.float32, "x"), rows, K, out.data_ptr(), _stream()), "split2_lines")
    return out


def layernorm_lines(x, w, b, eps=1e-5):
    d = x.shape[-1]
    rows = x.numel() // d
    y = torch.empty(rows, d // 32, 2, 32, dtype=torch.int16, device=x.device)
    check(_lib.load().r4d_layernorm_lines_f32(_dev(x, torch.float32, "x"), _dev(w, torch.float32, "w"), _dev(b, torch.float32, "b"),
                                              rows, d, eps, y.data_ptr(), _stream()), "layernorm_lines")
    return y


def conv1d_h2p(x_lines, planes, bias, epilogue="none", residual=None, out_lines=False):
    N, K = planes.shape[0], planes.shape[1] * 32
    M = x_lines.shape[0]
    epi = {"none": 0, "gelu": 1, "residual": 2}[epilogue]
    y = (torch.empty(M, N // 32, 2, 32, dtype=torch.int16, device=x_lines.device) if out_lines
         else torch.empty(M, N, dtype=torch.float32, device=x_lines.device))
    rp = _dev(residual, torch.float32, "residual") if residual is not None else None
    bp = _dev(bias, torch.float32, "bias") if bias is not None else None
    check(_lib.load().r4d_conv1d_h2p_f32(_dev(x_lines, torch.int16, "x_lines"), _dev(planes, torch.int16, "planes"), bp, rp, M, K, N, epi,
                                         int(bool(out_lines)), y.data_ptr(), _stream()), "conv1d_h2p")
    return y


def conv1d_h2(x, planes, bias, epilogue="none", residual=None):
    N, K = planes.shape[0], planes.shape[1] * 32
    M = x.numel() // K
    y = torch.empty(x.shape[:-1] + (N,), dtype=torch.float32, device=x.device)
    epi = {"none": 0, "gelu": 1, "residual": 2}[epilogue]
    rp = _dev(residual, torch.float32, "residual") if residual is not None else None
    bp = _dev(bias, torch.float32, "bias") if bias is not None else None
    check(_lib.load().r4d_conv1d_h2_f32(_dev(x, torch.float32, "x"), _dev(planes, torch.int16, "planes"), bp, rp, M, K, N, epi,
                                        y.data_ptr(), _stream()), "conv1d_h2")
    return y


def split3_planes(w, transposed=False):
    if transposed:
        N, K = w.shape
    else:
        K, N = w.shape
    planes = torch.empty(3, N, K, dtype=torch.int16, device=w.device)
    check(_lib.load().r4d_split3_planes_bf16(_dev(w, torch.float32, "w"), K, N, int(bool(transposed)), planes.data_ptr(),
                                             _stream()), "split3_planes")
    return planes


def fold_layernorm(wT, ln_w, ln_b):
    N, K = wT.shape
    wTg = torch.empty_like(wT)
    lnc = torch.empty(2, N, dtype=torch.float32, device=wT.device)
    check(_lib.load().r4d_fold_layernorm_f32(_dev(wT, torch.float32, "wT"), _dev(ln_w, torch.float32, "ln_w"),
                                             _dev(ln_b, torch.float32, "ln_b"), N, K, wTg.data_ptr(), lnc.data_ptr(), _stream()),
          "fold_layernorm")
    return wTg, lnc


def conv1d_s3(x, planes, bias, epilogue="none", residual=None):
    _, N, K = planes.shape
    M = x.numel() // K
    y = torch.empty(x.shape[:-1] + (N,), dtype=torch.float32, device=x.device)
    epi = {"none": 0, "gelu": 1, "residual": 2}[epilogue]
    rp = _dev(residual, torch.float32, "residual") if residual is not None else None
    bp = _dev(bias, torch.float32, "bias") if bias is not None else None
    check(_lib.load().r4d_conv1d_s3_f32(_dev(x, torch.float32, "x"), _dev(planes, torch.int16, "planes"), bp, rp, M, K, N, epi,
                                        y.data_ptr(), _stream()), "conv1d_s3")
    return y


def set_attention_fused(mode):
    _lib.load().r4d_set_attention_fused(-1 if mode is None or mode == -1 else (2 if mode == 2 else int(bool(mode))))


def set_attention_h2(on):
    return bool(_lib.load().r4d_set_attention_h2(int(bool(on))))


def set_attention_kblk(on):
    return bool(_lib.load().r4d_set_attention_kblk(int(bool(on))))


def pack_kblk_words(qkv_words, n_head):
    B, T, d3 = qkv_words.shape
    d = d3 // 3
    rows = B * T
    out = torch.empty((rows + 31) // 32 * 32 * d, dtype=torch.int32, device=qkv_words.device)
    check(_lib.load().r4d_pack_kblk_words(_dev(qkv_words, torch.int32, "qkv_words"), rows, n_head, d, out.data_ptr(), _stream()), "pack_kblk_words")
    return out


def attention_h2_kblk(qkv_words, kblk, n_head):
    B, T, d3 = qkv_words.shape
    d = d3 // 3
    a = torch.empty(B, T, d, dtype=torch.float32, device=qkv_words.device)
    check(_lib.load().r4d_attention_h2_kblk_f32(_dev(qkv_words, torch.int32, "qkv_words"), _dev(kblk, torch.int32, "kblk"), B, T, n_head, d,
                                                a.data_ptr(), _stream()), "attention_h2_kblk")
    return a


def pack_h2_words(x):
    x = x.contiguous()
    w = torch.empty(x.shape, dtype=torch.int32, device=x.device)
    check(_lib.load().r4d_pack_h2_words_f32(_dev(x, torch.float32, "x"), x.numel(), w.data_ptr(), _stream()), "pack_h2_words")
    return w


def attention_h2(qkv_words, n_head):
    B, T, d3 = qkv_words.shape
    d = d3 // 3
    a = torch.empty(B, T, d, dtype=torch.float32, device=qkv_words.device)
    check(_lib.load().r4d_attention_h2_f32(_dev(qkv_words, torch.int32, "qkv_words"), B, T, n_head, d, a.data_ptr(), _stream()),
          "attention_h2")
    return a


def attention(qkv, n_head):
    B, T, d3 = qkv.shape
    d = d3 // 3
    lib = _lib.load()
    nbytes = lib.r4d_attention_workspace_bytes(B, n_head, T)
    ws = workspace(nbytes, qkv.device, "attn")
    a = torch.empty(B, T, d, dtype=torch.float32, device=qkv.device)
    check(lib.r4d_attention_f32(_dev(qkv, torch.float32, "qkv"), B, T, n_head, d, a.data_ptr(), ws.data_ptr(),
                                ws.numel(), _stream()), "attention")
    return a


def lm_logits(hidden, wte):
    V, d = wte.shape
    M = hidden.numel() // d
    out = torch.empty(hidden.shape[:-1] + (V,), dtype=torch.float32, device=hidden.device)
    check(_lib.load().r4d_lm_logits_f32(_dev(hidden, torch.float32, "hidden"), _dev(wte, torch.float32, "wte"), M, V, d,
                                        out.data_ptr(), _stream()), "lm_logits")
    return out


RANGE_NONFINITE_HIDDEN, RANGE_BAD_NORM, RANGE_BAD_LABEL = 1, 2, 4
_RANGE_FLAG = None


def range_flag(device=None):
    global _RANGE_FLAG
    if _RANGE_FLAG is None:
        dev = device if device is not None else torch.device("cuda", torch.cuda.current_device())
        _RANGE_FLAG = torch.zeros(1, dtype=torch.int32, device=dev)
        check(_lib.load().r4d_set_range_flag(_RANGE_FLAG.data_ptr()), "set_range_flag")
    return _RANGE_FLAG


def take_range_flag():
    f = range_flag()
    v = int(f.item())
    if v:
        f.zero_()
    return v


def check_range(what):
    v = take_range_flag()
    if v:
        why = []
        if v & RANGE_NONFINITE_HIDDEN:
            why.append("a non-finite hidden state reached ln_f (an activation, q, k or v beyond the arithmetic's range: "
                       "|x| >= 2^18 in gemm mode 'f16x2'; 'bf16x3' and 'f32' have fp32's exponent range)")
        if v & RANGE_BAD_NORM:
            why.append("an embedding row could not be normalised (NaN, inf or zero norm)")
        if v & RANGE_BAD_LABEL:
            why.append("a token id outside [0, vocab) reached the LM cross entropy")
        raise _lib.R4DError(f"{what}: " + "; ".join(why) + " -- no ranking was produced from it")


def normalize_rows(x):
    n, d = x.shape
    range_flag(x.device)
    out = torch.empty_like(x)
    check(_lib.load().r4d_normalize_rows_f32(_dev(x, torch.float32, "x"), n, d, out.data_ptr(), _stream()),
          "normalize_rows")
    return out


SCORE_TOPK_MAX_QUERIES = 65535


def score_topk(q_hat, pool_hat, k, index_offset=0, want_scores=False):
    Q, d = q_hat.shape
    if Q > SCORE_TOPK_MAX_QUERIES:
        parts = [score_topk(q_hat[s:s + SCORE_TOPK_MAX_QUERIES].contiguous(), pool_hat, k, index_offset, want_scores)
                 for s in range(0, Q, SCORE_TOPK_MAX_QUERIES)]
        return (torch.cat([p[0] for p in parts]), torch.cat([p[1] for p in parts]),
                torch.cat([p[2] for p in parts]) if want_scores else None)
    N = pool_hat.shape[0]
    lib = _lib.load()
    ws = workspace(lib.r4d_score_topk_workspace_bytes(Q, N, k), q_hat.device, "score")
    vals = torch.empty(Q, k, dtype=torch.float32, device=q_hat.device)
    idx = torch.empty(Q, k, dtype=torch.int64, device=q_hat.device)
    scores = torch.empty(Q, N, dtype=torch.float32, device=q_hat.device) if want_scores else None
    check(lib.r4d_score_topk_f32(_dev(q_hat, torch.float32, "q_hat"), _dev(pool_hat, torch.float32, "pool_hat"), Q, N, d,
                                 k, int(index_offset), vals.data_ptr(), idx.data_ptr(),
                                 scores.data_ptr() if want_scores else None, ws.data_ptr(), ws.numel(), _stream()),
          "score_topk")
    return vals, idx, scores


def topk_f32(m, k):
    rows, n = m.shape
    lib = _lib.load()
    ws = workspace(lib.r4d_topk_f32_workspace_bytes(rows, n, k), m.device, "topk32")
    vals = torch.empty(rows, k, dtype=torch.float32, device=m.device)
    idx = torch.empty(rows, k, dtype=torch.int64, device=m.device)
    check(lib.r4d_topk_f32(_dev(m, torch.float32, "m"), rows, n, k, vals.data_ptr(), idx.data_ptr(), ws.data_ptr(),
                           ws.numel(), _stream()), "topk_f32")
    return vals, idx


def merge_topk(vals, idx):
    G, Q, k = vals.shape
    ov = torch.empty(Q, k, dtype=torch.float32, device=vals.device)
    oi = torch.empty(Q, k, dtype=torch.int64, device=vals.device)
    lib = _lib.load()
    ws = workspace(lib.r4d_merge_topk_workspace_bytes(G, Q, k), vals.device, "merge")
    check(lib.r4d_merge_topk_f32(_dev(vals, torch.float32, "vals"), _dev(idx, torch.int64, "idx"), G, Q, k,
                                 ov.data_ptr(), oi.data_ptr(), ws.data_ptr(), ws.numel(), _stream()), "merge_topk")
    return ov, oi


def argsort_desc(scores):
    rows, n = scores.shape
    perm = torch.empty(rows, n, dtype=torch.int32, device=scores.device)
    lib = _lib.load()
    f64 = scores.dtype == torch.float64
    fn = lib.r4d_argsort_desc_f64 if f64 else lib.r4d_argsort_desc_f32
    ptr = _dev(scores, torch.float64 if f64 else torch.float32, "scores")
    step = 65535
    for r0 in range(0, rows, step):
        nr = min(step, rows - r0)
        ws = workspace(lib.r4d_argsort_workspace_bytes(nr, n, 8 if f64 else 4), scores.device, "argsort")
        check(fn(ptr + r0 * n * scores.element_size(), nr, n, perm.data_ptr() + r0 * n * 4, ws.data_ptr(), ws.numel(),
                 _stream()), "argsort_desc")
    return perm


def jaccard(a_ptr, a_idx, b_ptr, b_idx, vocab, zero_diag=False, sort_rows=None, dense_split=None):
    na, nb = a_ptr.numel() - 1, b_ptr.numel() - 1
    out = torch.empty(na, nb, dtype=torch.float64, device=a_ptr.device)
    if a_idx.numel() == 0:
        a_idx = torch.zeros(1, dtype=torch.int32, device=a_ptr.device)
    if b_idx.numel() == 0:
        b_idx = torch.zeros(1, dtype=torch.int32, device=b_ptr.device)
    long_sets = a_idx.numel() > 4 * na
    if dense_split is None:
        dense_split = long_sets and na * nb >= 5_000_000
    if sort_rows is None:
        sort_rows = long_sets and na * nb >= 50_000_000
    lib = _lib.load()
    ws = None
    if dense_split or sort_rows:
        ws = workspace(lib.r4d_jaccard_prepared_workspace_bytes(na, a_idx.numel(), nb, b_idx.numel(), int(vocab)), a_ptr.device,
                       "jaccard")
    check(lib.r4d_jaccard_prepared_f64(_dev(a_ptr, torch.int32, "a_ptr"), _dev(a_idx, torch.int32, "a_idx"), na, a_idx.numel(),
                                       _dev(b_ptr, torch.int32, "b_ptr"), _dev(b_idx, torch.int32, "b_idx"), nb, b_idx.numel(),
                                       int(vocab), int(bool(zero_diag)), int(bool(dense_split)), int(bool(sort_rows)),
                                       out.data_ptr(), ws.data_ptr() if ws is not None else None, ws.numel() if ws is not None else 0,
                                       _stream()), "jaccard")
    return out


def topk_f64(m, k):
    rows, n = m.shape
    lib = _lib.load()
    ws = workspace(lib.r4d_topk_f64_workspace_bytes(rows, n, k), m.device, "topk64")
    vals = torch.empty(rows, k, dtype=torch.float64, device=m.device)
    idx = torch.empty(rows, k, dtype=torch.int32, device=m.device)
    check(lib.r4d_topk_f64(_dev(m, torch.float64, "m"), rows, n, k, vals.data_ptr(), idx.data_ptr(), ws.data_ptr(),
                           ws.numel(), _stream()), "topk_f64")
    return vals, idx
```

Measured before the change: 39970.

## Fuse LayerNorm into residual-projection GEMM via per-row-block tickets

Adds a LayerNorm phase to the h2p GEMM residual epilogue. The last tile to finish a 128-row block, found by an atomic ticket counter, normalises those full rows and writes them in f16 line format. This is used for ln_2 after the attention projection and for the next layer's ln_1 after the MLP projection, which removes separate LayerNorm launches and a reread of the hidden state. The cost is a counter memset per call, cross-workgroup handoff through sc1 loads and stores, and a serial LN tail done by the last workgroup in each row block.

```diff
diff --git a/include/r4d.h b/include/r4d.h
--- a/include/r4d.h
+++ b/include/r4d.h
@@ -123,6 +123,11 @@
 int r4d_split2_lines_f16(const float* x_d, int64_t rows, int32_t K, uint16_t* lines_d, void* stream);
 int r4d_conv1d_h2p_f32(const uint16_t* x_lines_d, const uint16_t* planes_d, const float* bias_d, const float* residual_d, int32_t M,
                        int32_t K, int32_t N, int32_t epilogue, int32_t out_lines, void* y_d, void* stream);
+
+int r4d_set_ln_fusion(int32_t on);
+int r4d_conv1d_h2p_ln_f32(const uint16_t* x_lines_d, const uint16_t* planes_d, const float* bias_d, const float* residual_d, int32_t M,
+                          int32_t K, int32_t N, const float* ln_w_d, const float* ln_b_d, float eps, void* y_d, uint16_t* ln_lines_d,
+                          uint32_t* counters_d, void* stream);
 
 #define R4D_RANGE_NONFINITE_HIDDEN 1u
 #define R4D_RANGE_BAD_NORM 2u
diff --git a/rag4dyg_amd/_lib.py b/rag4dyg_amd/_lib.py
--- a/rag4dyg_amd/_lib.py
+++ b/rag4dyg_amd/_lib.py
@@ -79,6 +79,8 @@
     "r4d_layernorm_lines_f32": (c_int32, [_P, _P, _P, c_int32, c_int32, c_float, _P, _P]),
     "r4d_split2_lines_f16": (c_int32, [_P, c_int64, c_int32, _P, _P]),
     "r4d_conv1d_h2p_f32": (c_int32, [_P, _P, _P, _P, c_int32, c_int32, c_int32, c_int32, c_int32, _P, _P]),
+    "r4d_set_ln_fusion": (c_int32, [c_int32]),
+    "r4d_conv1d_h2p_ln_f32": (c_int32, [_P, _P, _P, _P, c_int32, c_int32, c_int32, _P, _P, c_float, _P, _P, _P, _P]),
     "r4d_pack_h2_words_f32": (c_int32, [_P, c_int64, _P, _P]),
     "r4d_attention_h2_f32": (c_int32, [_P, c_int32, c_int32, c_int32, c_int32, _P, _P]),
     "r4d_gpt2_decode_workspace_bytes": (c_size_t, [POINTER(GPT2ConfigC), c_int32]),
diff --git a/rag4dyg_amd/build.py b/rag4dyg_amd/build.py
--- a/rag4dyg_amd/build.py
+++ b/rag4dyg_amd/build.py
@@ -35,7 +35,11 @@
 
 
 HANDOFF_KERNELS = {"topk.hip": {"topk_chunk_kernelIfE": (4, 2), "topk_chunk_kernelIdE": (4, 2)},
-                   "gemm_skinny.hip": {"gemm_skinny16_kernelILi2ELi0E": (2, 1), "gemm_skinny16_kernelILi3ELi0E": (2, 1)}}
+                   "gemm_skinny.hip": {"gemm_skinny16_kernelILi2ELi0E": (2, 1), "gemm_skinny16_kernelILi3ELi0E": (2, 1)},
+                   "gemm_h2p.hip": {"gemm_h2p_kernelILi128ELi256ELi2ELb0ELi2ELi4ELb1EE": (128, 48, "buffer", True),
+                                    "gemm_h2p_kernelILi128ELi128ELi2ELb0ELi2ELi4ELb1EE": (64, 48, "buffer", True)}}
+HANDOFF_FORMS = {"global": (r"global_store_dword(?:x2)? [^\n]*", r"global_load_dword(?:x2)? [^\n]*"),
+                 "buffer": (r"buffer_store_dword [^\n]*", r"buffer_load_dwordx4 [^\n]*")}
 
 
 def check_handoff_lowering(src):
@@ -49,15 +53,22 @@
         if r.returncode != 0:
             raise RuntimeError(f"hipcc -S failed for {src}:\n{r.stderr}")
         text = open(asm).read()
-    for name, (want_st, want_ld) in names.items():
-        m = re.search(r"^(_ZN3r4d\d+" + re.escape(name) + r"[^\n:]*):[^\n]*\n(.*?)s_endpgm", text, re.S | re.M)
+    for name, spec in names.items():
+        want_st, want_ld = spec[:2]
+        st_re, ld_re = HANDOFF_FORMS[spec[2] if len(spec) > 2 else "global"]
+        only_sc1 = len(spec) > 3 and spec[3]
+        m = re.search(r"^(_ZN3r4d\d+" + re.escape(name) + r"[^\n:]*):[^\n]*\n(.*?)^\.Lfunc_end", text, re.S | re.M)
         if not m:
             raise RuntimeError(f"hand-off check: kernel {name} not found in the assembly of {src}")
         body = m.group(2)
-        stores = re.findall(r"global_store_dword(?:x2)? [^\n]*", body)
-        loads_sc1 = [ln for ln in re.findall(r"global_load_dword(?:x2)? [^\n]*", body) if " sc1" in ln]
+        stores = re.findall(st_re, body)
+        loads = re.findall(ld_re, body)
+        loads_sc1 = [ln for ln in loads if " sc1" in ln]
         stores_sc1 = [ln for ln in stores if " sc1" in ln]
         ticket = re.findall(r"global_atomic_add[^\n]*", body)
+        if only_sc1 and (len(stores_sc1) != len(stores) or len(loads_sc1) != len(loads)):
+            raise RuntimeError(f"hand-off check FAILED for {name}: {len(stores) - len(stores_sc1)} stores and {len(loads) - len(loads_sc1)} loads "
+                               f"of the handed-off rows carry no sc1 in {os.path.basename(src)}")
         if not ticket or len(stores_sc1) < want_st or len(loads_sc1) < want_ld:
             raise RuntimeError(f"hand-off check FAILED for {name}: {len(stores_sc1)} sc1 stores (want {want_st}), {len(loads_sc1)} sc1 loads (want {want_ld}), "
                                f"{len(ticket)} ticket atomics -- the relaxed agent-scope publish / consume of {os.path.basename(src)} "
diff --git a/rag4dyg_amd/csrc/common.h b/rag4dyg_amd/csrc/common.h
--- a/rag4dyg_amd/csrc/common.h
+++ b/rag4dyg_amd/csrc/common.h
@@ -140,7 +140,8 @@
 int launch_split2_planes(const float* w, int N, int K, long long ld_k, long long ld_n, unsigned short* planes, hipStream_t s);
 extern int g_gemm_h2p;
 bool gemm_h2p_supported(int M, int K, int N);
-int launch_gemm_h2p(const S3Args& a, const unsigned short* a_lines, bool out_lines, hipStream_t stream);
+struct H2PLn { const float* w; const float* b; float eps; float* lines; unsigned* counters; };
+int launch_gemm_h2p(const S3Args& a, const unsigned short* a_lines, bool out_lines, hipStream_t stream, const H2PLn* ln = nullptr);
 int launch_split2_lines(const float* x, long long rows, int K, unsigned short* lines, hipStream_t s);
 extern int g_gemm_split3;
 int conv1d(const float* x, const float* w, const float* wT, const float* bias, const float* resid, int M, int K, int N,
diff --git a/rag4dyg_amd/csrc/encoder.hip b/rag4dyg_amd/csrc/encoder.hip
--- a/rag4dyg_amd/csrc/encoder.hip
+++ b/rag4dyg_amd/csrc/encoder.hip
@@ -15,6 +15,7 @@
 }
 
 int g_gemm_split3 = 1;
+static int g_ln_fusion = 1;
 
 int conv1d(const float* x, const float* w, const float* wT, const float* bias, const float* resid, int M, int K,
            int N, int epilogue, float* y, hipStream_t s, float* skinny_scratch, bool sk_counters_zeroed,
@@ -49,13 +50,14 @@
 }
 
 static int conv1d_lines(const unsigned short* x_lines, const unsigned short* w2h, const float* bias, const float* resid, int M, int K, int N,
-                        int epilogue, void* y, bool out_lines, hipStream_t s, unsigned* kblk = nullptr, int kb_hd = 0) {
+                        int epilogue, void* y, bool out_lines, hipStream_t s, unsigned* kblk = nullptr, int kb_hd = 0,
+                        const H2PLn* ln = nullptr) {
     S3Args a;
     memset(&a, 0, sizeof(a));
     a.planes = w2h; a.C = (float*)y; a.bias = bias; a.resid = resid;
     a.M = M; a.N = N; a.K = K; a.lda = K; a.ldc = N; a.ldr = N; a.epilogue = epilogue;
     a.kblk = kblk; a.kb_hd = kb_hd;
-    return launch_gemm_h2p(a, x_lines, out_lines, s);
+    return launch_gemm_h2p(a, x_lines, out_lines, s, ln);
 }
 
 static inline int tpad(int T) { return (T + 127) / 128 * 128; }
@@ -113,9 +115,11 @@
 struct Workspace {
     float *x, *ln, *qkv, *att, *fc, *scores, *pool;
     unsigned* kblk;
+    unsigned* ln_cnt;
     size_t bytes;
 };
-static Workspace carve(void* base, size_t M, size_t score_floats, size_t pool_floats, int d) {
+static size_t ln_cnt_words(size_t M, int n_layer) { return 2 * (size_t)n_layer * ((M + 127) / 128); }
+static Workspace carve(void* base, size_t M, size_t score_floats, size_t pool_floats, int d, size_t cnt_words = 0) {
     size_t off = 0;
     auto take = [&](size_t nfloat) {
         float* p = base ? (float*)((char*)base + off) : nullptr;
@@ -127,6 +131,7 @@
     w.scores = take(score_floats);
     w.pool = take(pool_floats);
     w.kblk = reinterpret_cast<unsigned*>(take(kblk_words(M, d)));
+    w.ln_cnt = reinterpret_cast<unsigned*>(take(cnt_words));
     w.bytes = off;
     return w;
 }
@@ -165,6 +170,11 @@
     g_attention_kblk = on != 0;
     return prev;
 }
+int r4d_set_ln_fusion(int32_t on) {
+    const int prev = g_ln_fusion;
+    g_ln_fusion = on != 0;
+    return prev;
+}
 int r4d_set_attention_h2(int32_t on) {
     const int prev = g_attention_h2;
     g_attention_h2 = on != 0;
@@ -181,7 +191,7 @@
 size_t r4d_gpt2_workspace_bytes(const r4d_gpt2_config* cfg, int32_t B, int32_t T) {
     if (!cfg || B <= 0 || T <= 0) return 0;
     return carve(nullptr, (size_t)B * T, score_floats(B, cfg->n_head, T), lnf_meanpool_scratch_floats(B, T, cfg->n_embd),
-                 cfg->n_embd).bytes;
+                 cfg->n_embd, ln_cnt_words((size_t)B * T, cfg->n_layer)).bytes;
 }
 
 size_t r4d_gpt2_groups_workspace_bytes(const r4d_gpt2_config* cfg, int32_t n_groups, const int32_t* Bs,
@@ -195,7 +205,7 @@
         if (f > sc) sc = f;
         pl += lnf_meanpool_scratch_floats(Bs[g], Ts[g], cfg->n_embd);
     }
-    return carve(nullptr, M, sc, pl, cfg->n_embd).bytes;
+    return carve(nullptr, M, sc, pl, cfg->n_embd, ln_cnt_words(M, cfg->n_layer)).bytes;
 }
 
 }
@@ -224,17 +234,31 @@
     }
     R4D_REQUIRE(Mtot <= 0x7fffffff / (size_t)(16 * d), "gpt2: %zu rows in one call is too many", Mtot);
     const int M = (int)Mtot;
-    Workspace ws = carve(workspace_d, Mtot, sc, pl, d);
+    Workspace ws = carve(workspace_d, Mtot, sc, pl, d, ln_cnt_words(Mtot, cfg->n_layer));
     if (!workspace_d || workspace_bytes < ws.bytes) {
         set_error("gpt2: workspace %zu bytes < required %zu", workspace_bytes, ws.bytes);
         return R4D_ERR_WORKSPACE;
     }
+    auto layer_lines = [&](int l) {
+        const r4d_gpt2_layer& L = w->layers[l];
+        return g_gemm_split3 == 2 && g_gemm_h2p && L.c_attn_h2 && L.c_fc_h2 && L.mlp_proj_h2 && layernorm_lines_supported(d) &&
+               gemm_h2p_supported(M, d, 3 * d) && gemm_h2p_supported(M, d, 4 * d) && gemm_h2p_supported(M, 4 * d, d);
+    };
+    const size_t cnt_slice = (Mtot + 127) / 128;
+    bool ln_fuse = false;
+    for (int l = 0; l < cfg->n_layer && g_ln_fusion; ++l) ln_fuse = ln_fuse || layer_lines(l);
+    if (ln_fuse && hipMemsetAsync(ws.ln_cnt, 0, ln_cnt_words(Mtot, cfg->n_layer) * sizeof(unsigned), s) != hipSuccess) {
+        set_error("gpt2: memset of the LayerNorm tickets failed");
+        return R4D_ERR_HIP;
+    }
+    bool ln_1_done = false;
     for (int l = 0; l < cfg->n_layer; ++l) {
         const r4d_gpt2_layer& L = w->layers[l];
         R4D_REQUIRE(L.ln_1_w && L.c_attn_w && L.attn_proj_w && L.ln_2_w && L.c_fc_w && L.mlp_proj_w,
                     "gpt2: null weight in layer %d", l);
-        const bool lines = g_gemm_split3 == 2 && g_gemm_h2p && L.c_attn_h2 && L.c_fc_h2 && L.mlp_proj_h2 && layernorm_lines_supported(d) &&
-                           gemm_h2p_supported(M, d, 3 * d) && gemm_h2p_supported(M, d, 4 * d) && gemm_h2p_supported(M, 4 * d, d);
+        const bool have_ln_1 = ln_1_done;
+        ln_1_done = false;
+        const bool lines = layer_lines(l);
         unsigned short* ln_lines = reinterpret_cast<unsigned short*>(ws.ln);
         unsigned short* fc_lines = reinterpret_cast<unsigned short*>(ws.fc);
         if (l == 0) {
@@ -245,6 +269,7 @@
                                                    ws.x + r0 * d, ws.ln + r0 * d, s, lines);
                 if (rc) return rc;
             }
+        } else if (have_ln_1) {
         } else if ((rc = lines ? launch_layernorm_lines(ws.x, L.ln_1_w, L.ln_1_b, M, d, cfg->ln_eps, ln_lines, s)
                                : launch_layernorm(ws.x, L.ln_1_w, L.ln_1_b, M, d, cfg->ln_eps, ws.ln, s))) {
             return rc;
@@ -309,13 +334,22 @@
                 if ((rc = attention(qkv + G.row0 * 3 * d, G.B, G.T, H, d, ws.att + G.row0 * d, ws.scores, s))) return rc;
             }
         }
-        if (att_lines) rc = conv1d_lines(reinterpret_cast<const unsigned short*>(ws.att), L.attn_proj_h2, L.attn_proj_b, ws.x, M, d, d, EPI_RESIDUAL, ws.x, false, s);
+        const bool fuse_ln_2 = att_lines && ln_fuse;
+        if (fuse_ln_2) {
+            const H2PLn ln = {L.ln_2_w, L.ln_2_b, cfg->ln_eps, ws.ln, ws.ln_cnt + (size_t)(2 * l) * cnt_slice};
+            rc = conv1d_lines(reinterpret_cast<const unsigned short*>(ws.att), L.attn_proj_h2, L.attn_proj_b, ws.x, M, d, d, EPI_RESIDUAL, ws.x, false, s, nullptr, 0, &ln);
+        } else if (att_lines) rc = conv1d_lines(reinterpret_cast<const unsigned short*>(ws.att), L.attn_proj_h2, L.attn_proj_b, ws.x, M, d, d, EPI_RESIDUAL, ws.x, false, s);
         else rc = conv1d(ws.att, L.attn_proj_w, L.attn_proj_wT, L.attn_proj_b, ws.x, M, d, d, EPI_RESIDUAL, ws.x, s, nullptr, false, L.attn_proj_w3, L.attn_proj_h2);
         if (rc) return rc;
         if (lines) {
-            if ((rc = launch_layernorm_lines(ws.x, L.ln_2_w, L.ln_2_b, M, d, cfg->ln_eps, ln_lines, s))) return rc;
+            if (!fuse_ln_2 && (rc = launch_layernorm_lines(ws.x, L.ln_2_w, L.ln_2_b, M, d, cfg->ln_eps, ln_lines, s))) return rc;
             if ((rc = conv1d_lines(ln_lines, L.c_fc_h2, L.c_fc_b, nullptr, M, d, 4 * d, EPI_GELU, fc_lines, true, s))) return rc;
-            if ((rc = conv1d_lines(fc_lines, L.mlp_proj_h2, L.mlp_proj_b, ws.x, M, 4 * d, d, EPI_RESIDUAL, ws.x, false, s))) return rc;
+            if (ln_fuse && l + 1 < cfg->n_layer && layer_lines(l + 1) && w->layers[l + 1].ln_1_w && w->layers[l + 1].ln_1_b) {
+                const r4d_gpt2_layer& Ln = w->layers[l + 1];
+                const H2PLn ln = {Ln.ln_1_w, Ln.ln_1_b, cfg->ln_eps, ws.ln, ws.ln_cnt + (size_t)(2 * l + 1) * cnt_slice};
+                if ((rc = conv1d_lines(fc_lines, L.mlp_proj_h2, L.mlp_proj_b, ws.x, M, 4 * d, d, EPI_RESIDUAL, ws.x, false, s, nullptr, 0, &ln))) return rc;
+                ln_1_done = true;
+            } else if ((rc = conv1d_lines(fc_lines, L.mlp_proj_h2, L.mlp_proj_b, ws.x, M, 4 * d, d, EPI_RESIDUAL, ws.x, false, s))) return rc;
             continue;
         }
         if ((rc = launch_layernorm(ws.x, L.ln_2_w, L.ln_2_b, M, d, cfg->ln_eps, ws.ln, s))) return rc;
diff --git a/rag4dyg_amd/csrc/encoder_ops.hip b/rag4dyg_amd/csrc/encoder_ops.hip
--- a/rag4dyg_amd/csrc/encoder_ops.hip
+++ b/rag4dyg_amd/csrc/encoder_ops.hip
@@ -1,16 +1,12 @@
 #include <string.h>
 #include "common.h"
 #include "h2.h"
+#include "ln4_row.h"
 
 namespace r4d {
 
 constexpr int MAXV = 32;
 
-__device__ __forceinline__ float wave_sum(float v) {
-#pragma unroll
-    for (int o = 32; o > 0; o >>= 1) v += __shfl_xor(v, o, 64);
-    return v;
-}
 __device__ __forceinline__ float wave_max(float v) {
 #pragma unroll
     for (int o = 32; o > 0; o >>= 1) v = fmaxf(v, __shfl_xor(v, o, 64));
@@ -43,15 +39,6 @@
 #pragma unroll
     for (int i = 0; i < MAXV; ++i)
         if (i < nv) y_out[(long long)row * d + lane + 64 * i] = v[i] * w[lane + 64 * i] + b[lane + 64 * i];
-}
-
-__device__ __forceinline__ void store_lines4(float* y_rows, long long row, int d, int col, float a0, float a1, float a2, float a3) {
-    unsigned h0, l0, h1, l1;
-    split2_pair<true>(a0, a1, h0, l0);
-    split2_pair<true>(a2, a3, h1, l1);
-    unsigned char* dst = reinterpret_cast<unsigned char*>(y_rows) + row * (long long)d * 4 + (col >> 5) * 128 + (col & 31) * 2;
-    *reinterpret_cast<uint2*>(dst) = make_uint2(h0, h1);
-    *reinterpret_cast<uint2*>(dst + 64) = make_uint2(l0, l1);
 }
 
 template <int NQ, bool LINES = false>
@@ -65,28 +52,7 @@
     float4 v[NQ];
 #pragma unroll
     for (int i = 0; i < NQ; ++i) v[i] = (i < nq) ? xr[64 * i] : make_float4(0.f, 0.f, 0.f, 0.f);
-    float s_ = 0.f;
-#pragma unroll
-    for (int i = 0; i < NQ; ++i) s_ += (v[i].x + v[i].y) + (v[i].z + v[i].w);
-    const float mean = wave_sum(s_) / (float)d;
-    float q = 0.f;
-#pragma unroll
-    for (int i = 0; i < NQ; ++i)
-        if (i < nq) {
-            const float a0 = v[i].x - mean, a1 = v[i].y - mean, a2 = v[i].z - mean, a3 = v[i].w - mean;
-            q += (a0 * a0 + a1 * a1) + (a2 * a2 + a3 * a3);
-        }
-    const float rstd = rsqrtf(wave_sum(q) / (float)d + eps);
-    float4* yr = reinterpret_cast<float4*>(y_out + (long long)row * d) + lane;
-#pragma unroll
-    for (int i = 0; i < NQ; ++i)
-        if (i < nq) {
-            const float4 ww = reinterpret_cast<const float4*>(w)[lane + 64 * i], bb = reinterpret_cast<const float4*>(b)[lane + 64 * i];
-            const float4 y4 = make_float4((v[i].x - mean) * rstd * ww.x + bb.x, (v[i].y - mean) * rstd * ww.y + bb.y,
-                                          (v[i].z - mean) * rstd * ww.z + bb.z, (v[i].w - mean) * rstd * ww.w + bb.w);
-            if constexpr (LINES) store_lines4(y_out, row, d, 4 * lane + 256 * i, y4.x, y4.y, y4.z, y4.w);
-            else yr[64 * i] = y4;
-        }
+    ln4_row<NQ, LINES>(v, nq, d, lane, w, b, eps, y_out, row);
 }
 
 bool layernorm_lines_supported(int d) { return d % 256 == 0 && d <= 64 * MAXV; }
diff --git a/rag4dyg_amd/csrc/gemm_h2p.hip b/rag4dyg_amd/csrc/gemm_h2p.hip
--- a/rag4dyg_amd/csrc/gemm_h2p.hip
+++ b/rag4dyg_amd/csrc/gemm_h2p.hip
@@ -2,6 +2,7 @@
 #include <string.h>
 #include "common.h"
 #include "h2.h"
+#include "ln4_row.h"
 
 namespace r4d {
 
@@ -31,7 +32,29 @@
 struct H2PShape {
     int M, N, K, ldc, ldr;
     unsigned* kblk; int kb_hd;
+    H2PLn ln;
 };
+
+template <int NQ>
+__device__ __forceinline__ void h2p_ln_phase(float* xblk, int rows_blk, long long row0, int N, int wid, int lane, const H2PLn& ln) {
+    constexpr int RB = 16 / NQ;
+    const int nq = N >> 8;
+    const __amdgpu_buffer_rsrc_t x_rsrc = __builtin_amdgcn_make_buffer_rsrc(xblk, 0, rows_blk * N * 4, 0x00020000);
+    for (int rb = wid; rb < rows_blk; rb += 8 * RB) {
+        float4 v[RB][NQ];
+#pragma unroll
+        for (int k = 0; k < RB; ++k) {
+            const int r = min(rb + 8 * k, rows_blk - 1);
+#pragma unroll
+            for (int i = 0; i < NQ; ++i)
+                v[k][i] = (i < nq) ? __builtin_bit_cast(float4, __builtin_amdgcn_raw_buffer_load_b128(x_rsrc, (r * N + 4 * lane + 256 * i) * 4, 0, 16))
+                                   : make_float4(0.f, 0.f, 0.f, 0.f);
+        }
+#pragma unroll
+        for (int k = 0; k < RB; ++k)
+            if (rb + 8 * k < rows_blk) ln4_row<NQ, true>(v[k], nq, N, lane, ln.w, ln.b, ln.eps, ln.lines, row0 + rb + 8 * k);
+    }
+}
 
 __device__ __forceinline__ void h2p_dma2(const void* base, unsigned v0, unsigned v1, unsigned lds_dst) {
     unsigned keep;
@@ -53,7 +76,7 @@
 }
 template <int N_> __device__ __forceinline__ void h2p_wait_vm() { asm volatile("s_waitcnt vmcnt(%0)" :: "n"(N_) : "memory"); }
 
-template <int BM, int BN, int EPI, bool OUT_LINES, int WGM = 2, int WGN = 4>
+template <int BM, int BN, int EPI, bool OUT_LINES, int WGM = 2, int WGN = 4, bool LNF = false>
 __global__ __launch_bounds__(64 * WGM * WGN, (WGM * WGN) / 4) void gemm_h2p_kernel(const unsigned short* __restrict__ Al, const unsigned short* __restrict__ Bp,
                                                           float* __restrict__ Cg, const float* __restrict__ biasg,
                                                           const float* __restrict__ residg, const H2PShape g) {
@@ -64,7 +87,10 @@
     constexpr int NGA = BM / 8 / NW, NGB = BN / 8 / NW;
     constexpr int NDMA = NGA + NGB;
     static_assert(BM == 128 && (BN == 256 || BN == 128) && TM >= 1 && TN >= 1 && (NGA == 2 || NGA == 4) && (NGB == 2 || NGB == 4 || NGB == 8), "tile");
+    static_assert(!LNF || (EPI == EPI_RESIDUAL && !OUT_LINES && NW == 8), "LayerNorm fusion: the residual epilogue, 8 wavefronts");
+    constexpr int ST_AUX = LNF ? 16 : 0;
     __shared__ u32x4p lds[NBUF * STAGE];
+    __shared__ unsigned ticket_s;
 
     const int nblk = gridDim.x, xq = nblk >> 3, xr = nblk & 7, xcd = blockIdx.x & 7;
     const int bid = xcd * xq + min(xcd, xr) + (blockIdx.x >> 3);
@@ -292,12 +318,13 @@
                     } else {
 #pragma unroll
                         for (int r = 0; r < 16; ++r)
-                            __builtin_amdgcn_raw_buffer_store_b32(o[r], c_rsrc, lane_c, ((i * 32 + (r & 3) + 8 * (r >> 2)) * g.ldc + j * 32) * 4, 0);
+                            __builtin_amdgcn_raw_buffer_store_b32(o[r], c_rsrc, lane_c, ((i * 32 + (r & 3) + 8 * (r >> 2)) * g.ldc + j * 32) * 4, ST_AUX);
                     }
                 }
             }
-            return;
-        }
+        } else {
+        const __amdgpu_buffer_rsrc_t e_rsrc = __builtin_amdgcn_make_buffer_rsrc(
+            C + (long long)m0 * g.ldc + n0, 0, LNF ? ((min(BM, g.M - m0) - 1) * g.ldc + min(BN, g.N - n0)) * 4 : 0, 0x00020000);
 #pragma unroll
         for (int j = 0; j < TN; ++j) {
             const int col = n0 + wn * WN + j * 32 + li;
@@ -320,9 +347,25 @@
                                 __builtin_bit_cast(unsigned, v);
                         continue;
                     }
-                    if (row < g.M && col_ok) C[(long long)row * g.ldc + col] = v;
+                    if (row < g.M && col_ok) {
+                        if constexpr (LNF) __builtin_amdgcn_raw_buffer_store_b32(__builtin_bit_cast(unsigned, v), e_rsrc, ((row - m0) * g.ldc + (col - n0)) * 4, 0, ST_AUX);
+                        else C[(long long)row * g.ldc + col] = v;
+                    }
                 }
             }
+        }
+        }
+        if constexpr (LNF) {
+            h2p_wait_vm<0>();
+            __syncthreads();
+            if (tid == 0) ticket_s = __hip_atomic_fetch_add(g.ln.counters + tile_m, 1u, __ATOMIC_RELAXED, __HIP_MEMORY_SCOPE_AGENT);
+            __syncthreads();
+            if (ticket_s != (unsigned)tiles_n - 1u) return;
+            const int rows_blk = min(BM, g.M - m0);
+            const int wid_u = __builtin_amdgcn_readfirstlane(wid);
+            if (g.N <= 512) h2p_ln_phase<2>(C + (long long)m0 * g.N, rows_blk, m0, g.N, wid_u, lane, g.ln);
+            else if (g.N <= 1024) h2p_ln_phase<4>(C + (long long)m0 * g.N, rows_blk, m0, g.N, wid_u, lane, g.ln);
+            else h2p_ln_phase<8>(C + (long long)m0 * g.N, rows_blk, m0, g.N, wid_u, lane, g.ln);
         }
     }
 }
@@ -346,12 +389,19 @@
 }
 
 template <int BN>
-static int launch_h2p(const S3Args& a, const unsigned short* a_lines, bool out_lines, int cls, hipStream_t stream) {
+static int launch_h2p(const S3Args& a, const unsigned short* a_lines, bool out_lines, int cls, hipStream_t stream, const H2PLn* ln) {
     const int tiles = cdiv(a.M, 128) * cdiv(a.N, BN);
     ProfScope prof(cls, 2.0 * (double)a.M * a.N * a.K, stream);
     H2PShape sh;
     sh.M = a.M; sh.N = a.N; sh.K = a.K; sh.ldc = a.ldc; sh.ldr = a.ldr;
     sh.kblk = a.kblk; sh.kb_hd = a.kblk ? a.kb_hd : 0;
+    memset(&sh.ln, 0, sizeof(sh.ln));
+    if (ln) {
+        sh.ln = *ln;
+        hipLaunchKernelGGL((gemm_h2p_kernel<128, BN, EPI_RESIDUAL, false, 2, 4, true>), dim3(tiles), dim3(512), 0, stream, a_lines, a.planes, a.C, a.bias, a.resid, sh);
+        R4D_CHECK_LAUNCH("gemm_h2p+layernorm");
+        return R4D_OK;
+    }
 #define H2P_LAUNCH_(E, OL) hipLaunchKernelGGL((gemm_h2p_kernel<128, BN, E, OL>), dim3(tiles), dim3(512), 0, stream, a_lines, a.planes, a.C, a.bias, a.resid, sh)
     if (out_lines) {
         if (a.epilogue != EPI_GELU) { set_error("gemm_h2p: line output exists for the GELU epilogue only"); return R4D_ERR_INVALID; }
@@ -370,7 +420,7 @@
     return R4D_OK;
 }
 
-int launch_gemm_h2p(const S3Args& a, const unsigned short* a_lines, bool out_lines, hipStream_t stream) {
+int launch_gemm_h2p(const S3Args& a, const unsigned short* a_lines, bool out_lines, hipStream_t stream, const H2PLn* ln) {
     R4D_REQUIRE(a_lines && a.planes && a.C, "gemm_h2p: null pointer");
     R4D_REQUIRE(gemm_h2p_supported(a.M, a.K, a.N), "gemm_h2p: unsupported shape M=%d K=%d N=%d", a.M, a.K, a.N);
     R4D_REQUIRE(((uintptr_t)a_lines % 16) == 0 && ((uintptr_t)a.planes % 16) == 0, "gemm_h2p: alignment");
@@ -378,11 +428,19 @@
     R4D_REQUIRE(a.epilogue != EPI_RESIDUAL || a.resid, "gemm_h2p: the residual epilogue needs the second buffer");
     R4D_REQUIRE(!a.kblk || (a.epilogue == EPI_H2WORDS && a.N % 3 == 0 && a.kb_hd >= 32 && a.kb_hd % 32 == 0 && (a.N / 3) % a.kb_hd == 0),
                 "gemm_h2p: the key-blocked K image goes with the h2-word epilogue, N = 3 d and a head_dim that is a multiple of 32");
+    if (ln) {
+        R4D_REQUIRE(a.epilogue == EPI_RESIDUAL && !out_lines, "gemm_h2p: LayerNorm fusion goes with the residual epilogue only");
+        R4D_REQUIRE(a.N == a.ldc && a.N == a.ldr && layernorm_lines_supported(a.N),
+                    "gemm_h2p: LayerNorm fusion needs whole model rows (N = %d, ldc = %d, ldr = %d) and N %% 256 == 0", a.N, a.ldc, a.ldr);
+        R4D_REQUIRE(ln->w && ln->b && ln->lines && ln->counters, "gemm_h2p: LayerNorm fusion: null pointer");
+        R4D_REQUIRE((((uintptr_t)a.C | (uintptr_t)ln->lines | (uintptr_t)ln->w | (uintptr_t)ln->b) & 15) == 0 && ((uintptr_t)ln->counters & 3) == 0,
+                    "gemm_h2p: LayerNorm fusion: alignment");
+    }
     const long long b0 = (long long)cdiv(a.M, 128) * cdiv(a.N, 256), b1 = (long long)cdiv(a.M, 128) * cdiv(a.N, 128);
     const double c0 = (double)((b0 + 255) / 256) * 128 * 256, c1 = (double)((b1 + 255) / 256) * 128 * 128 / 0.9;
-    if (c1 < c0) { R4D_BRANCH(H2P_128x128); return launch_h2p<128>(a, a_lines, out_lines, PK_GEMM_H2_128x128, stream); }
+    if (c1 < c0) { R4D_BRANCH(H2P_128x128); return launch_h2p<128>(a, a_lines, out_lines, PK_GEMM_H2_128x128, stream, ln); }
     R4D_BRANCH(H2P_128x256);
-    return launch_h2p<256>(a, a_lines, out_lines, PK_GEMM_H2_128x256, stream);
+    return launch_h2p<256>(a, a_lines, out_lines, PK_GEMM_H2_128x256, stream, ln);
 }
 
 int launch_split2_lines(const float* x, long long rows, int K, unsigned short* lines, hipStream_t s) {
@@ -421,4 +479,19 @@
     return launch_gemm_h2p(a, x_lines_d, out_lines != 0, (hipStream_t)stream);
 }
 
-}
+int r4d_conv1d_h2p_ln_f32(const uint16_t* x_lines_d, const uint16_t* planes_d, const float* bias_d, const float* residual_d, int32_t M,
+                          int32_t K, int32_t N, const float* ln_w_d, const float* ln_b_d, float eps, void* y_d, uint16_t* ln_lines_d,
+                          uint32_t* counters_d, void* stream) {
+    R4D_REQUIRE(residual_d && ln_w_d && ln_b_d && ln_lines_d && counters_d, "conv1d_h2p_ln: null pointer");
+    R4D_REQUIRE(M >= 1, "conv1d_h2p_ln: M = %d", M);
+    S3Args a;
+    memset(&a, 0, sizeof(a));
+    a.planes = planes_d; a.C = (float*)y_d; a.bias = bias_d; a.resid = residual_d;
+    a.M = M; a.N = N; a.K = K; a.lda = K; a.ldc = N; a.ldr = N; a.epilogue = EPI_RESIDUAL;
+    H2PLn ln;
+    ln.w = ln_w_d; ln.b = ln_b_d; ln.eps = eps; ln.lines = reinterpret_cast<float*>(ln_lines_d); ln.counters = counters_d;
+    R4D_HIP(hipMemsetAsync(counters_d, 0, (size_t)cdiv(M, 128) * sizeof(uint32_t), (hipStream_t)stream));
+    return launch_gemm_h2p(a, x_lines_d, false, (hipStream_t)stream, &ln);
+}
+
+}
diff --git a/rag4dyg_amd/csrc/ln4_row.h b/rag4dyg_amd/csrc/ln4_row.h
--- /dev/null
+++ b/rag4dyg_amd/csrc/ln4_row.h
@@ -0,0 +1,49 @@
+#pragma once
+#include "common.h"
+#include "h2.h"
+
+namespace r4d {
+
+__device__ __forceinline__ float wave_sum(float v) {
+#pragma unroll
+    for (int o = 32; o > 0; o >>= 1) v += __shfl_xor(v, o, 64);
+    return v;
+}
+
+__device__ __forceinline__ void store_lines4(float* y_rows, long long row, int d, int col, float a0, float a1, float a2, float a3) {
+    unsigned h0, l0, h1, l1;
+    split2_pair<true>(a0, a1, h0, l0);
+    split2_pair<true>(a2, a3, h1, l1);
+    unsigned char* dst = reinterpret_cast<unsigned char*>(y_rows) + row * (long long)d * 4 + (col >> 5) * 128 + (col & 31) * 2;
+    *reinterpret_cast<uint2*>(dst) = make_uint2(h0, h1);
+    *reinterpret_cast<uint2*>(dst + 64) = make_uint2(l0, l1);
+}
+
+template <int NQ, bool LINES>
+__device__ __forceinline__ void ln4_row(const float4 (&v)[NQ], int nq, int d, int lane, const float* __restrict__ w,
+                                        const float* __restrict__ b, float eps, float* __restrict__ y_out, long long row) {
+    float s_ = 0.f;
+#pragma unroll
+    for (int i = 0; i < NQ; ++i) s_ += (v[i].x + v[i].y) + (v[i].z + v[i].w);
+    const float mean = wave_sum(s_) / (float)d;
+    float q = 0.f;
+#pragma unroll
+    for (int i = 0; i < NQ; ++i)
+        if (i < nq) {
+            const float a0 = v[i].x - mean, a1 = v[i].y - mean, a2 = v[i].z - mean, a3 = v[i].w - mean;
+            q += (a0 * a0 + a1 * a1) + (a2 * a2 + a3 * a3);
+        }
+    const float rstd = rsqrtf(wave_sum(q) / (float)d + eps);
+    float4* yr = reinterpret_cast<float4*>(y_out + row * d) + lane;
+#pragma unroll
+    for (int i = 0; i < NQ; ++i)
+        if (i < nq) {
+            const float4 ww = reinterpret_cast<const float4*>(w)[lane + 64 * i], bb = reinterpret_cast<const float4*>(b)[lane + 64 * i];
+            const float4 y4 = make_float4((v[i].x - mean) * rstd * ww.x + bb.x, (v[i].y - mean) * rstd * ww.y + bb.y,
+                                          (v[i].z - mean) * rstd * ww.z + bb.z, (v[i].w - mean) * rstd * ww.w + bb.w);
+            if constexpr (LINES) store_lines4(y_out, row, d, 4 * lane + 256 * i, y4.x, y4.y, y4.z, y4.w);
+            else yr[64 * i] = y4;
+        }
+}
+
+}
diff --git a/rag4dyg_amd/ops.py b/rag4dyg_amd/ops.py
--- a/rag4dyg_amd/ops.py
+++ b/rag4dyg_amd/ops.py
@@ -147,6 +147,28 @@
     return y
 
 
+def set_ln_fusion(on):
+    return bool(_lib.load().r4d_set_ln_fusion(1 if on else 0))
+
+
+def conv1d_h2p_ln(x_lines, planes, bias, residual, ln_w, ln_b, eps=1e-5, out=None, ln_lines=None, counters=None):
+    N, K = planes.shape[0], planes.shape[1] * 32
+    M = x_lines.shape[0]
+    dev = x_lines.device
+    y = out if out is not None else torch.empty(M, N, dtype=torch.float32, device=dev)
+    lines = ln_lines if ln_lines is not None else torch.empty(M, N // 32, 2, 32, dtype=torch.int16, device=dev)
+    cnt = counters if counters is not None else torch.empty((M + 127) // 128, dtype=torch.int32, device=dev)
+    if tuple(y.shape) != (M, N) or lines.numel() != M * N or cnt.numel() < (M + 127) // 128:
+        raise ValueError("conv1d_h2p_ln: out / ln_lines / counters have the wrong size")
+    bp = _dev(bias, torch.float32, "bias") if bias is not None else None
+    check(_lib.load().r4d_conv1d_h2p_ln_f32(_dev(x_lines, torch.int16, "x_lines"), _dev(planes, torch.int16, "planes"), bp,
+                                            _dev(residual, torch.float32, "residual"), M, K, N, _dev(ln_w, torch.float32, "ln_w"),
+                                            _dev(ln_b, torch.float32, "ln_b"), eps, _dev(y, torch.float32, "out"),
+                                            _dev(lines, torch.int16, "ln_lines"), _dev(cnt, torch.int32, "counters"), _stream()),
+          "conv1d_h2p_ln")
+    return y, lines
+
+
 def conv1d_h2(x, planes, bias, epilogue="none", residual=None):
     N, K = planes.shape[0], planes.shape[1] * 32
     M = x.numel() // K
```

After: 39310. 1.7% lower.
